# facebookresearch/gtn

Hardware: AMD Instinct MI355X
Metric: CTC forward+backward losses/sec (T=1000, C=256) (higher is better)
Workload: dtype f32; 1 GPU; BASELINE config C3: compose(ctc_target, emissions)+forwardScore CTC loss fwd+bwd, T=1000, C=256, U=100, batch=512 per GPU; global_batch=512, parallelism=dp1 (utterance sharding, all_gather of losses), rccl_ranks=0

## Files before the change

gtn_amd/_capi.py:

```python
import ctypes as C
import os

c_graph = C.c_void_p
c_graph_p = C.POINTER(C.c_void_p)
c_i32_p = C.POINTER(C.c_int)
c_i64_p = C.POINTER(C.c_int64)
c_u8_p = C.POINTER(C.c_uint8)
c_f32_p = C.POINTER(C.c_float)

GRAD_FN = C.CFUNCTYPE(C.c_int, C.c_void_p, c_graph_p, C.c_int, c_graph)
CTX_FREE = C.CFUNCTYPE(None, C.c_void_p)

OK, INVALID_ARGUMENT, LOGIC_ERROR, RUNTIME_ERROR, OUT_OF_RANGE, DEVICE_ERROR = range(6)

_SIGS = {
    "gtnx_set_device": [C.c_int],
    "gtnx_get_device": [c_i32_p],
    "gtnx_set_stream": [C.c_void_p],
    "gtnx_compose_mode": [C.c_int, C.POINTER(C.c_int)],
    "gtnx_synchronize": [],
    "gtnx_memory_stats": [C.POINTER(C.c_uint64), C.POINTER(C.c_uint64)],
    "gtnx_empty_cache": [],
    "gtnx_reclaim": [],
    "gtnx_graph_create": [C.c_int, c_graph_p],
    "gtnx_graph_copy": [c_graph, c_graph_p],
    "gtnx_graph_deep_copy": [c_graph, c_graph_p],
    "gtnx_graph_destroy": [c_graph],
    "gtnx_graph_add_node": [c_graph, C.c_int, C.c_int, c_i32_p],
    "gtnx_graph_add_arc": [c_graph, C.c_int, C.c_int, C.c_int, C.c_int, C.c_float, c_i32_p],
    "gtnx_graph_add_nodes": [c_graph, C.c_int, C.c_void_p, C.c_void_p],
    "gtnx_graph_add_arcs": [c_graph, C.c_int, C.c_void_p, C.c_void_p, C.c_void_p, C.c_void_p, C.c_void_p],
    "gtnx_graph_num_nodes": [c_graph, c_i64_p],
    "gtnx_graph_num_arcs": [c_graph, c_i64_p],
    "gtnx_graph_num_start": [c_graph, c_i64_p],
    "gtnx_graph_num_accept": [c_graph, c_i64_p],
    "gtnx_graph_item": [c_graph, c_f32_p],
    "gtnx_graph_arc_sort": [c_graph, C.c_int],
    "gtnx_graph_mark_arc_sorted": [c_graph, C.c_int],
    "gtnx_graph_ilabel_sorted": [c_graph, c_i32_p],
    "gtnx_graph_olabel_sorted": [c_graph, c_i32_p],
    "gtnx_graph_weights": [c_graph, C.c_int, C.POINTER(c_f32_p)],
    "gtnx_graph_get_weights": [c_graph, C.c_void_p],
    "gtnx_graph_set_weights": [c_graph, C.c_void_p],
    "gtnx_graph_set_weights_device": [c_graph, C.c_void_p],
    "gtnx_graph_weights_device": [c_graph, C.POINTER(C.c_void_p)],
    "gtnx_graph_labels_to_array": [c_graph, C.c_void_p, C.c_int],
    "gtnx_graph_get_start": [c_graph, C.c_void_p],
    "gtnx_graph_get_accept": [c_graph, C.c_void_p],
    "gtnx_graph_is_start": [c_graph, C.c_int, c_i32_p],
    "gtnx_graph_is_accept": [c_graph, C.c_int, c_i32_p],
    "gtnx_graph_make_accept": [c_graph, C.c_int],
    "gtnx_graph_num_out": [c_graph, C.c_int, c_i64_p],
    "gtnx_graph_num_in": [c_graph, C.c_int, c_i64_p],
    "gtnx_graph_get_out": [c_graph, C.c_int, C.c_void_p],
    "gtnx_graph_get_in": [c_graph, C.c_int, C.c_void_p],
    "gtnx_graph_get_arcs": [c_graph, C.c_void_p, C.c_void_p, C.c_void_p, C.c_void_p],
    "gtnx_graph_get_arc": [c_graph, C.c_int, c_i32_p, c_i32_p, c_i32_p, c_i32_p, c_f32_p],
    "gtnx_graph_set_weight": [c_graph, C.c_int, C.c_float],
    "gtnx_graph_calc_grad": [c_graph, c_i32_p],
    "gtnx_graph_set_calc_grad": [c_graph, C.c_int],
    "gtnx_graph_is_grad_available": [c_graph, c_i32_p],
    "gtnx_graph_grad": [c_graph, c_graph_p],
    "gtnx_graph_zero_grad": [c_graph],
    "gtnx_graph_add_grad": [c_graph, C.c_void_p, C.c_int64],
    "gtnx_graph_add_grad_graph": [c_graph, c_graph],
    "gtnx_graph_id": [c_graph, C.POINTER(C.c_size_t)],
    "gtnx_graph_create_op": [c_graph_p, C.c_int, GRAD_FN, C.c_void_p, CTX_FREE, c_graph_p],
    "gtnx_graph_num_inputs": [c_graph, c_i64_p],
    "gtnx_graph_get_input": [c_graph, C.c_int, c_graph_p],
    "gtnx_graph_set_inputs": [c_graph, c_graph_p, C.c_int],
    "gtnx_graph_set_grad_fn": [c_graph, GRAD_FN, C.c_void_p, CTX_FREE],
    "gtnx_graph_has_grad_fn": [c_graph, c_i32_p],
    "gtnx_scalar_graph": [C.c_float, C.c_int, c_graph_p],
    "gtnx_linear_graph": [C.c_int, C.c_int, C.c_int, c_graph_p],
    "gtnx_linear_graph_n": [C.c_int, C.c_int, C.c_int, C.c_int, C.c_void_p, c_graph_p],
    "gtnx_linear_graph_borrow_n": [C.c_int, C.c_int, C.c_int, C.c_int, C.c_void_p, c_graph_p],
    "gtnx_negate": [c_graph, c_graph_p],
    "gtnx_add": [c_graph, c_graph, c_graph_p],
    "gtnx_subtract": [c_graph, c_graph, c_graph_p],
    "gtnx_compose": [c_graph, c_graph, c_graph_p],
    "gtnx_intersect": [c_graph, c_graph, c_graph_p],
    "gtnx_forward_score": [c_graph, c_graph_p],
    "gtnx_viterbi_score": [c_graph, c_graph_p],
    "gtnx_viterbi_path": [c_graph, c_graph_p],
    "gtnx_negate_n": [c_graph_p, C.c_int, c_graph_p],
    "gtnx_add_n": [c_graph_p, C.c_int, c_graph_p, C.c_int, c_graph_p],
    "gtnx_subtract_n": [c_graph_p, C.c_int, c_graph_p, C.c_int, c_graph_p],
    "gtnx_compose_n": [c_graph_p, C.c_int, c_graph_p, C.c_int, c_graph_p],
    "gtnx_intersect_n": [c_graph_p, C.c_int, c_graph_p, C.c_int, c_graph_p],
    "gtnx_forward_score_n": [c_graph_p, C.c_int, c_graph_p],
    "gtnx_viterbi_score_n": [c_graph_p, C.c_int, c_graph_p],
    "gtnx_viterbi_path_n": [c_graph_p, C.c_int, c_graph_p],
    "gtnx_items_n": [c_graph_p, C.c_int, C.c_void_p],
    "gtnx_items_device_n": [c_graph_p, C.c_int, C.c_void_p],
    "gtnx_grads_device_n": [c_graph_p, C.c_int, C.c_void_p, C.c_void_p],
    "gtnx_grads_bind_device_n": [c_graph_p, C.c_int, C.c_void_p, C.c_void_p],
    "gtnx_clone": [c_graph, C.c_int, c_graph_p],
    "gtnx_concat": [c_graph_p, C.c_int, c_graph_p],
    "gtnx_closure": [c_graph, c_graph_p],
    "gtnx_union": [c_graph_p, C.c_int, c_graph_p],
    "gtnx_batch_from_graphs": [c_graph_p, C.c_int, c_graph_p],
    "gtnx_batch_ctc_targets": [C.c_void_p, C.c_void_p, C.c_int, C.c_int, C.c_int, c_graph_p],
    "gtnx_batch_asg_force_align": [C.c_void_p, C.c_void_p, C.c_int, c_graph, C.c_int, c_graph_p],
    "gtnx_batch_linear": [C.c_int, C.c_int, C.c_int, C.c_int, C.c_void_p, C.c_int, c_graph_p],
    "gtnx_batch_linear_rows": [C.c_int, C.c_int, C.c_int, C.c_void_p, C.c_int, C.c_void_p, C.c_int, c_graph_p],
    "gtnx_batch_destroy": [c_graph],
    "gtnx_batch_size": [c_graph, c_i32_p],
    "gtnx_batch_get": [c_graph, C.c_int, c_graph_p],
    "gtnx_batch_negate": [c_graph, c_graph_p],
    "gtnx_batch_add": [c_graph, c_graph, c_graph_p],
    "gtnx_batch_subtract": [c_graph, c_graph, c_graph_p],
    "gtnx_batch_subtract_into": [c_graph, c_graph, C.c_void_p, c_graph_p],
    "gtnx_batch_compose": [c_graph, c_graph, c_graph_p],
    "gtnx_batch_intersect": [c_graph, c_graph, c_graph_p],
    "gtnx_batch_forward_score": [c_graph, c_graph_p],
    "gtnx_batch_viterbi_score": [c_graph, c_graph_p],
    "gtnx_batch_viterbi_path": [c_graph, c_graph_p],
    "gtnx_batch_viterbi_align": [c_graph, C.c_void_p, C.c_void_p, C.c_int64, C.c_void_p, C.c_void_p],
    "gtnx_batch_align_stats": [c_i64_p, c_i64_p],
    "gtnx_batch_viterbi_decode": [c_graph, c_graph, C.c_void_p, C.c_void_p, C.c_int64, C.c_void_p, C.c_void_p,
                                  C.c_void_p],
    "gtnx_batch_decode_stats": [c_i64_p, c_i64_p],
    "gtnx_batch_full_connect_stats": [c_i64_p, c_i64_p],
    "gtnx_batch_linear_decode": [c_graph, C.c_void_p, C.c_int, C.c_void_p, C.c_int64, C.c_void_p, C.c_void_p,
                                 C.c_void_p, C.c_void_p],
    "gtnx_batch_linear_decode_stats": [c_i64_p, c_i64_p],
    "gtnx_batch_backward": [c_graph, C.c_int],
    "gtnx_batch_items": [c_graph, C.c_void_p],
    "gtnx_batch_items_device": [c_graph, C.c_void_p],
    "gtnx_batch_grads_bind_device": [c_graph, C.c_void_p, C.c_void_p],
    "gtnx_batch_grads_device": [c_graph, C.c_void_p, C.c_void_p],
    "gtnx_backward": [c_graph, C.c_int],
    "gtnx_backward_with_grad": [c_graph, c_graph, C.c_int],
    "gtnx_backward_n": [c_graph_p, C.c_int, C.c_int],
    "gtnx_equal": [c_graph, c_graph, c_i32_p],
    "gtnx_isomorphic": [c_graph, c_graph, c_i32_p],
    "gtnx_remove": [c_graph, C.c_int, C.c_int, c_graph_p],
    "gtnx_graph_load_buffer": [C.c_void_p, C.c_size_t, c_graph_p],
    "gtnx_parallel_enter": [],
    "gtnx_parallel_leave": [],
    "gtnx_parallel_flush": [],
    "gtnx_prof_enable": [C.c_int],
    "gtnx_prof_reset": [],
    "gtnx_prof_get": [C.c_char_p, C.POINTER(C.c_double), c_i64_p, C.POINTER(C.c_double)],
    "gtnx_prof_names": [C.c_char_p, C.c_size_t],
    "gtnx_debug_symbolic_route": [c_graph, C.c_int, c_i32_p],
    "gtnx_debug_route_name": [C.c_int, C.c_char_p, C.c_size_t],
    "gtnx_debug_viterbi_ties": [c_i64_p, c_i64_p],
    "gtnx_debug_tie_ranks": [c_graph, C.c_void_p, C.c_void_p, C.c_void_p],
    "gtnx_comm_create": [c_i32_p, C.c_int, C.POINTER(C.c_void_p)],
    "gtnx_comm_destroy": [C.c_void_p],
    "gtnx_comm_size": [C.c_void_p, c_i32_p],
    "gtnx_comm_all_gather_f32": [C.c_void_p, C.POINTER(C.c_void_p), C.POINTER(C.c_void_p), C.c_int64],
    "gtnx_comm_all_reduce_sum_f32": [C.c_void_p, C.POINTER(C.c_void_p), C.c_int64],
}

_RESTYPE = {
    "gtnx_last_error": (C.c_char_p, []),
    "gtnx_version": (C.c_char_p, []),
    "gtnx_backend": (C.c_char_p, []),
    "gtnx_device_count": (C.c_int, []),
}

ALL_SYMBOLS = sorted(list(_SIGS) + list(_RESTYPE))


def default_library_path():
    return os.path.join(os.path.dirname(os.path.abspath(__file__)), "lib", "libgtn_amd.so")


def load(path=None):
    path = path or default_library_path()
    if not os.path.exists(path):
        raise ImportError(
            f"gtn_amd: native library not found at {path}. Build it with "
            "`python -c 'import __graft_entry__ as g; g.build()'` (hipcc, gfx950). "
            "There is no CPU fallback."
        )
    lib = C.CDLL(path, mode=C.RTLD_GLOBAL if hasattr(C, "RTLD_GLOBAL") else 0)
    for name, args in _SIGS.items():
        try:
            fn = getattr(lib, name)
        except AttributeError:
            if name.startswith("gtnx_batch_") or name.startswith("gtnx_comm_") or name in ("gtnx_linear_graph_borrow_n", "gtnx_grads_bind_device_n",
                                                             "gtnx_parallel_enter", "gtnx_parallel_leave", "gtnx_parallel_flush"):
                continue
            raise
        fn.argtypes = args
        fn.restype = C.c_int
    for name, (res, args) in _RESTYPE.items():
        fn = getattr(lib, name)
        fn.argtypes = args
        fn.restype = res
    lib._path = path
    return lib
```

gtn_amd/criteria/ctc_criterion.h:

```cpp
#pragma once

#include <chrono>
#include <cstdint>
#include <stdexcept>
#include <vector>

#include "gtn/gtn.h"

namespace gtn {
namespace criteria {

inline Graph ctcTargetGraph(const std::vector<int>& target, int blank = 0, bool calcGrad = true) {
  const int L = 2 * (int)target.size() + 1;
  std::vector<uint8_t> st(L, 0), ac(L, 0);
  std::vector<int> src, dst, lab;
  src.reserve(3 * L);
  dst.reserve(3 * L);
  lab.reserve(3 * L);
  for (int l = 0; l < L; l++) {
    const int idx = (l - 1) / 2;
    st[l] = l == 0;
    ac[l] = l == L - 1 || l + 2 == L;
    const int label = l % 2 ? target[idx] : blank;
    src.push_back(l), dst.push_back(l), lab.push_back(label);
    if (l > 0) src.push_back(l - 1), dst.push_back(l), lab.push_back(label);
    if (l % 2 && l > 1 && label != target[idx - 1]) src.push_back(l - 2), dst.push_back(l), lab.push_back(label);
  }
  Graph ctc(calcGrad);
  detail::check(gtnx_graph_add_nodes(ctc.handle(), L, st.data(), ac.data()));
  detail::check(gtnx_graph_add_arcs(ctc.handle(), (int)src.size(), src.data(), dst.data(), lab.data(), lab.data(), nullptr));
  ctc.arcSort();
  return ctc;
}

struct CtcStepTimes {
  double build = 0, linear = 0, intersect = 0, forward = 0, backward = 0;
};

inline void ctcLossBatch(
    const void* emissions,
    const int* labels,
    const int* lengths,
    int B,
    int T,
    int C,
    int blank,
    void* lossDev,
    void* gradDev,
    bool targetGrad = true,
    CtcStepTimes* times = nullptr,
    Batch* targetsOut = nullptr,
    const int* frames = nullptr) {
  auto now = [] { return std::chrono::steady_clock::now(); };
  auto ms = [](auto a, auto b) { return std::chrono::duration<double, std::milli>(b - a).count(); };
  if (frames)
    for (int b = 0; b < B; ++b)
      if (frames[b] < 1 || frames[b] > T) throw std::invalid_argument("[ctcLossBatch] a frame count outside 1 .. T");
  auto t0 = now();
  Batch ctcs = Batch::ctcTargets(labels, lengths, B, blank, targetGrad);
  auto t1 = now();
  Batch ems = Batch::linear(B, T, C, emissions, gradDev != nullptr, true, frames);
  std::vector<int64_t> off(B);
  for (int b = 0; b < B; ++b) off[b] = (int64_t)b * T * C;
  if (gradDev) ems.bindGrads(gradDev, off.data());
  auto t2 = now();
  Batch comp = batched::intersect(ctcs, ems);
  auto t3 = now();
  Batch score = batched::forwardScore(comp);
  Batch norm = batched::forwardScore(ems);
  Batch losses = batched::subtract(norm, score, lossDev);
  auto t4 = now();
  if (gradDev) batched::backward(losses);
  auto t5 = now();
  if (times) *times = {ms(t0, t1), ms(t1, t2), ms(t2, t3), ms(t3, t4), ms(t4, t5)};
  losses.itemsToDevice(lossDev);
  if (gradDev) ems.gradsToDevice(gradDev, off.data());
  if (targetsOut) *targetsOut = std::move(ctcs);
}

inline void ctcLossBatch(
    const void* emissions,
    const std::vector<std::vector<int>>& targets,
    int T,
    int C,
    int blank,
    void* lossDev,
    void* gradDev,
    bool targetGrad = true,
    CtcStepTimes* times = nullptr) {
  std::vector<int> flat, len;
  for (auto& t : targets) {
    flat.insert(flat.end(), t.begin(), t.end());
    len.push_back((int)t.size());
  }
  ctcLossBatch(emissions, flat.data(), len.data(), (int)targets.size(), T, C, blank, lossDev, gradDev, targetGrad, times);
}

inline void ctcAlignBatch(
    const void* emissions,
    const int* targets,
    const int* lengths,
    int B,
    int T,
    int C,
    int blank,
    const int* frames,
    void* labels,
    void* tokens,
    void* scores) {
  Batch ctcs = Batch::ctcTargets(targets, lengths, B, blank, false);
  Batch ems = Batch::linear(B, T, C, emissions, false, true);
  Batch comp = batched::intersect(ctcs, ems);
  batched::viterbiAlign(comp, static_cast<int*>(labels), T, static_cast<int*>(tokens), static_cast<float*>(scores), frames);
}

inline void ctcDecodeBatch(
    const void* emissions,
    int B,
    int T,
    int C,
    int blank,
    const int* frames,
    void* labelsDev,
    void* scoresDev,
    void* collapsedDev,
    void* startsDev,
    void* lengthsDev) {
  Batch ems = Batch::linear(B, T, C, emissions, false, true);
  batched::linearDecode(ems, static_cast<int*>(labelsDev), T, static_cast<float*>(scoresDev), frames, blank,
                        static_cast<int*>(collapsedDev), static_cast<int*>(startsDev), static_cast<int*>(lengthsDev));
}

}
}
```

gtn_amd/csrc/band.hip:

```cpp
#include <hip/hip_runtime.h>

#include <algorithm>
#include <cstdlib>
#include <stdexcept>
#include <type_traits>

#include "kernels.h"

#ifdef GTNX_BAND_TIMING
__device__ long long g_band_timing[256];
#endif

namespace gtnx {
namespace {

constexpr float NEGF = -1.0e30f;
constexpr float DEADF = -1.0e29f;
constexpr float LOG2E = 1.44269504088896340736f;
constexpr double LN2 = 0.693147180559945309417;
constexpr int BW = 256;
constexpr int WG = 512;
constexpr int WGB = 768;
constexpr int NBE = 5;
constexpr int NBG = 7;
// ... 172 lines not shown
          }
        }
      }
    }
  }
}

__device__ __forceinline__ float em2(float x) { return fmaxf(x * LOG2E, NEGF); }

__device__ __forceinline__ int row_of(int e, int W, float invW) {
  int r = int(float(e) * invW);
  if (r * W > e) --r;
  if ((r + 1) * W <= e) ++r;
  return r;
}

template <int NS, int LN = BW>
struct Stage {
  float v[NS];
  template <bool VEC>
  __device__ __forceinline__ void issue(const GTNX_G float* src, int cnt, int tid) {
    if (cnt <= 0) return;
#pragma unroll
    for (int i = 0; i < NS / 4; ++i) {
      if (i > 0 && 4 * i * LN >= cnt) break;
      const int e = min(4 * (i * LN + tid), cnt - 4);
      const gtnx_f4 q = *reinterpret_cast<const GTNX_G gtnx_f4*>(reinterpret_cast<const GTNX_G char*>(src) + unsigned(4 * e));
      v[4 * i] = q.x;
      v[4 * i + 1] = q.y;
      v[4 * i + 2] = q.z;
      v[4 * i + 3] = q.w;
    }
  }
  int off[NS / 4];
  __device__ __forceinline__ void init_offsets(int W, int stride, int K, int tid, bool reverse = true) {
    const float invW = 1.0f / float(W);
#pragma unroll
    for (int i = 0; i < NS / 4; ++i) {
      const int e = 4 * (i * LN + tid);
      const int r = row_of(min(e, 4096), W, invW);
      off[i] = (reverse ? K - 1 - r : r) * stride + (e - r * W);
    }
  }
  template <class F>
  __device__ __forceinline__ void each_vec(int cnt, int shift, int tid, F&& f) const {
#pragma unroll
    for (int i = 0; i < NS / 4; ++i) {
      if (i > 0 && 4 * i * LN >= cnt) break;
      if (4 * (i * LN + tid) < cnt) f(i, off[i] - shift, gtnx_f4{v[4 * i], v[4 * i + 1], v[4 * i + 2], v[4 * i + 3]});
    }
  }
  __device__ __forceinline__ void settle_all() {
#pragma unroll
    for (int i = 0; i < NS; ++i) asm volatile("" : "+v"(v[i]));
  }
  template <bool VEC, class F>
  __device__ __forceinline__ void each(int cnt, int W, int tid, F&& f) const {
    const float invW = 1.0f / float(W);
    if constexpr (VEC) {
#pragma unroll
      for (int i = 0; i < NS / 4; ++i) {
        if (i > 0 && 4 * i * LN >= cnt) break;
        const int e = 4 * (i * LN + tid);
        if (e < cnt) {
          const int r = row_of(e, W, invW);
          f(i, e, r, e - r * W, gtnx_f4{v[4 * i], v[4 * i + 1], v[4 * i + 2], v[4 * i + 3]});
        }
      }
    } else {
#pragma unroll
      for (int i = 0; i < NS / 4; ++i) {
        if (i > 0 && 4 * i * LN >= cnt) break;
        if (4 * (i * LN + tid) < cnt) {
          const int e = min(4 * (i * LN + tid), cnt - 4);
          const int r0 = row_of(e, W, invW), c0 = e - r0 * W;
#pragma unroll
          for (int k = 0; k < 4; ++k) {
            int r = r0, col = c0 + k;
            if (col >= W) {
              col -= W;
              ++r;
            }
            f(i, e + k, r, col, gtnx_f4{v[4 * i + k], 0.0f, 0.0f, 0.0f});
          }
        }
      }
    }
  }
};

struct BandLds {
  int CS;
  int o_ering, o_aring, o_oring, o_snode, o_misc, total;
};
__host__ __device__ inline BandLds band_lds(int C, int K, int NSmax, bool backward) {
  BandLds L;
  L.CS = C + 4;
  int o = 0;
  L.o_ering = o;
  o += (backward ? NBGE : NBE) * K * L.CS;
  o = (o + 3) & ~3;
  L.o_aring = o;
  o += backward ? NBE * K * NSmax : 0;
  o = (o + 3) & ~3;
  L.o_oring = o;
  o += backward ? max(NBG * K * NSmax, 2 * C) : 0;
  o = (o + 3) & ~3;
  L.o_snode = o;
  o += backward ? 512 : 0;
  L.o_misc = o;
  o += 160 + 32 + 8 + 2 * NBE * K * 4 + 40 * K + 8 + 512;
  L.total = o;
  return L;
}
struct BandMisc {
  double *offr, *red, *find, *aofr;
  float *bndr, *fin, *lsep;
};
template <int K>
__device__ __forceinline__ BandMisc band_misc(float* lds, const BandLds& L) {
  BandMisc m;
  m.offr = reinterpret_cast<double*>(lds + L.o_misc);
  m.red = m.offr + 80;
  m.find = m.red + 16;
  m.aofr = m.find + 4;
  m.bndr = lds + L.o_misc + 200 + 2 * NBE * K * 4;
  m.fin = m.bndr + 40 * K;
  m.lsep = m.fin + 8;
  return m;
}

__device__ __forceinline__ float wave_max_of(const float* v, int n) {
  float mx = v[0];
  for (int j = 1; j < n; ++j) mx = fmaxf(mx, v[j]);
  return wave_max(mx);
}

template <int NPL, bool UNIT, int K, bool VEC>
__global__ __launch_bounds__(WG) void band_forward_kernel(const BandPair* __restrict__ pairs, int NSmax) {
#define GTNX_BAND_PAIR pairs[blockIdx.x]
#include "band_forward_body.inc"
#undef GTNX_BAND_PAIR
}
template <int NPL, bool UNIT, int K, bool VEC>
__global__ __launch_bounds__(WG) void band_forward_one_kernel(BandPair one, int NSmax) {
#define GTNX_BAND_PAIR one
#include "band_forward_body.inc"
#undef GTNX_BAND_PAIR
}

__device__ __forceinline__ BandPair band_patched(BandPair P, const BandPatch& pt) {
  if (pt.on) {
    const int b = P.bidx;
    P.delta = pt.delta + b;
    P.delta_norm = pt.delta_norm ? pt.delta_norm + b : nullptr;
    P.rowlse = pt.rowlse ? pt.rowlse + int64_t(b) * pt.M : nullptr;
    P.norm = nullptr;
    P.em_copy = nullptr;
    P.grad_em = pt.grad_em ? pt.grad_em + int64_t(b) * pt.A : nullptr;
    P.grad_fixed = pt.grad_fixed ? pt.grad_fixed + P.goff : nullptr;
  }
  return P;
}
template <int NPL, bool UNIT, bool GRADG, int K, bool VEC, bool BIG>
__global__ __launch_bounds__(WGB, BIG ? 3 : 6) void band_backward_kernel(const BandPair* __restrict__ pairs, int NSmax, BandPatch patch) {
#define GTNX_BAND_PAIR band_patched(pairs[blockIdx.x], patch)
#include "band_backward_body.inc"
#undef GTNX_BAND_PAIR
}
template <int NPL, bool UNIT, bool GRADG, int K, bool VEC, bool BIG>
__global__ __launch_bounds__(WGB, BIG ? 3 : 6) void band_backward_one_kernel(BandPair one, int NSmax) {
#define GTNX_BAND_PAIR one
#include "band_backward_body.inc"
#undef GTNX_BAND_PAIR
}


__global__ __launch_bounds__(512) void ctc_targets_kernel(const CtcTargetArgs* __restrict__ args, int blank) {
  const CtcTargetArgs a = args[blockIdx.x];
  __shared__ __attribute__((aligned(16))) int tl[256 + 4];
  __shared__ __attribute__((aligned(16))) int tk[256 + 4];
  const int N = a.N, U = (N - 1) >> 1, m = threadIdx.x;
  if (m < 260) {
    const int v = m < U ? a.labels[m] : 0x7fffffff;
    tl[m] = v;
    tk[m] = (m > 0 && m < U && v != a.labels[m - 1]) ? 1 : 0;
  }
  __syncthreads();
  if (m >= N) return;
  const bool odd = (m & 1) != 0;
  const int my = odd ? tl[(m - 1) >> 1] : blank;
  const int skip = odd ? tk[(m - 1) >> 1] : 0;
  const int mi = (m - 1) >> 1;
  const int before = odd ? mi : (m >> 1);
  int rank = 0, skips = 0;
  for (int o = 0; o < U; o += 4) {
    const gtnx_i4 l4 = *reinterpret_cast<const gtnx_i4*>(tl + o), k4 = *reinterpret_cast<const gtnx_i4*>(tk + o);
    const int lo[4] = {l4.x, l4.y, l4.z, l4.w}, ko[4] = {k4.x, k4.y, k4.z, k4.w};
#pragma unroll
    for (int k = 0; k < 4; ++k) {
      const bool front = o + k < before;
      rank += (lo[k] < my || (lo[k] == my && front)) ? 1 : 0;
      skips += front ? ko[k] : 0;
    }
  }
  rank += blank < my ? U + 1 : (blank == my ? (m + 1) >> 1 : 0);
  const int base = (m > 0 ? 2 * m - 1 : 0) + skips;
  GTNX_G BandNode* nd = const_cast<GTNX_G BandNode*>(a.nodes);
  nd[m].lab = my;
  nd[m].aid[0] = base;
  nd[m].aid[1] = m > 0 ? base + 1 : -1;
  nd[m].aid[2] = skip ? base + 2 : -1;
  a.nflags[m] = uint8_t((m == 0 ? NF_START : 0) | (m + 2 >= N ? NF_ACCEPT : 0));
  a.snode[rank] = m;
  a.slab[rank] = my;
  if (m == N - 1 && a.n_arcs) a.n_arcs[0] = base + 1 + (m > 0 ? 1 : 0) + skip;
}

__global__ __launch_bounds__(512) void band_viterbi_kernel(const BandDecode* __restrict__ pairs) {
  const BandDecode P = pairs[blockIdx.x];
  const int T = P.T, C = P.C, N = P.N, NS = P.NS;
  extern __shared__ float lds[];
  const float NINF = -__builtin_inff();
  float* a0 = lds;
  float* a1 = lds + 516;
  float* stage = lds + 1032;
  const int m = threadIdx.x;
  const GTNX_G gtnx_i4* nodes = reinterpret_cast<const GTNX_G gtnx_i4*>(P.nodes);
  int lab = 0;
  float wi[3] = {NINF, NINF, NINF};
  bool accept = false, start = false;
  if (m < N) {
    const gtnx_i4 q = nodes[m];
    lab = q.x >= 0 ? q.x : 0;
    const int a[3] = {q.y, q.z, q.w};
#pragma unroll
    for (int k = 0; k < 3; ++k)
      if (a[k] >= 0) wi[k] = P.w ? P.w[a[k]] : 0.0f;
    const uint8_t f = P.nflags[m];
    start = (f & NF_START) != 0;
    accept = (f & NF_ACCEPT) != 0;
  }
  if (m < 2) a0[m] = a1[m] = NINF;
  a0[2 + m] = start ? 0.0f : NINF;
  a1[2 + m] = NINF;
  int tie = 0;
  const int R = max(1, min(64, P.stage_floats / C));
  float* cur = a0;
  float* nxt = a1;
  __syncthreads();
  for (int t0 = 0; t0 < T; t0 += R) {
    const int rows = min(R, T - t0);
    for (int e = threadIdx.x; e < rows * C; e += blockDim.x) stage[e] = P.em[int64_t(t0) * C + e];
    __syncthreads();
    for (int i = 0; i < rows; ++i) {
      const float e = stage[i * C + lab];
      const float c0 = cur[2 + m] + (wi[0] + e), c1 = cur[1 + m] + (wi[1] + e), c2 = cur[m] + (wi[2] + e);
      float best = c0;
      int k = 0;
      if (c1 > best) best = c1, k = 1;
      if (c2 > best) best = c2, k = 2;
      if (best > NINF && ((k != 0 && c0 == best) || (k != 1 && c1 == best) || (k != 2 && c2 == best))) tie = 1;
      if (m < NS) P.bp[int64_t(t0 + i) * NS + m] = uint8_t(best > NINF ? k : 3);
      nxt[2 + m] = m < N ? best : NINF;
      __syncthreads();
      float* sw = cur;
      cur = nxt;
      nxt = sw;
    }
  }
  __shared__ float red_v[8];
  __shared__ int red_m[8], s_best, s_tie;
  float v = accept ? cur[2 + m] : NINF;
  int bm = (m < N && accept && v > NINF) ? m : 1 << 30;
  const float wmx = wave_max(v);
  if (!(v == wmx)) bm = 1 << 30;
  int cnt = (bm != (1 << 30)) ? 1 : 0;
  for (int o = 32; o > 0; o >>= 1) {
    bm = min(bm, __shfl_xor(bm, o));
    cnt += __shfl_xor(cnt, o);
  }
  if ((threadIdx.x & 63) == 0) {
    red_v[threadIdx.x >> 6] = wmx;
    red_m[threadIdx.x >> 6] = bm;
  }
  if (cnt > 1) tie = 1;
  if (threadIdx.x == 0) s_tie = 0;
  __syncthreads();
  if (threadIdx.x == 0) {
    float bv = NINF;
    int bn = -1;
    for (int w = 0; w < 8; ++w) {
      if (red_m[w] == (1 << 30)) continue;
      if (red_v[w] > bv) bv = red_v[w], bn = red_m[w];
      else if (red_v[w] == bv && bv > NINF) s_tie = 1;
    }
    s_best = bn;
    P.score[0] = bv;
  }
  if (tie) atomicOr(&s_tie, 1);
  __syncthreads();
  const int best = s_best;
  if (threadIdx.x == 0) {
    P.tie[0] = s_tie;
    P.path_len[0] = best >= 0 ? T : -1;
  }
  if (best < 0 || T == 0) return;
  uint8_t* bst = reinterpret_cast<uint8_t*>(stage);
  const int RB = max(1, min(T, P.stage_floats * 4 / NS));
  __shared__ int s_node;
  if (threadIdx.x == 0) {
    s_node = best;
    P.pnode[T] = best;
  }
  for (int hi = T; hi > 0; hi -= RB) {
    const int lo = max(0, hi - RB);
    __syncthreads();
    for (int e = threadIdx.x; e < (hi - lo) * NS; e += blockDim.x) bst[e] = P.bp[int64_t(lo) * NS + e];
    __syncthreads();
    if (threadIdx.x == 0) {
      int node = s_node;
      for (int t = hi - 1; t >= lo; --t) {
        node -= bst[(t - lo) * NS + node] & 3;
        P.pnode[t] = node;
      }
      s_node = node;
    }
  }
  __threadfence_block();
  __syncthreads();
  for (int t = threadIdx.x; t < T; t += blockDim.x) {
    const int m1 = P.pnode[t + 1], k = m1 - P.pnode[t];
    const gtnx_i4 q = nodes[m1];
    const int arc = k == 0 ? q.y : (k == 1 ? q.z : q.w);
    P.path_arc[t] = arc;
    P.path_lab[t] = q.x;
    P.path_w[t] = (P.w ? P.w[arc] : 0.0f) + P.em[int64_t(t) * C + q.x];
  }
}

constexpr int VBLK = 2048;

template <int NPL, bool RANKED>
__global__ __launch_bounds__(64) void band_viterbi_wave_kernel(const BandDecode* __restrict__ pairs) {
  const BandDecode P = pairs[blockIdx.x];
  const int T = P.T, C = P.C, N = P.N;
  const int lane = threadIdx.x;
  constexpr int SPW = 16 / NPL;
  constexpr int NLD = VBLK / 256;
  __shared__ __attribute__((aligned(16))) float ring[3 * VBLK];
  const float NINF = -__builtin_inff();
  const GTNX_G gtnx_i4* nodes = reinterpret_cast<const GTNX_G gtnx_i4*>(P.nodes);
  int loff[NPL];
  float w0[NPL], w1[NPL], w2[NPL], alpha[NPL];
  bool acc[NPL];
#pragma unroll
  for (int j = 0; j < NPL; ++j) {
    const int m = lane * NPL + j;
    loff[j] = 0;
    w0[j] = w1[j] = w2[j] = NINF;
    alpha[j] = NINF;
    acc[j] = false;
    if (m < N) {
      const gtnx_i4 q = nodes[m];
      loff[j] = 4 * (q.x >= 0 ? q.x : 0);
      if (q.y >= 0) w0[j] = P.w ? P.w[q.y] : 0.0f;
      if (q.z >= 0) w1[j] = P.w ? P.w[q.z] : 0.0f;
      if (q.w >= 0) w2[j] = P.w ? P.w[q.w] : 0.0f;
      const uint8_t f = P.nflags[m];
// ... 279 lines not shown
    big_lds(band_backward_kernel<NPL, false, true, K, VEC, BIG>);
    big_lds(band_backward_kernel<NPL, false, false, K, VEC, BIG>);
    if constexpr (ONE) {
      big_lds(band_backward_one_kernel<NPL, true, true, K, VEC, BIG>);
      big_lds(band_backward_one_kernel<NPL, true, false, K, VEC, BIG>);
      big_lds(band_backward_one_kernel<NPL, false, true, K, VEC, BIG>);
      big_lds(band_backward_one_kernel<NPL, false, false, K, VEC, BIG>);
    }
  }
  if constexpr (ONE) {
    if (one) {
      if (unit) {
        if (gradg) hipLaunchKernelGGL((band_backward_one_kernel<NPL, true, true, K, VEC, BIG>), dim3(1), dim3(WGB), lds, st, *one, ns);
        else hipLaunchKernelGGL((band_backward_one_kernel<NPL, true, false, K, VEC, BIG>), dim3(1), dim3(WGB), lds, st, *one, ns);
      } else {
        if (gradg) hipLaunchKernelGGL((band_backward_one_kernel<NPL, false, true, K, VEC, BIG>), dim3(1), dim3(WGB), lds, st, *one, ns);
        else hipLaunchKernelGGL((band_backward_one_kernel<NPL, false, false, K, VEC, BIG>), dim3(1), dim3(WGB), lds, st, *one, ns);
      }
      return;
    }
  }
  if (unit) {
    if (gradg) hipLaunchKernelGGL((band_backward_kernel<NPL, true, true, K, VEC, BIG>), dim3(n), dim3(WGB), lds, st, d, ns, pt);
    else hipLaunchKernelGGL((band_backward_kernel<NPL, true, false, K, VEC, BIG>), dim3(n), dim3(WGB), lds, st, d, ns, pt);
  } else {
    if (gradg) hipLaunchKernelGGL((band_backward_kernel<NPL, false, true, K, VEC, BIG>), dim3(n), dim3(WGB), lds, st, d, ns, pt);
    else hipLaunchKernelGGL((band_backward_kernel<NPL, false, false, K, VEC, BIG>), dim3(n), dim3(WGB), lds, st, d, ns, pt);
  }
}
template <int NPL, int K>
void launch_bwd(const BandPair* d, const BandPair* one, int n, int ns, size_t lds, bool unit, bool gradg, bool vec, bool big,
                hipStream_t st, const BandPatch& pt) {
  if constexpr (K == 2) {
    if (big) {
      if (vec) launch_bwd3<NPL, K, true, true>(d, one, n, ns, lds, unit, gradg, st, pt);
      else launch_bwd3<NPL, K, false, true>(d, one, n, ns, lds, unit, gradg, st, pt);
      return;
    }
  }
  if (vec) launch_bwd3<NPL, K, true, false>(d, one, n, ns, lds, unit, gradg, st, pt);
  else launch_bwd3<NPL, K, false, false>(d, one, n, ns, lds, unit, gradg, st, pt);
}

constexpr size_t LDS_TWO = 78 * 1024;
constexpr size_t LDS_ONE = 156 * 1024;

}

int band_block_rows(int C, int max_NS, bool backward);
static int band_backward_lds_stride(int K, int max_NS) { return K == 4 ? (max_NS + 15) / 16 * 16 : max_NS; }
int band_max_nodes() { return 512; }
int band_max_labels() { return 1024; }
int band_min_labels() { return 4; }
int band_npl(int max_nodes) { return max_nodes <= 256 ? 1 : 2; }
int band_row_stride(int N, int) { return (N + 3) / 4 * 4; }
#ifndef GTNX_FWD_SHIFT_ROWS
#define GTNX_FWD_SHIFT_ROWS 4
#endif
int band_forward_lgrn(int C) {
  const int K = band_block_rows(C, 0, false);
  return K >= GTNX_FWD_SHIFT_ROWS ? (GTNX_FWD_SHIFT_ROWS == 8 ? 3 : 2) : (K >= 4 ? 2 : 1);
}
int band_block_rows(int C, int max_NS, bool backward) {
  for (int k = backward ? 4 : 8; k >= 2; k /= 2) {
    if (k * C > 2048 || k * max_NS > 2048) continue;
    if (backward && k > 2 && (k * C > 1024 || k * max_NS > 1024)) continue;
    const int ns_lds = backward ? band_backward_lds_stride(k, max_NS) : max_NS;
    if (4 * size_t(band_lds(C, k, ns_lds, backward).total) + 64 <= LDS_TWO) return k;
  }
  if (4 * size_t(band_lds(C, 2, max_NS, backward).total) + 64 <= LDS_ONE) return 2;
  return 0;
}

bool band_one_ok(int npl, int C, int max_NS, bool vec, bool backward) {
  if (npl != 1 || !vec) return false;
  if (!backward) return true;
  const int K = band_block_rows(C, max_NS, true);
  return !(K * C > 1024 || K * max_NS > 1024);
}
void launch_band_forward(const BandPair* d_pairs, int n, int npl, int C, int max_NS, bool unit, bool vec, hipStream_t st,
                         const BandPair* one) {
  if (n <= 0) return;
  if (one && (n != 1 || !band_one_ok(npl, C, max_NS, vec, false))) throw std::logic_error("band.hip: not a single-pair launch");
  const int K = band_block_rows(C, 0, false);
  const size_t lds = 4 * size_t(band_lds(C, K, max_NS, false).total) + 64;
  if (npl == 1) {
    if (K == 8) launch_fwd<1, 8>(d_pairs, one, n, max_NS, lds, unit, vec, st);
    else if (K == 4) launch_fwd<1, 4>(d_pairs, one, n, max_NS, lds, unit, vec, st);
    else launch_fwd<1, 2>(d_pairs, one, n, max_NS, lds, unit, vec, st);
  } else {
    if (K == 8) launch_fwd<2, 8>(d_pairs, one, n, max_NS, lds, unit, vec, st);
    else if (K == 4) launch_fwd<2, 4>(d_pairs, one, n, max_NS, lds, unit, vec, st);
    else launch_fwd<2, 2>(d_pairs, one, n, max_NS, lds, unit, vec, st);
  }
}

void launch_band_backward(const BandPair* d_pairs, int n, int npl, int C, int max_NS, bool unit, bool gradg, bool vec,
                          hipStream_t st, const BandPair* one, const BandPatch* patch) {
  if (n <= 0) return;
  if (one && patch) throw std::logic_error("band.hip: a patched launch reads a device table");
  BandPatch pt{};
  if (patch) pt = *patch;
  if (one && (n != 1 || !band_one_ok(npl, C, max_NS, vec, true))) throw std::logic_error("band.hip: not a single-pair launch");
  const int K = band_block_rows(C, max_NS, true);
  const bool big = K * C > 1024 || K * max_NS > 1024;
  const int ns_lds = band_backward_lds_stride(K, max_NS);
  const size_t lds = 4 * size_t(band_lds(C, K, ns_lds, true).total) + 64;
  if (npl == 1) {
    if (K == 4) launch_bwd<1, 4>(d_pairs, one, n, ns_lds, lds, unit, gradg, vec, big, st, pt);
    else launch_bwd<1, 2>(d_pairs, one, n, ns_lds, lds, unit, gradg, vec, big, st, pt);
  } else {
    if (K == 4) throw std::logic_error("band.hip: four rows per block with two nodes per lane");
    launch_bwd<2, 2>(d_pairs, one, n, ns_lds, lds, unit, gradg, vec, big, st, pt);
  }
}

template <int NPL>
static void launch_viterbi_wave(const BandDecode* d_pairs, int n, int ranked, hipStream_t st) {
  if (ranked) hipLaunchKernelGGL((band_viterbi_wave_kernel<NPL, true>), dim3(n), dim3(64), 0, st, d_pairs);
  else hipLaunchKernelGGL((band_viterbi_wave_kernel<NPL, false>), dim3(n), dim3(64), 0, st, d_pairs);
}
bool band_viterbi_wave_ok(int max_nodes, int max_labels, int vec) {
  static const bool force_wg = std::getenv("GTNX_VITERBI_WG") != nullptr;
  return !force_wg && vec && max_nodes <= 512 && max_labels <= VBLK;
}
void launch_band_viterbi(const BandDecode* d_pairs, int n, int stage_floats, int max_nodes, int max_labels, int vec,
                         hipStream_t st, int ranked) {
  if (n <= 0) return;
  if (band_viterbi_wave_ok(max_nodes, max_labels, vec)) {
    if (max_nodes <= 64) launch_viterbi_wave<1>(d_pairs, n, ranked, st);
    else if (max_nodes <= 128) launch_viterbi_wave<2>(d_pairs, n, ranked, st);
    else if (max_nodes <= 256) launch_viterbi_wave<4>(d_pairs, n, ranked, st);
    else launch_viterbi_wave<8>(d_pairs, n, ranked, st);
    return;
  }
  if (ranked) return;
  static std::atomic<uint64_t> done{0};
  if (gtnx_first_on_device first{done}) big_lds(band_viterbi_kernel);
  hipLaunchKernelGGL(band_viterbi_kernel, dim3(n), dim3(512), 4 * size_t(1032 + stage_floats) + 64, st, d_pairs);
}

void launch_asg_fal_targets(const AsgFalArgs* d_args, int n, int n_labels, hipStream_t st) {
  if (n > 0) hipLaunchKernelGGL(asg_fal_targets_kernel, dim3(n), dim3(512), 0, st, d_args, n_labels);
}
void launch_asg_fal_scatter(const float* g, const int* maps, const int64_t* tab, int n_seq, int64_t longest, float* trans_grad,
                            hipStream_t st) {
  if (n_seq > 0 && longest > 0)
    hipLaunchKernelGGL(asg_fal_scatter_kernel, dim3(unsigned(std::min<int64_t>((longest + 255) / 256, 64)), unsigned(n_seq)),
                       dim3(256), 0, st, g, maps, tab, trans_grad);
}
void launch_ctc_targets(const CtcTargetArgs* d_args, int n, int blank, hipStream_t st) {
  if (n > 0) hipLaunchKernelGGL(ctc_targets_kernel, dim3(n), dim3(512), 0, st, d_args, blank);
}

}
```

gtn_amd/csrc/band_forward_body.inc:

```
#ifndef GTNX_FWD_SHIFT_ROWS
#define GTNX_FWD_SHIFT_ROWS 4
#endif
  constexpr int RNk = K >= GTNX_FWD_SHIFT_ROWS ? GTNX_FWD_SHIFT_ROWS : (K >= 4 ? 4 : K);
  constexpr int NP = K / RNk;
  constexpr int D = 8 / K > GTNX_FWD_DEPTH ? 8 / K : GTNX_FWD_DEPTH;
  const BandPair P = GTNX_BAND_PAIR;
  const int T = P.T, C = P.C, NS = P.NS;
  extern __shared__ float lds[];
  const BandLds L = band_lds(C, K, NSmax, false);
  float* ering = lds + L.o_ering;
  const BandMisc M = band_misc<K>(lds, L);
  const int CS = L.CS;
  const int wv = __builtin_amdgcn_readfirstlane(threadIdx.x >> 6);
  const bool sweeper = wv < 4;
  const int l = threadIdx.x & 63;
  const int nblocks = (T + K - 1) / K;
  const int nticks = nblocks + 3;
  GTNX_TM_INIT(0);

  if (sweeper) {
    __builtin_amdgcn_s_setprio(1);
    const int w = wv;
    const int m0 = threadIdx.x * NPL;
    NodeRegs<NPL> g;
// ... 179 lines not shown
      constexpr bool COPY = decltype(copy_tag)::value;
      float* base = ering + c5 * K * CS;
      GTNX_G float* cdst = em_copy + int64_t(c) * K * C;
      s.template each<VEC>(rows_of(c) * C, C, hid, [&](int, int e, int r, int col, gtnx_f4 q) {
        float* d = base + r * CS + col;
        if (vec) *reinterpret_cast<gtnx_f4*>(d) = gtnx_f4{em2(q.x), em2(q.y), em2(q.z), em2(q.w)};
        else d[0] = em2(q.x);
        if (COPY) {
          if (vec) __builtin_nontemporal_store(q, reinterpret_cast<GTNX_G gtnx_f4*>(cdst + e));
          else __builtin_nontemporal_store(q.x, cdst + e);
        }
      });
    };
    constexpr int LPR = BW / K, G16 = LPR / 16;
    const int EPL = (C + LPR - 1) / LPR;
    double normacc = 0.0;
    auto lse_a_n = [&](int c, int c5 , auto nconst) {
      constexpr int NE = decltype(nconst)::value;
      const int rows = rows_of(c), rr = hid / LPR, sub = hid - rr * LPR;
      if (rows <= 0) return;
      const float* e = ering + (c5 * K + min(rr, rows - 1)) * CS + sub * EPL;
      float x[NE];
      float m = NEGF;
      if (VEC && (EPL & 3) == 0) {
#pragma unroll
        for (int i = 0; i < NE; i += 4) {
          const bool in = i < EPL && sub * EPL + i < C;
          const gtnx_f4 q = in ? *reinterpret_cast<const gtnx_f4*>(e + i) : gtnx_f4{NEGF, NEGF, NEGF, NEGF};
          x[i] = q.x, x[i + 1] = q.y, x[i + 2] = q.z, x[i + 3] = q.w;
          m = fmaxf(fmaxf(m, fmaxf(q.x, q.y)), fmaxf(q.z, q.w));
        }
      } else {
#pragma unroll
        for (int i = 0; i < NE; ++i) {
          x[i] = (i < EPL && sub * EPL + i < C) ? e[i] : NEGF;
          m = fmaxf(m, x[i]);
        }
      }
      m = row16_max(m);
      float sum = 0.0f;
#pragma unroll
      for (int i = 0; i < NE; ++i) sum += (i < EPL) ? ex2(x[i] - m) : 0.0f;
      sum = row16_sum(sum);
      if ((hid & 15) == 0 && rr < rows) {
        float* p = M.lsep + (c & 1) * 256 + (rr * 8 + (sub >> 4)) * 2;
        p[0] = m;
        p[1] = sum;
      }
    };
    auto lse_a = [&](int c, int c5) {
      if (EPL <= 4) lse_a_n(c, c5, std::integral_constant<int, 4>{});
      else if (EPL <= 8) lse_a_n(c, c5, std::integral_constant<int, 8>{});
      else lse_a_n(c, c5, std::integral_constant<int, 16>{});
    };
    auto lse_b = [&](int c) {
      const int rows = rows_of(c);
      if (hid < rows) {
        const float* p = M.lsep + (c & 1) * 256 + hid * 16;
        float Mx = p[0];
#pragma unroll
        for (int k = 1; k < G16; ++k) Mx = fmaxf(Mx, p[2 * k]);
        float S = 0.0f;
#pragma unroll
        for (int k = 0; k < G16; ++k) S += p[2 * k + 1] * ex2(p[2 * k] - Mx);
        const float l2 = Mx + lg2(S);
        if (P.rowlse) P.rowlse[c * K + hid] = l2;
        normacc += double(l2);
      }
    };
    auto run = [&](auto copy_tag) {
      issue(st[0], 0);
      land(st[0], 0, 0, copy_tag);
#pragma unroll
      for (int c = 1; c <= D; ++c) issue(st[c % D], c);
      lds_barrier();
      int t5 = 0;
      for (int tau0 = 0; tau0 < nticks; tau0 += D) {
#pragma unroll
        for (int d = 0; d < D; ++d) {
          const int tau = tau0 + d;
          if (tau >= nticks) break;
          GTNX_TM(0);
          const int n5 = t5 + 1 == NBE ? 0 : t5 + 1;
          land(st[(d + 1) % D], tau + 1, n5, copy_tag);
          GTNX_TM(1);
          issue(st[(d + 1) % D], tau + 1 + D);
          GTNX_TM(2);
          if (want_lse) {
            if (tau >= 1 && tau - 1 < nblocks) lse_b(tau - 1);
            if (tau < nblocks) lse_a(tau, t5);
          }
          t5 = n5;
          GTNX_TM(4);
          lds_barrier();
          GTNX_TM(6);
          GTNX_TM_TICK();
        }
      }
    };
    auto run_copy = [&]() {
      constexpr int DC = GTNX_FWD_COPY_DEPTH < 8 / K ? 8 / K : GTNX_FWD_COPY_DEPTH;
      constexpr int R = DC + 1;
      Stage<8> sc[R];
      issue(sc[0], 0);
      land(sc[0], 0, 0, std::true_type{});
#pragma unroll
      for (int c = 1; c <= DC; ++c) issue(sc[c % R], c);
      lds_barrier();
      int t5 = 0;
      for (int tau0 = 0; tau0 < nticks; tau0 += R) {
#pragma unroll
        for (int d = 0; d < R; ++d) {
          const int tau = tau0 + d;
          if (tau >= nticks) break;
          GTNX_TM(0);
          const int n5 = t5 + 1 == NBE ? 0 : t5 + 1;
          sc[(d + 1) % R].settle_all();
          issue(sc[d % R], tau + 1 + DC);
          GTNX_TM(2);
          land(sc[(d + 1) % R], tau + 1, n5, std::true_type{});
          GTNX_TM(1);
          if (want_lse) {
            if (tau >= 1 && tau - 1 < nblocks) lse_b(tau - 1);
            if (tau < nblocks) lse_a(tau, t5);
          }
          t5 = n5;
          GTNX_TM(4);
          lds_barrier();
          GTNX_TM(6);
          GTNX_TM_TICK();
        }
      }
    };
    if (em_copy) {
      if (GTNX_FWD_COPY_ROTATE) run_copy();
      else run(std::true_type{});
    } else {
      run(std::false_type{});
    }
    if (hid < 16) M.red[hid] = normacc;
  }
  GTNX_TM_DUMP();
  lds_barrier();
  if (threadIdx.x == 0) {
    double Mx = double(NEGF);
    for (int k = 0; k < 4; ++k)
      if (M.fin[2 * k] > DEADF) Mx = fmax(Mx, M.find[k] + double(M.fin[2 * k]));
    const bool dead = !(Mx > double(DEADF));
    float S = 0.0f;
    for (int k = 0; k < 4; ++k)
      if (M.fin[2 * k] > DEADF) S += M.fin[2 * k + 1] * ex2(float(M.find[k] + double(M.fin[2 * k]) - Mx));
    const double z2 = dead ? double(NEGF) : Mx + double(lg2(S));
    P.aoff[0] = z2;
    P.score[0] = dead ? -__builtin_inff() : float(z2 * LN2);
    if (P.norm) {
      double n2 = 0.0;
      for (int k = 0; k < 16; ++k) n2 += M.red[k];
      P.norm[0] = n2 < double(DEADF) ? -__builtin_inff() : float(n2 * LN2);
    }
  }
```

gtn_amd/csrc/batch.cpp:

```cpp
#include "batch.h"

#include <algorithm>
#include <atomic>
#include <cstdlib>
#include <cstring>
#include <limits>
#include <unordered_map>
#include <unordered_set>

namespace gtnx {

namespace {

std::atomic<uint64_t> g_batch_seq{1};

struct CompMode {
  int old;
  CompMode() : old(compose_mode_hint(2)) {}
  ~CompMode() { compose_mode_hint(old); }
};

BatchP make_batch(Batch::Kind k, int n, bool cg) {
  auto b = std::make_shared<Batch>();
  b->kind = k;
// ... 231 lines not shown
    }
    DevMemP dt = upload_vec(tab);
    launch_asg_fal_scatter(out.g_dev, out.rec_mem->as<int>(), dt->as<int64_t>(), out.n, longest, gm->as<float>(), rt.stream());
    tr.add_grad_device(gm, gm->as<float>(), true);
  }
};

std::atomic<int64_t> g_full_fast{0}, g_full_fallback{0};
struct BFullOp : BatchOp {
  AsgFullArgs args{};
  DevMemP arena;
  DevMemP rows_mem;
  DevMemP w_mem;
  DevMemP through_acc;
  void backward(Batch& out) override {
    Batch& prod = *inputs[0];
    Batch& ch = *prod.chain;
    Graph& tr = prod.fixed->graphs[0];
    Runtime& rt = Runtime::get();
    const float* delta = out.g_dev;
    if (through_acc || t_batch_retain) {
      const size_t n = size_t(prod.n);
      if (!through_acc) through_acc = rt.alloc_zero(sizeof(float) * (n ? n : 1));
      launch_vec_axpby(through_acc->as<float>(), out.g_dev, nullptr, n, 1.0f, 0.0f, 1, rt.stream());
      delta = through_acc->as<float>();
    }
    const bool want_tr = tr.calc_grad();
    if (!ch.calc_grad && !want_tr) return;
    GradTarget ge;
    if (ch.calc_grad) ge = grad_target(ch, false);
    AsgFullArgs a = args;
    a.delta = delta;
    a.grad_em = ge.ptr;
    const size_t A = size_t(a.N) + size_t(a.N) * size_t(a.N);
    DevMemP part;
    if (want_tr) {
      part = rt.alloc(sizeof(float) * A * size_t(a.n));
      a.partial = part->as<float>();
    }
    {
      GTNX_PROF("asg_full_backward", 4.0 * double(a.n) * a.M * a.N * (ge.ptr ? 3 : 2) + (want_tr ? 4.0 * double(A) * a.n : 0.0));
      launch_asg_full_backward(a, rt.stream());
    }
    if (ch.calc_grad) add_scratch(ch, ge);
    if (want_tr) {
      DevMemP gm = rt.alloc(sizeof(float) * A);
      {
        GTNX_PROF("asg_full_reduce", 4.0 * double(A) * (a.n + 1));
        launch_asg_full_reduce(part->as<float>(), a.n, a.N, gm->as<float>(), rt.stream());
      }
      tr.add_grad_device(gm, gm->as<float>(), true);
    }
  }
};

struct BFromGraphsOp : BatchOp {
  DevMemP passed;
  void backward(Batch& out) override {
    Batch& src = *inputs[0];
    Runtime& rt = Runtime::get();
    const size_t n = size_t(src.n);
    DevMemP delta = rt.alloc(sizeof(float) * (n ? n : 1));
    if (passed)
      launch_vec_axpby(delta->as<float>(), out.g_dev, passed->as<float>(), n, 1.0f, -1.0f, 0, rt.stream());
    else
      rt.d2d(delta->ptr, out.g_dev, sizeof(float) * n);
    if (retain) {
      if (!passed) passed = rt.alloc(sizeof(float) * (n ? n : 1));
      rt.d2d(passed->ptr, out.g_dev, sizeof(float) * n);
    }
    std::vector<Graph> roots;
    for (int b = 0; b < src.n; ++b) {
      Graph& r = src.graphs[size_t(b)];
      if (!r.calc_grad()) continue;
      r.add_grad_device(delta, delta->as<float>() + b, true);
      roots.push_back(r);
    }
    if (!roots.empty()) op_backward(roots, nullptr, retain, false);
  }
  bool retain = false;
};

}

Batch::~Batch() {
  if (host_ev) (void)hipEventDestroy(static_cast<hipEvent_t>(host_ev));
  if (give_back && !origins.empty()) {
    for (const Origin& o : origins) {
      auto* part = new std::vector<Graph>();
      part->reserve(o.end - o.begin);
      for (size_t i = o.begin; i < o.end && i < graphs.size(); ++i) part->push_back(std::move(graphs[i]));
      give_back(o.home, part);
    }
    graphs.clear();
    return;
  }
  if (graphs.size() < 64 || !Runtime::initialized()) return;
  Runtime& rt = Runtime::get();
  for (size_t i = 0; i < graphs.size(); i += 32) {
    auto* part = new std::vector<Graph>();
    const size_t e = std::min(graphs.size(), i + 32);
    part->reserve(e - i);
    for (size_t k = i; k < e; ++k) part->push_back(std::move(graphs[k]));
    rt.defer_delete(part, [](void* q) { delete static_cast<std::vector<Graph>*>(q); }, e - i);
  }
  graphs.clear();
}

int64_t Batch::elem_size(int b) const {
  switch (kind) {
    case SCALAR: return 1;
    case LINEAR: return int64_t(M) * C;
    case CTC_TARGETS:
      if (fal) return 2 * int64_t(lab_off[size_t(b) + 1] - lab_off[size_t(b)]);
      return 3 * int64_t(2 * (lab_off[size_t(b) + 1] - lab_off[size_t(b)]) + 1);
    default: return 0;
  }
}

BatchP batch_from_graphs(std::vector<Graph> gs) {
  bool cg = false;
  for (auto& g : gs) cg |= g.calc_grad();
  BatchP b = make_batch(Batch::GRAPHS, int(gs.size()), cg);
  b->graphs = std::move(gs);
  b->materialised = true;
  return b;
}

namespace {
Graph ctc_target_graph_host(const int* t, int U, int blank, bool cg) {
  const int L = 2 * U + 1;
  std::vector<uint8_t> st(size_t(L), 0), ac(size_t(L), 0);
  std::vector<int> src, dst, lab;
  src.reserve(size_t(3 * L));
  dst.reserve(size_t(3 * L));
  lab.reserve(size_t(3 * L));
  for (int l = 0; l < L; ++l) {
    const int idx = (l - 1) / 2;
    st[size_t(l)] = l == 0;
    ac[size_t(l)] = l == L - 1 || l + 2 == L;
    const int label = l % 2 ? t[idx] : blank;
    src.push_back(l), dst.push_back(l), lab.push_back(label);
    if (l > 0) src.push_back(l - 1), dst.push_back(l), lab.push_back(label);
    if (l % 2 && l > 1 && label != t[idx - 1]) src.push_back(l - 2), dst.push_back(l), lab.push_back(label);
  }
  Graph g(cg);
  g.add_nodes(L, st.data(), ac.data());
  g.add_arcs(int(src.size()), src.data(), dst.data(), lab.data(), lab.data(), nullptr);
  g.arc_sort(false);
  return g;
}
}

BatchP batch_ctc_targets(const int* labels, const int* lengths, int n, int blank, bool calc_grad) {
  GTNX_HOST_T("batch.ctc_targets");
  if (n < 0) throw_invalid("[gtnx_batch_ctc_targets] negative batch size");
  BatchP b = make_batch(Batch::CTC_TARGETS, n, calc_grad);
  b->blank = blank;
  b->lab_off.resize(size_t(n) + 1);
  b->lab_off[0] = 0;
  for (int i = 0; i < n; ++i) {
    if (lengths[i] < 0) throw_invalid("[gtnx_batch_ctc_targets] negative length");
    b->lab_off[size_t(i) + 1] = b->lab_off[size_t(i)] + lengths[i];
    b->max_nodes = std::max(b->max_nodes, 2 * lengths[i] + 1);
  }
  const size_t total = size_t(b->lab_off[size_t(n)]);
  b->labels.assign(labels, labels + total);
  int mn = blank;
  b->max_label = blank;
  for (size_t i = 0; i < total; ++i) {
    b->max_label = std::max(b->max_label, labels[i]);
    mn = std::min(mn, labels[i]);
  }
  if (mn < 0 || b->max_nodes > band_max_nodes() || n == 0) {
    std::vector<Graph> gs;
    gs.reserve(size_t(n));
    for (int i = 0; i < n; ++i)
      gs.push_back(ctc_target_graph_host(labels + b->lab_off[size_t(i)], lengths[i], blank, calc_grad));
    return batch_from_graphs(std::move(gs));
  }
  Runtime& rt = Runtime::get();
  const size_t lab_bytes = align_up(sizeof(int) * (total ? total : 1), 256);
  const size_t arg_bytes = align_up(sizeof(CtcTargetArgs) * size_t(n), 256);
  size_t bytes = lab_bytes + arg_bytes;
  b->rec_off.resize(size_t(n));
  for (int i = 0; i < n; ++i) {
    const size_t N = size_t(2 * lengths[i] + 1);
    b->rec_off[size_t(i)] = bytes;
    bytes += align_up(sizeof(BandNode) * N, 64) + align_up(N, 64) + 2 * align_up(4 * N, 64) + 64;
  }
  b->rec_mem = rt.alloc(bytes);
  PinnedMemP pin = rt.alloc_pinned(lab_bytes + arg_bytes);
  std::memcpy(pin->ptr, labels, sizeof(int) * total);
  CtcTargetArgs* args = reinterpret_cast<CtcTargetArgs*>(static_cast<char*>(pin->ptr) + lab_bytes);
  for (int i = 0; i < n; ++i) {
    const size_t N = size_t(2 * lengths[i] + 1);
    char* base = b->rec_mem->as<char>(b->rec_off[size_t(i)]);
    CtcTargetArgs& a = args[size_t(i)];
    a.labels = b->rec_mem->as<int>() + b->lab_off[size_t(i)];
    a.nodes = reinterpret_cast<BandNode*>(base);
    base += align_up(sizeof(BandNode) * N, 64);
    a.nflags = reinterpret_cast<uint8_t*>(base);
    base += align_up(N, 64);
    a.snode = reinterpret_cast<int*>(base);
    base += align_up(4 * N, 64);
    a.slab = reinterpret_cast<int*>(base);
    base += align_up(4 * N, 64);
    a.n_arcs = reinterpret_cast<int*>(base);
    a.N = int(N);
    a.pad = 0;
  }
  rt.h2d_pinned(b->rec_mem->ptr, pin->ptr, lab_bytes + arg_bytes);
  launch_ctc_targets(reinterpret_cast<const CtcTargetArgs*>(b->rec_mem->as<char>(lab_bytes)), n, blank, rt.stream());
  return b;
}


BatchP batch_asg_force_align(const int* labels, const int* lengths, int n, Graph& transitions, int n_labels) {
  if (n < 0) throw_invalid("[gtnx_batch_asg_force_align] negative batch size");
  if (transitions.num_nodes() != int64_t(n_labels) + 1 || transitions.num_arcs() != int64_t(n_labels) * (n_labels + 1))
    throw_invalid("[gtnx_batch_asg_force_align] the transitions graph must have the asgTransitions(N) layout");
  BatchP b = make_batch(Batch::CTC_TARGETS, n, transitions.calc_grad());
  b->fal = true;
  b->trans = transitions;
  b->trans_labels = n_labels;
  b->lab_off.resize(size_t(n) + 1);
  b->lab_off[0] = 0;
  int max_u = 0;
  for (int i = 0; i < n; ++i) {
    if (lengths[i] < 0) throw_invalid("[gtnx_batch_asg_force_align] negative length");
    b->lab_off[size_t(i) + 1] = b->lab_off[size_t(i)] + lengths[i];
    max_u = std::max(max_u, lengths[i]);
  }
  b->max_nodes = max_u + 1;
  const size_t total = size_t(b->lab_off[size_t(n)]);
  b->labels.assign(labels, labels + total);
  int mn = 0;
  for (size_t i = 0; i < total; ++i) {
    b->max_label = std::max(b->max_label, labels[i]);
    mn = std::min(mn, labels[i]);
  }
  if (mn < 0 || b->max_label >= n_labels || b->max_nodes > band_max_nodes() || n == 0) {
    b->kind = Batch::GRAPHS;
    batch_materialise(*b);
    return b;
  }
  Runtime& rt = Runtime::get();
  std::vector<Weights*> ws{transitions.w.get()};
  ensure_weights_device_batch(ws);
  size_t bytes = align_up(sizeof(int) * (total ? total : 1), 256);
  b->rec_off.resize(size_t(n));
  b->w_off.resize(size_t(n));
  b->map_off.resize(size_t(n));
  for (int i = 0; i < n; ++i) {
    const size_t N = size_t(lengths[i]) + 1, A = 2 * size_t(lengths[i]);
    b->rec_off[size_t(i)] = bytes;
    bytes += align_up(sizeof(BandNode) * N, 64) + align_up(N, 64) + 2 * align_up(4 * N, 64);
    b->w_off[size_t(i)] = bytes;
    bytes += align_up(4 * (A ? A : 1), 64);
    b->map_off[size_t(i)] = bytes;
    bytes += align_up(4 * (A ? A : 1), 64);
  }
  b->rec_mem = rt.alloc(bytes);
  {
    PinnedMemP pin = rt.alloc_pinned(sizeof(int) * (total ? total : 1));
    std::memcpy(pin->ptr, labels, sizeof(int) * total);
    rt.h2d_pinned(b->rec_mem->ptr, pin->ptr, sizeof(int) * total);
  }
  std::vector<AsgFalArgs> args;
  args.resize(size_t(n));
  for (int i = 0; i < n; ++i) {
    const size_t N = size_t(lengths[i]) + 1;
    char* base = b->rec_mem->as<char>(b->rec_off[size_t(i)]);
    AsgFalArgs& a = args[size_t(i)];
    a.labels = b->rec_mem->as<int>() + b->lab_off[size_t(i)];
    a.trans_w = transitions.w->dev;
    a.nodes = reinterpret_cast<BandNode*>(base);
    base += align_up(sizeof(BandNode) * N, 64);
    a.nflags = reinterpret_cast<uint8_t*>(base);
    base += align_up(N, 64);
    a.snode = reinterpret_cast<int*>(base);
    base += align_up(4 * N, 64);
    a.slab = reinterpret_cast<int*>(base);
    a.w = b->rec_mem->as<float>(b->w_off[size_t(i)]);
    a.arc_map = b->rec_mem->as<int>(b->map_off[size_t(i)]);
    a.U = lengths[i];
    a.pad = 0;
  }
  DevMemP d = upload_vec(args);
  launch_asg_fal_targets(d->as<AsgFalArgs>(), n, n_labels, rt.stream());
  auto op = std::make_shared<BFalOp>();
  op->seq = g_batch_seq.fetch_add(1);
  b->op = op;
  return b;
}

BatchP batch_linear(int n, int M, int C, bool calc_grad, const void* dev, bool borrow, const int* rows) {
  if (n < 0 || M < 0 || C < 0) throw_invalid("[gtnx_batch_linear] negative size");
  int64_t pad_rows = 0;
  if (rows)
    for (int i = 0; i < n; ++i) {
      if (rows[i] < 1 || rows[i] > M) throw_invalid("[gtnx_batch_linear_rows] a row count outside 1 .. M");
      pad_rows += M - rows[i];
    }
  Runtime& rt = Runtime::get();
  BatchP b = make_batch(Batch::LINEAR, n, calc_grad);
  b->M = M;
  b->C = C;
  const size_t bytes = sizeof(float) * size_t(n) * size_t(M) * size_t(C);
  if (borrow && dev) {
    b->w_mem = std::make_shared<DevMem>();
    b->w_mem->ptr = const_cast<void*>(dev);
    b->w_mem->bytes = bytes;
    b->w_mem->borrowed = true;
  } else {
    b->w_mem = dev ? rt.alloc(bytes ? bytes : 4) : rt.alloc_zero(bytes ? bytes : 4);
    if (dev && bytes) rt.d2d(b->w_mem->ptr, dev, bytes);
  }
  b->w_dev = b->w_mem->as<float>();
  if (pad_rows > 0) {
    b->rows.assign(rows, rows + n);
    b->pad_floats = pad_rows * C;
  }
  return b;
}

BatchP batch_ctc_targets_from_graphs(const std::vector<Graph>& gs) {
  GTNX_HOST_T("batch.ctc_targets_from_graphs");
  const int n = int(gs.size());
  if (n == 0) return nullptr;
  detect_ctc_shape(*gs[0].s);
  const Structure& s0 = *gs[0].s;
  if (!s0.ctc_labels) return nullptr;
  const bool cg = gs[0].calc_grad();
  std::vector<int> flat, len;
  len.reserve(size_t(n));
  flat.reserve(size_t(n) * s0.ctc_labels->size());
  for (auto& g : gs) {
    detect_ctc_shape(*g.s);
    const Structure& s = *g.s;
    if (!s.ctc_labels || s.ctc_blank != s0.ctc_blank || g.calc_grad() != cg || s.N > band_max_nodes() ||
        !g.w->is_all_zero())
      return nullptr;
    flat.insert(flat.end(), s.ctc_labels->begin(), s.ctc_labels->end());
    len.push_back(int(s.ctc_labels->size()));
  }
  BatchP b = batch_ctc_targets(flat.data(), len.data(), n, s0.ctc_blank, cg);
  if (b->kind != Batch::CTC_TARGETS) return nullptr;
  b->graphs = gs;
  b->leaf = true;
  for (auto& g : gs) g.s->leaf_batch = b;
  return b;
}

BatchP batch_linear_from_graphs(const std::vector<Graph>& gs) {
  GTNX_HOST_T("batch.linear_from_graphs");
  const int n = int(gs.size());
  if (n == 0) return nullptr;
  const Structure& s0 = *gs[0].s;
  if (s0.kind != KIND_LINEAR || s0.M < 1 || s0.C < 1) return nullptr;
  const bool cg = gs[0].calc_grad();
  std::vector<Weights*> ws;
  ws.reserve(size_t(n));
  std::unordered_set<Weights*> distinct;
  for (auto& g : gs) {
    const Structure& s = *g.s;
// ... 47 lines not shown

namespace {
void push_grads_to_graphs(Batch& x) {
  if (!x.g_dev) return;
  GTNX_HOST_T("batch.push_grads_to_graphs");
  GradSink sink;
  const size_t n = size_t(x.n);
  for (size_t i = 0; i < n; ++i) {
    if (i + 6 < n) __builtin_prefetch(x.graphs[i + 6].g.get(), 1);
    if (i + 3 < n) __builtin_prefetch(x.graphs[i + 3].s.get(), 1);
    Graph& g = x.graphs[i];
    if (!g.calc_grad()) continue;
    float* ptr = x.g_dev + x.g_off[i];
    if (!g.s->deferred) {
      std::lock_guard<std::mutex> lk(g.s->grad_lock);
      if (!g.is_grad_available()) {
        g.g->lazy_owner = x.g_mem;
        g.g->lazy_ptr = ptr;
        continue;
      }
    }
    sink.add(g, x.g_mem, ptr);
  }
  sink.flush();
  x.g_dev = nullptr;
  x.g_mem.reset();
}
}

void batch_materialise(Batch& x) {
  if (x.materialised) return;
  if (x.leaf) {
    x.materialised = true;
    push_grads_to_graphs(x);
    return;
  }
  GraphSlabScope slab_scope(size_t(x.n > 0 ? x.n : 0));
  std::vector<Graph> gs;
  switch (x.fal && x.kind == Batch::GRAPHS ? Batch::CTC_TARGETS : x.kind) {
    case Batch::GRAPHS: break;
    case Batch::CTC_TARGETS:
      gs.reserve(size_t(x.n));
      if (x.fal) {
        std::vector<Graph> fals;
        for (int i = 0; i < x.n; ++i) {
          const int* t = x.labels.data() + x.lab_off[size_t(i)];
          const int U = x.lab_off[size_t(i) + 1] - x.lab_off[size_t(i)];
          Graph f(false);
          f.add_node(true, U == 0);
          for (int l = 1; l <= U; ++l) {
            f.add_node(false, l == U);
            f.add_arc(l - 1, l, t[l - 1], t[l - 1], 0.0f);
            f.add_arc(l, l, t[l - 1], t[l - 1], 0.0f);
          }
          fals.push_back(std::move(f));
        }
        std::vector<Graph> tr{x.trans};
        gs = op_compose(fals, tr, false);
        break;
      }
      for (int i = 0; i < x.n; ++i)
        gs.push_back(ctc_target_graph_host(x.labels.data() + x.lab_off[size_t(i)],
                                           x.lab_off[size_t(i) + 1] - x.lab_off[size_t(i)], x.blank, x.calc_grad));
      break;
    case Batch::LINEAR: {
      gs.reserve(size_t(x.n));
      const int64_t stride = int64_t(x.M) * x.C;
      for (int i = 0; i < x.n; ++i) {
        Graph g = Graph::make_result(x.calc_grad);
        Structure& s = *g.s;
        const int rows = x.rows_of(i);
        const int64_t A = int64_t(rows) * x.C;
        s.kind = KIND_LINEAR;
        s.M = rows;
        s.C = x.C;
        s.N = int64_t(rows) + 1;
        s.A = A;
        s.ilabel_sorted = s.olabel_sorted = true;
        Weights& w = *g.w;
        w.n = A;
        if (x.w_pend) x.w_pend->settle();
        w.dev_mem = x.w_mem;
        w.dev = x.w_dev + size_t(i) * size_t(stride);
        w.dev_valid = true;
        w.host_valid = false;
        w.version++;
        gs.push_back(std::move(g));
      }
      break;
    }
    case Batch::PRODUCT: {
      batch_materialise(*x.fixed);
      batch_materialise(*x.chain);
      std::unique_ptr<CompMode> symbolic;
      if (!x.wide && !x.full) symbolic.reset(new CompMode);
      if (x.full) g_full_fallback.fetch_add(x.n);
      gs = x.chain_first ? op_compose(x.chain->graphs, x.fixed->graphs, x.intersect)
                         : op_compose(x.fixed->graphs, x.chain->graphs, x.intersect);
      break;
    }
    case Batch::SCALAR: {
      if (!x.v_mem && x.v_dev) {
        Runtime& rt = Runtime::get();
        x.v_mem = rt.alloc(sizeof(float) * size_t(x.n ? x.n : 1));
        rt.d2d(x.v_mem->ptr, x.v_dev, sizeof(float) * size_t(x.n));
        x.v_dev = x.v_mem->as<float>();
      }
      if (!x.op) {
        gs.reserve(size_t(x.n));
        for (int i = 0; i < x.n; ++i) {
          Graph g(false);
          Structure& s = *g.s;
          s.kind = KIND_LINEAR;
          s.M = s.C = 1;
          s.N = 2;
          s.A = 1;
          Weights& w = *g.w;
          w.n = 1;
          w.dev_mem = x.v_mem;
          w.dev = x.v_dev + i;
          w.dev_valid = true;
          w.host_valid = false;
          w.version++;
          gs.push_back(std::move(g));
        }
        break;
      }
      for (auto& in : x.op->inputs) batch_materialise(*in);
      if (auto* so = dynamic_cast<BScalarOp*>(x.op.get())) {
        std::vector<Graph> none;
        gs = op_scalar(so->kind, so->inputs[0]->graphs, so->inputs.size() > 1 ? so->inputs[1]->graphs : none);
      } else {
        gs = op_shortest_distance(x.op->inputs[0]->graphs, false);
      }
      break;
    }
  }
  if (x.kind != Batch::GRAPHS || x.fal) x.graphs = std::move(gs);
  x.materialised = true;
  if (x.g_dev && ((x.kind == Batch::CTC_TARGETS && !x.fal) || x.kind == Batch::LINEAR)) {
    for (int i = 0; i < x.n; ++i) x.graphs[size_t(i)].add_grad_device(x.g_mem, x.g_dev + x.g_off[size_t(i)], true);
    x.g_dev = nullptr;
    x.g_mem.reset();
  }
}

Graph batch_get(const BatchP& x, int i) {
  if (i < 0 || i >= x->n) throw_range("[gtnx_batch_get] element index out of range");
  batch_materialise(*x);
  return x->graphs[size_t(i)];
}

namespace {
bool asg_transitions_layout(Graph& g, int N) {
  if (!g.s || g.s->lazy || g.s->deferred || g.s->kind != KIND_EXPLICIT || N < 1) return false;
  if (g.num_nodes() != int64_t(N) + 1 || g.num_arcs() != int64_t(N) * (N + 1)) return false;
  Structure& s = *g.s;
  s.ensure_host();
  const size_t A = size_t(N) * size_t(N + 1);
  if (s.src.size() != A || s.dst.size() != A || s.il.size() != A || s.ol.size() != A || s.nflags.size() != size_t(N) + 1)
    return false;
  if (s.nflags[0] != NF_START) return false;
  for (int i = 0; i < N; ++i) {
    if (s.nflags[size_t(i) + 1] != NF_ACCEPT) return false;
    if (s.src[size_t(i)] != 0 || s.dst[size_t(i)] != i + 1 || s.il[size_t(i)] != i || s.ol[size_t(i)] != i) return false;
    for (int j = 0; j < N; ++j) {
      const size_t k = size_t(N) + size_t(i) * size_t(N) + size_t(j);
      if (s.src[k] != j + 1 || s.dst[k] != i + 1 || s.il[k] != i || s.ol[k] != i) return false;
    }
  }
  return true;
}
}

void batch_full_connect_stats(int64_t* fast, int64_t* fallback) {
  if (fast) *fast = g_full_fast.load();
  if (fallback) *fallback = g_full_fallback.load();
}

BatchP batch_compose(const BatchP& a, const BatchP& b, bool intersect) {
  {
    const bool a_lin = native(*a, Batch::LINEAR) && b->kind == Batch::GRAPHS && !b->fal && b->n == 1 && b->graphs.size() == 1;
    const bool b_lin = native(*b, Batch::LINEAR) && a->kind == Batch::GRAPHS && !a->fal && a->n == 1 && a->graphs.size() == 1;
    if (a_lin || b_lin) {
      const BatchP& lin = a_lin ? a : b;
      const BatchP& one = a_lin ? b : a;
      static const bool all = [] {
        const char* e = std::getenv("GTNX_FULL_CONNECT");
        return e && *e && std::strcmp(e, "0") != 0;
      }();
      if (!lin->leaf && !lin->materialised && lin->n > 0 && lin->M >= 1 && lin->w_dev && (!lin->rows.empty() || all) &&
          asg_transitions_layout(one->graphs[0], lin->C)) {
        if (lin->C <= asg_full_max_labels()) {
          struct Op : BatchOp {
            void backward(Batch&) override {}
          };
          auto op = std::make_shared<Op>();
          op->inputs = {a, b};
          BatchP r = result(Batch::PRODUCT, lin->n, op);
          r->fixed = one;
          r->chain = lin;
          r->chain_first = a_lin;
          r->intersect = intersect;
          r->full = true;
          return r;
        }
        g_full_fallback.fetch_add(lin->n);
      }
    }
  }
  const Batch *fx = nullptr, *ch = nullptr;
  bool chain_first = false;
  if (native(*a, Batch::CTC_TARGETS) && native(*b, Batch::LINEAR)) fx = a.get(), ch = b.get();
  if (native(*a, Batch::LINEAR) && native(*b, Batch::CTC_TARGETS)) fx = b.get(), ch = a.get(), chain_first = true;
  const bool wide = fx && fx->fal && ch->C > band_max_labels() && ch->C <= asg_align_max_labels();
  if (fx && a->n == b->n && ch->C >= band_min_labels() && (ch->C <= band_max_labels() || wide) && fx->max_label < ch->C &&
      ch->M <= (1 << 20)) {
    struct Op : BatchOp {
      void backward(Batch&) override {}
    };
    auto op = std::make_shared<Op>();
    op->inputs = {a, b};
    BatchP r = result(Batch::PRODUCT, a->n, op);
    r->fixed = chain_first ? b : a;
    r->chain = chain_first ? a : b;
    r->chain_first = chain_first;
    r->intersect = intersect;
    r->wide = wide;
    return r;
  }
  batch_materialise(*a);
  batch_materialise(*b);
  return batch_from_graphs(op_compose(a->graphs, b->graphs, intersect));
}

BatchP batch_shortest_distance(const BatchP& x, bool tropical) {
  GTNX_HOST_T("batch.shortest_distance");
  Runtime& rt = Runtime::get();
  if (!tropical && native(*x, Batch::PRODUCT) && !x->materialised && x->full) {
    Batch& ch = *x->chain;
    Graph& tr = x->fixed->graphs[0];
    if (ch.w_pend) ch.w_pend->settle();
    std::vector<Weights*> ws{tr.w.get()};
    ensure_weights_device_batch(ws);
    const int n = x->n, M = ch.M, N = ch.C;
    const bool keep = x->calc_grad;
    auto op = std::make_shared<BFullOp>();
    op->inputs = {x};
    size_t bytes = align_up(4 * size_t(n), 256);
    const size_t o_zd = bytes;
    bytes = align_up(bytes + 8 * size_t(n), 256);
    const size_t o_L = bytes;
    if (keep) bytes = align_up(bytes + 8 * size_t(n) * size_t(M), 256);
    const size_t o_la = bytes;
    if (keep) bytes += 4 * size_t(n) * size_t(M) * size_t(N);
    op->arena = rt.alloc(bytes);
    if (!ch.rows.empty()) op->rows_mem = upload_vec(ch.rows);
    op->w_mem = tr.w->dev_mem;
    AsgFullArgs& a = op->args;
    a.em = ch.w_dev;
    a.rows = op->rows_mem ? op->rows_mem->as<int>() : nullptr;
    a.w = tr.w->dev;
    a.score = op->arena->as<float>();
    a.zd = op->arena->as<double>(o_zd);
    a.L = keep ? op->arena->as<double>(o_L) : nullptr;
    a.la = keep ? op->arena->as<float>(o_la) : nullptr;
    a.n = n;
    a.M = M;
    a.N = N;
    int64_t frames = 0;
    for (int b = 0; b < n; ++b) frames += ch.rows_of(b);
    {
      GTNX_PROF("asg_full_forward", 4.0 * double(frames) * N * (keep ? 2 : 1));
      launch_asg_full_forward(a, rt.stream());
    }
    g_full_fast.fetch_add(n);
    DevMemP arena = op->arena;
    BatchP r = result(Batch::SCALAR, n, op);
    r->v_mem = arena;
    r->v_dev = arena->as<float>();
    return r;
  }
  if (!tropical && native(*x, Batch::PRODUCT) && !x->materialised && !x->wide && !x->full) {
    Batch& fx = *x->fixed;
    Batch& ch = *x->chain;
    const int n = x->n, T = ch.M, C = ch.C;
    auto op = std::make_shared<BFsBandOp>();
    op->inputs = {x};
    const bool want_norm = ch.nc_norm == nullptr;
    size_t bytes = align_up(4 * size_t(n), 256);
    const size_t o_norm = bytes;
    bytes = align_up(bytes + 4 * size_t(n), 256);
    const size_t o_lse = bytes;
    bytes = align_up(bytes + 4 * size_t(n) * size_t(T > 0 ? T : 1), 256);
    std::vector<size_t> oo, ao;
    oo.resize(size_t(n));
    ao.resize(size_t(n));
    for (int b = 0; b < n; ++b) {
      const int Ub = fx.lab_off[size_t(b) + 1] - fx.lab_off[size_t(b)];
      const int N = fx.fal ? Ub + 1 : 2 * Ub + 1;
      const int ns = band_row_stride(N, band_npl(N));
      oo[size_t(b)] = bytes;
      bytes = align_up(bytes + 8 * (4 * size_t(T) + 16), 256);
      ao[size_t(b)] = bytes;
      bytes = align_up(bytes + 4 * size_t(T + 1) * size_t(ns), 256);
    }
    op->arena = rt.alloc(bytes);
    op->pairs.resize(size_t(n));
    std::vector<std::pair<BandLaunchKey, BandPair>> tab;
    tab.reserve(size_t(n));
    double abytes = 0;
    std::shared_ptr<PendingCopy> pend = ch.w_pend;
    std::unique_lock<std::mutex> pend_lock;
    bool fuse_copy = false;
    if (pend && !pend->done.load(std::memory_order_acquire)) {
      pend_lock = std::unique_lock<std::mutex>(pend->mu);
      fuse_copy = !pend->done.load(std::memory_order_relaxed) && pend->device == rt.device();
      const size_t A = size_t(T) * size_t(C);
      for (int b = 0; b < n && fuse_copy; ++b) fuse_copy = pend->src_of(ch.w_dev + size_t(b) * A) != nullptr;
      fuse_copy = fuse_copy && pend->segs.size() == size_t(n);
      if (!fuse_copy) {
        pend_lock.unlock();
        pend->settle();
      }
    }
    int64_t goff_run = 0;
    for (int b = 0; b < n; ++b) {
      BandPair& p = op->pairs[size_t(b)];
      p = BandPair{};
      const int U = fx.lab_off[size_t(b) + 1] - fx.lab_off[size_t(b)];
      const size_t N = fx.fal ? size_t(U) + 1 : size_t(2 * U + 1);
      char* base = fx.rec_mem->as<char>(fx.rec_off[size_t(b)]);
      p.nodes = reinterpret_cast<BandNode*>(base);
      base += align_up(sizeof(BandNode) * N, 64);
      p.nflags = reinterpret_cast<uint8_t*>(base);
      base += align_up(N, 64);
      p.snode = reinterpret_cast<int*>(base);
      base += align_up(4 * N, 64);
      p.slab = reinterpret_cast<int*>(base);
      p.n_lab = fx.fal ? U : int(N);
      p.w = fx.fal ? fx.rec_mem->as<float>(fx.w_off[size_t(b)]) : nullptr;
      p.em = ch.w_dev + size_t(b) * size_t(T) * size_t(C);
      p.N = int(N);
      p.T = ch.rows_of(b);
      p.C = C;
      p.NS = band_row_stride(p.N, band_npl(p.N));
      p.alpha = op->arena->as<float>(ao[size_t(b)]);
      p.aoff = op->arena->as<double>(oo[size_t(b)]);
      p.score = op->arena->as<float>(4 * size_t(b));
      if (want_norm) {
        p.norm = op->arena->as<float>(o_norm + 4 * size_t(b));
        p.rowlse = op->arena->as<float>(o_lse + 4 * size_t(b) * size_t(T));
      }
      p.hot = (!fx.fal && U + 1 >= 8) ? fx.blank : -1;
      p.lgrn = band_forward_lgrn(C);
      p.bidx = b;
      p.goff = goff_run;
      goff_run += int64_t(fx.elem_size(b));
      BandPair q = p;
      if (fuse_copy) {
        q.em = static_cast<const float*>(pend->src_of(p.em));
        q.em_copy = const_cast<float*>(p.em);
      }
      tab.push_back({BandLaunchKey{C, band_npl(q.N), fx.fal ? 0 : 1, 0, band_vec_ok(q)}, q});
      abytes += 4.0 * p.T * C + 4.0 * double(p.T + 1) * p.NS + (fuse_copy ? 4.0 * T * C : 0.0);
    }
    band_launch(tab, false, "band_forward_score", abytes, fuse_copy ? nullptr : &op->fwd_table);
    if (fuse_copy) pend->done.store(true, std::memory_order_release);
    if (want_norm) {
      ch.nc_mem = op->arena;
      ch.nc_norm = op->arena->as<float>(o_norm);
      ch.nc_rowlse = op->arena->as<float>(o_lse);
    }
    DevMemP arena = op->arena;
    BatchP r = result(Batch::SCALAR, n, op);
    r->v_mem = arena;
    r->v_dev = arena->as<float>();
    return r;
  }
  if (!tropical && native(*x, Batch::LINEAR) && !x->materialised && x->nc_norm) {
    auto op = std::make_shared<BFsLinearOp>();
    op->inputs = {x};
    BatchP r = result(Batch::SCALAR, x->n, op);
    r->v_mem = x->nc_mem;
    r->v_dev = x->nc_norm;
    return r;
  }
  if (!tropical && native(*x, Batch::LINEAR) && !x->materialised && x->n > 0 && x->M > 0) {
    if (x->w_pend) x->w_pend->settle();
    auto op = std::make_shared<BFsLinearOp>();
    op->inputs = {x};
    const int n = x->n;
    DevMemP res = rt.alloc(sizeof(float) * size_t(n) * 9);
    float* scal = res->as<float>();
    float* partial = scal + n;
    std::vector<LinArgs> args;
    args.resize(size_t(n));
    const size_t A = size_t(x->M) * size_t(x->C);
    for (int b = 0; b < n; ++b) {
      LinArgs& a = args[size_t(b)];
      a.w = x->w_dev + size_t(b) * A;
      a.M = x->rows_of(b);
      a.C = x->C;
      a.out_score = scal + b;
      a.partial = partial + size_t(b) * 8;
      a.delta = nullptr;
      a.grad = nullptr;
      a.accumulate = 0;
    }
    DevMemP d = upload_vec(args);
    const bool vec_rows = x->C % 4 == 0 && x->C <= 1024 && (reinterpret_cast<uintptr_t>(x->w_dev) & 15) == 0 && (A % 4) == 0;
    {
      GTNX_PROF("linear_forward", 4.0 * double(A) * n);
      launch_linear_forward(d->as<LinArgs>(), n, 0, vec_rows ? 1 : 0, rt.stream());
    }
    BatchP r = result(Batch::SCALAR, n, op);
    r->v_mem = res;
    r->v_dev = scal;
    return r;
  }
  batch_materialise(*x);
  return batch_from_graphs(op_shortest_distance(x->graphs, tropical));
}

BatchP batch_viterbi_path(const BatchP& x) {
  batch_materialise(*x);
  return batch_from_graphs(op_viterbi_path(x->graphs));
}

namespace {
std::atomic<int64_t> g_align_fast{0}, g_align_fallback{0};

void align_fallback(const BatchP& x, const int* frames, int* labels_dev, int64_t row_stride, int* tokens_dev,
                    float* scores_dev) {
  if (tokens_dev)
    throw_invalid("[gtnx_batch_viterbi_align] token indices are defined for device-built CTC targets or ASG force-alignment "
                  "acceptors composed with a linear batch only (this batch takes the path-graph route)");
  if (frames)
    throw_invalid("[gtnx_batch_viterbi_align] per-utterance frame counts need device-built CTC targets or ASG "
                  "force-alignment acceptors composed with a linear batch (this batch takes the path-graph route)");
  GTNX_HOST_T("batch.viterbi_align.fallback");
  Runtime& rt = Runtime::get();
  const int n = x->n;
  int64_t width = (x->kind == Batch::PRODUCT && x->chain && x->chain->kind == Batch::LINEAR) ? x->chain->M : 0;
  BatchP paths = batch_viterbi_path(x);
  for (int b = 0; b < n; ++b) width = std::max<int64_t>(width, paths->graphs[size_t(b)].num_arcs());
  if (width > row_stride) throw_invalid("[gtnx_batch_viterbi_align] row_stride is shorter than the longest path");
  PinnedMemP hl = rt.alloc_pinned(sizeof(int) * size_t(n) * size_t(width ? width : 1));
  PinnedMemP hs = rt.alloc_pinned(sizeof(float) * size_t(n));
  std::fill(hl->as<int>(), hl->as<int>() + size_t(n) * size_t(width), -1);
  for (int b = 0; b < n; ++b) {
    Graph& g = paths->graphs[size_t(b)];
    const int64_t len = g.num_arcs();
    float score = g.num_nodes() > 0 ? 0.0f : -std::numeric_limits<float>::infinity();
    if (len > 0) {
      g.s->ensure_host();
      std::copy(g.s->il.begin(), g.s->il.begin() + len, hl->as<int>() + size_t(b) * size_t(width));
      const float* w = g.weights_host(false);
      for (int64_t t = 0; t < len; ++t) score += w[t];
    }
    hs->as<float>()[b] = score;
  }
  if (width > 0)
    HIP_CHECK(hipMemcpy2DAsync(labels_dev, sizeof(int) * size_t(row_stride), hl->ptr, sizeof(int) * size_t(width),
                               sizeof(int) * size_t(width), size_t(n), hipMemcpyHostToDevice, rt.stream()));
  if (scores_dev) rt.h2d_pinned(scores_dev, hs->ptr, sizeof(float) * size_t(n));
  g_align_fallback.fetch_add(n);
}
}

void batch_align_stats(int64_t* fast, int64_t* fallback) {
  if (fast) *fast = g_align_fast.load();
  if (fallback) *fallback = g_align_fallback.load();
}

void batch_viterbi_align(const BatchP& x, const int* frames, int* labels_dev, int64_t row_stride, int* tokens_dev,
                         float* scores_dev) {
  GTNX_HOST_T("batch.viterbi_align");
  Runtime& rt = Runtime::get();
  if (!labels_dev) throw_invalid("[gtnx_batch_viterbi_align] null labels pointer");
  if (row_stride < 0) throw_invalid("[gtnx_batch_viterbi_align] negative row stride");
  const int n = x->n;
  if (n <= 0) return;
  if (!ptr_local_to(labels_dev, rt.device()) || (tokens_dev && !ptr_local_to(tokens_dev, rt.device())) ||
      (scores_dev && !ptr_local_to(scores_dev, rt.device())))
    throw_invalid("[gtnx_batch_viterbi_align] an output pointer is not memory of the engine's current device");
  bool fast = x->kind == Batch::PRODUCT && x->fixed && x->chain && x->fixed->kind == Batch::CTC_TARGETS && !x->fixed->fal &&
              x->chain->kind == Batch::LINEAR && x->fixed->rec_mem && x->fixed->n == n && x->chain->n == n;
  if (fast) {
    const Batch& fx = *x->fixed;
    const Batch& ch = *x->chain;
    const int vec = ch.C % 4 == 0 && (reinterpret_cast<uintptr_t>(ch.w_dev) & 15) == 0;
    fast = band_align_ok(fx.max_nodes, ch.C, vec) && fx.max_label < ch.C;
    for (size_t i = 0; i < fx.labels.size() && fast; ++i) fast = fx.labels[i] > fx.blank;
  }
  bool asg = x->kind == Batch::PRODUCT && x->fixed && x->chain && x->fixed->kind == Batch::CTC_TARGETS && x->fixed->fal &&
             x->chain->kind == Batch::LINEAR && x->fixed->rec_mem && x->fixed->n == n && x->chain->n == n;
  if (asg) {
    const Batch& fx = *x->fixed;
    const Batch& ch = *x->chain;
    const int vec = ch.C % 4 == 0 && (reinterpret_cast<uintptr_t>(ch.w_dev) & 15) == 0;
    asg = asg_align_ok(fx.max_nodes, ch.C, vec) && fx.trans_labels == ch.C && fx.max_label < ch.C;
  }
  if (!fast && !asg) {
    align_fallback(x, frames, labels_dev, row_stride, tokens_dev, scores_dev);
    return;
  }
  Batch& fx = *x->fixed;
  Batch& ch = *x->chain;
  const int T = ch.M, C = ch.C;
  if (row_stride < T) throw_invalid("[gtnx_batch_viterbi_align] row_stride is shorter than the chains");
  if (frames)
    for (int b = 0; b < n; ++b) {
      if (frames[b] < 0 || frames[b] > T) throw_invalid("[gtnx_batch_viterbi_align] a frame count outside 0 .. T");
      if (frames[b] > ch.rows_of(b))
        throw_invalid("[gtnx_batch_viterbi_align] a frame count beyond the rows the chain carries");
    }
  if (ch.w_pend) ch.w_pend->settle();
  if (asg) {
    const int npl = asg_align_npl(fx.max_nodes);
    const size_t plane = asg_align_plane_bytes(T, npl);
    DevMemP work = rt.alloc(plane * size_t(n));
    std::vector<AsgAlignArgs> tab(static_cast<size_t>(n));
    double abytes = 0;
    for (int b = 0; b < n; ++b) {
      AsgAlignArgs& a = tab[size_t(b)];
      a = AsgAlignArgs{};
      const int U = fx.lab_off[size_t(b) + 1] - fx.lab_off[size_t(b)];
      const size_t N = size_t(U) + 1;
      char* base = fx.rec_mem->as<char>(fx.rec_off[size_t(b)]);
      a.nodes = reinterpret_cast<BandNode*>(base);
      a.nflags = reinterpret_cast<uint8_t*>(base + align_up(sizeof(BandNode) * N, 64));
      a.w = fx.rec_mem->as<float>(fx.w_off[size_t(b)]);
      a.em = ch.w_dev + size_t(b) * size_t(T) * size_t(C);
      a.bp = work->as<unsigned>(plane * size_t(b));
      a.labels = labels_dev + int64_t(b) * row_stride;
      a.tokens = tokens_dev ? tokens_dev + int64_t(b) * row_stride : nullptr;
      a.score = scores_dev ? scores_dev + b : nullptr;
      a.N = int(N);
      a.T = frames ? frames[b] : ch.rows_of(b);
      a.T_full = T;
      a.C = C;
      abytes += 4.0 * a.T * C + 0.25 * double(a.T) * double(N) + 8.0 * a.T;
    }
    DevMemP d = upload_vec(tab);
    GTNX_PROF("asg_viterbi_align", abytes);
    launch_asg_align(d->as<AsgAlignArgs>(), n, fx.max_nodes, rt.stream());
    g_align_fast.fetch_add(n);
    return;
  }
  const int npl = align_npl(fx.max_nodes);
  const size_t plane = align_up((size_t(T) * size_t(npl) + 15) / 16 * 256 + 256, 256);
  DevMemP work = rt.alloc(plane * size_t(n));
  std::vector<AlignArgs> tab(static_cast<size_t>(n));
  double abytes = 0;
  for (int b = 0; b < n; ++b) {
    AlignArgs& a = tab[size_t(b)];
    a = AlignArgs{};
    const int* t = fx.labels.data() + fx.lab_off[size_t(b)];
    const int U = fx.lab_off[size_t(b) + 1] - fx.lab_off[size_t(b)];
    const size_t N = size_t(2 * U + 1);
    char* base = fx.rec_mem->as<char>(fx.rec_off[size_t(b)]);
    a.nodes = reinterpret_cast<BandNode*>(base);
    a.nflags = reinterpret_cast<uint8_t*>(base + align_up(sizeof(BandNode) * N, 64));
    a.em = ch.w_dev + size_t(b) * size_t(T) * size_t(C);
    a.bp = work->as<unsigned>(plane * size_t(b));
    a.labels = labels_dev + int64_t(b) * row_stride;
    a.tokens = tokens_dev ? tokens_dev + int64_t(b) * row_stride : nullptr;
    a.score = scores_dev ? scores_dev + b : nullptr;
    a.N = int(N);
    a.T = frames ? frames[b] : ch.rows_of(b);
    a.T_full = T;
    a.C = C;
    int p = 0;
    while (p + 1 < U && t[p] < t[p + 1]) ++p;
// ... 505 lines not shown
```

gtn_amd/csrc/batch.h:

```cpp
#pragma once

#include <memory>
#include <vector>

#include "ops.h"

namespace gtnx {

struct Batch;
using BatchP = std::shared_ptr<Batch>;

struct BatchOp {
  uint64_t seq = 0;
  std::vector<BatchP> inputs;
  virtual void backward(Batch& out) = 0;
  virtual ~BatchOp() {}
};

struct Batch {
  enum Kind { GRAPHS, CTC_TARGETS, LINEAR, PRODUCT, SCALAR };
  Kind kind = GRAPHS;
  int n = 0;
  bool calc_grad = false;

  bool materialised = false;
  std::vector<Graph> graphs;
  bool leaf = false;
  struct Origin {
    std::shared_ptr<void> home;
    size_t begin, end;
  };
  std::vector<Origin> origins;
  void (*give_back)(const std::shared_ptr<void>& home, std::vector<Graph>* part) = nullptr;
  std::vector<float> host_vals;
  bool host_vals_valid = false;
  PinnedMemP host_pin;
  void* host_ev = nullptr;

  std::vector<int> labels, lab_off;
  int blank = 0;
  int max_label = -1, max_nodes = 0;
  DevMemP rec_mem;
  std::vector<size_t> rec_off;
  bool fal = false;
  Graph trans;
  int trans_labels = 0;
  std::vector<size_t> w_off, map_off;
  int M = 0, C = 0;
  DevMemP w_mem;
  float* w_dev = nullptr;
  std::shared_ptr<PendingCopy> w_pend;
  DevMemP nc_mem;
  float* nc_norm = nullptr;
  float* nc_rowlse = nullptr;
  std::vector<int> rows;
  int64_t pad_floats = 0;
  DevMemP pad_mem;
  int rows_of(int b) const { return rows.empty() ? M : rows[size_t(b)]; }
  BatchP fixed, chain;
  bool chain_first = false, intersect = false;
  bool wide = false;
  bool full = false;
  DevMemP v_mem;
  float* v_dev = nullptr;

  std::shared_ptr<BatchOp> op;
  bool tape_cleared = false;
  DevMemP g_mem;
  float* g_dev = nullptr;
  std::vector<int64_t> g_off;
  DevMemP dest_mem;
  float* dest = nullptr;

  int64_t elem_size(int b) const;
  ~Batch();
};

BatchP batch_from_graphs(std::vector<Graph> gs);
BatchP batch_ctc_targets(const int* labels, const int* lengths, int n, int blank, bool calc_grad);
BatchP batch_asg_force_align(const int* labels, const int* lengths, int n, Graph& transitions, int n_labels);
BatchP batch_linear(int n, int M, int C, bool calc_grad, const void* dev, bool borrow, const int* rows = nullptr);
BatchP batch_compose(const BatchP& a, const BatchP& b, bool intersect);
BatchP batch_shortest_distance(const BatchP& x, bool tropical);
void batch_full_connect_stats(int64_t* fast, int64_t* fallback);
BatchP batch_viterbi_path(const BatchP& x);
void batch_viterbi_align(const BatchP& x, const int* frames, int* labels_dev, int64_t row_stride, int* tokens_dev,
                         float* scores_dev);
void batch_align_stats(int64_t* fast, int64_t* fallback);
void batch_viterbi_decode(const BatchP& ems, Graph& transitions, const int* frames, int* labels_dev, int64_t row_stride,
                          float* scores_dev, int* collapsed_dev, int* lengths_dev);
void batch_decode_stats(int64_t* fast, int64_t* fallback);
void batch_linear_decode(const BatchP& ems, const int* frames, int blank, int* labels_dev, int64_t row_stride,
                         float* scores_dev, int* collapsed_dev, int* starts_dev, int* lengths_dev);
void batch_linear_decode_stats(int64_t* fast, int64_t* fallback);
BatchP batch_scalar(ScalarKind k, const BatchP& a, const BatchP& b, void* items_dev = nullptr);
void batch_backward(const BatchP& root, bool retain);
void batch_items_host(const BatchP& x, float* out);
void batch_items_device(const BatchP& x, void* dev_out);
void batch_grads_device(const BatchP& x, void* dev_out, const int64_t* offsets);
void batch_grads_bind(const BatchP& x, void* dev_out, const int64_t* offsets);
Graph batch_get(const BatchP& x, int i);
float batch_item_host(const BatchP& x, int i);
void batch_prefetch_items(const BatchP& x);
BatchP batch_ctc_targets_from_graphs(const std::vector<Graph>& gs);
BatchP batch_linear_from_graphs(const std::vector<Graph>& gs);
void batch_materialise(Batch& x);

}
```

gtn_amd/csrc/capi.cpp:

```cpp
#include <atomic>
#include <chrono>
#include <condition_variable>
#include <cstdlib>
#include <cstring>
#include <mutex>
#include <string>
#include <vector>

#include "batch.h"
#include "ops.h"
#include "ops_internal.h"
#include "region.h"

#define GTNX_API extern "C" __attribute__((visibility("default")))

using namespace gtnx;

namespace {
thread_local std::string g_err;

gtnx_status_t fail(gtnx_status_t s, const std::string& m) {
  g_err = m;
  return s;
}
// ... 592 lines not shown
    auto r = make_linear_graphs_device(B, M, N, cg != 0, dev, true);
    put(r, out);
  });
}

#define UNARY_FN(name, expr, LAZY_OK, ROP)                                  \
  GTNX_API gtnx_status_t name(gtnx_graph_t g, gtnx_graph_t* out) {          \
    return guard([&] {                                                      \
      if (region_active()) {                                                \
        *out = H(region_record(ROP, RAW(g), nullptr));                      \
        return;                                                             \
      }                                                                     \
      std::vector<Graph> v{LAZY_OK ? GL(g) : G(g)};                         \
      auto r = expr;                                                        \
      *out = H(std::move(r[0]));                                            \
    });                                                                     \
  }                                                                         \
  GTNX_API gtnx_status_t name##_n(const gtnx_graph_t* g, int n, gtnx_graph_t* out) { \
    return guard([&] {                                                      \
      if (n >= 2) {                                                         \
        run_vector(ROP, g, n, nullptr, 0, out);                             \
        return;                                                             \
      }                                                                     \
      auto v = vec(g, n, LAZY_OK);                                          \
      auto r = expr;                                                        \
      put(r, out);                                                          \
    });                                                                     \
  }
#define BINARY_FN(name, expr, ROP)                                                      \
  GTNX_API gtnx_status_t name(gtnx_graph_t a, gtnx_graph_t b, gtnx_graph_t* out) {      \
    return guard([&] {                                                                  \
      if (region_active()) {                                                            \
        *out = H(region_record(ROP, RAW(a), &RAW(b)));                                  \
        return;                                                                         \
      }                                                                                 \
      std::vector<Graph> va{G(a)}, vb{G(b)};                                            \
      auto r = expr;                                                                    \
      *out = H(std::move(r[0]));                                                        \
    });                                                                                 \
  }                                                                                     \
  GTNX_API gtnx_status_t name##_n(const gtnx_graph_t* a, int na, const gtnx_graph_t* b, \
                                  int nb, gtnx_graph_t* out) {                          \
    return guard([&] {                                                                  \
      if (na >= 2 || nb >= 2) {                                                         \
        run_vector(ROP, a, na, b, nb, out);                                             \
        return;                                                                         \
      }                                                                                 \
      auto va = vec(a, na);                                                             \
      auto vb = vec(b, nb);                                                             \
      auto r = expr;                                                                    \
      put(r, out);                                                                      \
    });                                                                                 \
  }

namespace {
std::vector<Graph> g_empty;
void run_vector(RegionOp op, const gtnx_graph_t* a, int na, const gtnx_graph_t* b, int nb, gtnx_graph_t* out) {
  std::vector<Graph*> pa(static_cast<size_t>(na > 0 ? na : 0)), pb(static_cast<size_t>(b && nb > 0 ? nb : 0));
  for (int i = 0; i < na; ++i) pa[size_t(i)] = &RAW(a[i]);
  for (size_t i = 0; i < pb.size(); ++i) pb[i] = &RAW(b[i]);
  const int n = b ? std::max(na, nb) : na;
  std::vector<Graph> res(static_cast<size_t>(n), Graph(Graph::Empty{}));
  region_run_vector(op, pa.data(), na, b ? pb.data() : nullptr, nb, res.data());
  put(res, out);
}
}
UNARY_FN(gtnx_negate, op_scalar(SK_NEGATE, v, g_empty), false, RO_NEG)
BINARY_FN(gtnx_add, op_scalar(SK_ADD, va, vb), RO_ADD)
BINARY_FN(gtnx_subtract, op_scalar(SK_SUBTRACT, va, vb), RO_SUB)
BINARY_FN(gtnx_compose, op_compose(va, vb, false), RO_COMPOSE)
BINARY_FN(gtnx_intersect, op_compose(va, vb, true), RO_INTERSECT)
UNARY_FN(gtnx_forward_score, op_shortest_distance(v, false), true, RO_FS)
UNARY_FN(gtnx_viterbi_score, op_shortest_distance(v, true), true, RO_VS)
UNARY_FN(gtnx_viterbi_path, op_viterbi_path(v), true, RO_VP)

GTNX_API gtnx_status_t gtnx_items_n(const gtnx_graph_t* g, int n, float* out) {
  return guard([&] {
    bool all = n > 0;
    for (int i = 0; i < n && all; ++i) {
      Graph& raw = RAW(g[i]);
      all = raw.s->pending && region_item(raw, out + i);
    }
    if (all) return;
    auto v = vec(g, n);
    items_host(v, out);
  });
}
GTNX_API gtnx_status_t gtnx_items_device_n(const gtnx_graph_t* g, int n, void* out) {
  return guard([&] {
    std::vector<Graph*> hs(static_cast<size_t>(n > 0 ? n : 0));
    for (int i = 0; i < n; ++i) hs[size_t(i)] = &RAW(g[i]);
    if (region_items_device(hs.data(), n, out)) return;
    auto v = vec(g, n);
    items_device(v, out);
  });
}
GTNX_API gtnx_status_t gtnx_grads_device_n(const gtnx_graph_t* g, int n, void* out, const int64_t* offsets) {
  return guard([&] {
    auto v = vec(g, n);
    grads_device(v, out, offsets);
  });
}
GTNX_API gtnx_status_t gtnx_grads_bind_device_n(const gtnx_graph_t* g, int n, void* out, const int64_t* offsets) {
  return guard([&] {
    auto v = vec(g, n);
    grads_bind_device(v, out, offsets);
  });
}

GTNX_API gtnx_status_t gtnx_clone(gtnx_graph_t g, int projection, gtnx_graph_t* out) {
  return guard([&] {
    if (projection < 0 || projection > 2) throw_invalid("[gtnx_clone] projection must be 0, 1 or 2");
    std::vector<Graph> v{G(g)};
    *out = H(op_rational(RAT_CLONE, v, projection));
  });
}
GTNX_API gtnx_status_t gtnx_concat(const gtnx_graph_t* g, int n, gtnx_graph_t* out) {
  return guard([&] {
    auto v = vec(g, n);
    *out = H(op_rational(RAT_CONCAT, v, 0));
  });
}
GTNX_API gtnx_status_t gtnx_closure(gtnx_graph_t g, gtnx_graph_t* out) {
  return guard([&] {
    std::vector<Graph> v{G(g)};
    *out = H(op_rational(RAT_CLOSURE, v, 0));
  });
}
GTNX_API gtnx_status_t gtnx_union(const gtnx_graph_t* g, int n, gtnx_graph_t* out) {
  return guard([&] {
    auto v = vec(g, n);
    *out = H(op_rational(RAT_UNION, v, 0));
  });
}

GTNX_API gtnx_status_t gtnx_remove(gtnx_graph_t g, int ilabel, int olabel, gtnx_graph_t* out) {
  return guard([&] { *out = H(op_remove(G(g), ilabel, olabel)); });
}

namespace {
inline BatchP& BH(gtnx_batch_t h) {
  if (!h) throw_invalid("null batch handle");
  return *reinterpret_cast<BatchP*>(h);
}
inline gtnx_batch_t HB(BatchP b) { return reinterpret_cast<gtnx_batch_t>(new BatchP(std::move(b))); }
}
GTNX_API gtnx_status_t gtnx_batch_from_graphs(const gtnx_graph_t* g, int n, gtnx_batch_t* out) {
  return guard([&] { *out = HB(batch_from_graphs(vec(g, n, true))); });
}
GTNX_API gtnx_status_t gtnx_batch_ctc_targets(const int* labels, const int* lengths, int n, int blank, int cg,
                                              gtnx_batch_t* out) {
  return guard([&] { *out = HB(batch_ctc_targets(labels, lengths, n, blank, cg != 0)); });
}
GTNX_API gtnx_status_t gtnx_batch_asg_force_align(const int* labels, const int* lengths, int n, gtnx_graph_t transitions,
                                                  int n_labels, gtnx_batch_t* out) {
  return guard([&] { *out = HB(batch_asg_force_align(labels, lengths, n, G(transitions), n_labels)); });
}
GTNX_API gtnx_status_t gtnx_batch_linear(int n, int M, int N, int cg, const void* dev, int borrow, gtnx_batch_t* out) {
  return guard([&] { *out = HB(batch_linear(n, M, N, cg != 0, dev, borrow != 0)); });
}
GTNX_API gtnx_status_t gtnx_batch_linear_rows(int n, int M, int N, const int* rows, int cg, const void* dev, int borrow,
                                             gtnx_batch_t* out) {
  return guard([&] { *out = HB(batch_linear(n, M, N, cg != 0, dev, borrow != 0, rows)); });
}
GTNX_API gtnx_status_t gtnx_batch_destroy(gtnx_batch_t b) {
  return guard([&] {
    auto* p = reinterpret_cast<BatchP*>(b);
    if (!p) return;
    if (Runtime::initialized())
      Runtime::get().defer_delete(p, [](void* q) { delete static_cast<BatchP*>(q); },
                                  (*p && (*p)->materialised) ? size_t((*p)->n > 0 ? (*p)->n : 1) : 1);
    else
      delete p;
  });
}
GTNX_API gtnx_status_t gtnx_batch_size(gtnx_batch_t b, int* out) {
  return guard([&] { *out = BH(b)->n; });
}
GTNX_API gtnx_status_t gtnx_batch_get(gtnx_batch_t b, int i, gtnx_graph_t* out) {
  return guard([&] { *out = H(batch_get(BH(b), i)); });
}
GTNX_API gtnx_status_t gtnx_batch_negate(gtnx_batch_t a, gtnx_batch_t* out) {
  return guard([&] { *out = HB(batch_scalar(SK_NEGATE, BH(a), nullptr)); });
}
GTNX_API gtnx_status_t gtnx_batch_add(gtnx_batch_t a, gtnx_batch_t b, gtnx_batch_t* out) {
  return guard([&] { *out = HB(batch_scalar(SK_ADD, BH(a), BH(b))); });
}
GTNX_API gtnx_status_t gtnx_batch_subtract(gtnx_batch_t a, gtnx_batch_t b, gtnx_batch_t* out) {
  return guard([&] { *out = HB(batch_scalar(SK_SUBTRACT, BH(a), BH(b))); });
}
GTNX_API gtnx_status_t gtnx_batch_subtract_into(gtnx_batch_t a, gtnx_batch_t b, void* items_device, gtnx_batch_t* out) {
  return guard([&] { *out = HB(batch_scalar(SK_SUBTRACT, BH(a), BH(b), items_device)); });
}
GTNX_API gtnx_status_t gtnx_batch_compose(gtnx_batch_t a, gtnx_batch_t b, gtnx_batch_t* out) {
  return guard([&] { *out = HB(batch_compose(BH(a), BH(b), false)); });
}
GTNX_API gtnx_status_t gtnx_batch_intersect(gtnx_batch_t a, gtnx_batch_t b, gtnx_batch_t* out) {
  return guard([&] { *out = HB(batch_compose(BH(a), BH(b), true)); });
}
GTNX_API gtnx_status_t gtnx_batch_forward_score(gtnx_batch_t a, gtnx_batch_t* out) {
  return guard([&] { *out = HB(batch_shortest_distance(BH(a), false)); });
}
GTNX_API gtnx_status_t gtnx_batch_viterbi_score(gtnx_batch_t a, gtnx_batch_t* out) {
  return guard([&] { *out = HB(batch_shortest_distance(BH(a), true)); });
}
GTNX_API gtnx_status_t gtnx_batch_full_connect_stats(int64_t* fast, int64_t* fallback) {
  return guard([&] { batch_full_connect_stats(fast, fallback); });
}
GTNX_API gtnx_status_t gtnx_batch_viterbi_path(gtnx_batch_t a, gtnx_batch_t* out) {
  return guard([&] { *out = HB(batch_viterbi_path(BH(a))); });
}
GTNX_API gtnx_status_t gtnx_batch_viterbi_align(gtnx_batch_t a, const int* frames, void* labels_device, int64_t row_stride,
                                                void* tokens_device, void* scores_device) {
  return guard([&] {
    batch_viterbi_align(BH(a), frames, static_cast<int*>(labels_device), row_stride, static_cast<int*>(tokens_device),
                        static_cast<float*>(scores_device));
  });
}
GTNX_API gtnx_status_t gtnx_batch_align_stats(int64_t* fast, int64_t* fallback) {
  return guard([&] { batch_align_stats(fast, fallback); });
}
GTNX_API gtnx_status_t gtnx_batch_viterbi_decode(gtnx_batch_t ems, gtnx_graph_t transitions, const int* frames,
                                                 void* labels_device, int64_t row_stride, void* scores_device,
                                                 void* collapsed_device, void* lengths_device) {
  return guard([&] {
    batch_viterbi_decode(BH(ems), G(transitions), frames, static_cast<int*>(labels_device), row_stride,
                         static_cast<float*>(scores_device), static_cast<int*>(collapsed_device),
                         static_cast<int*>(lengths_device));
  });
}
GTNX_API gtnx_status_t gtnx_batch_decode_stats(int64_t* fast, int64_t* fallback) {
  return guard([&] { batch_decode_stats(fast, fallback); });
}
GTNX_API gtnx_status_t gtnx_batch_linear_decode(gtnx_batch_t ems, const int* frames, int blank, void* labels_device,
                                                int64_t row_stride, void* scores_device, void* collapsed_device,
                                                void* starts_device, void* lengths_device) {
  return guard([&] {
    batch_linear_decode(BH(ems), frames, blank, static_cast<int*>(labels_device), row_stride,
                        static_cast<float*>(scores_device), static_cast<int*>(collapsed_device),
                        static_cast<int*>(starts_device), static_cast<int*>(lengths_device));
  });
}
GTNX_API gtnx_status_t gtnx_batch_linear_decode_stats(int64_t* fast, int64_t* fallback) {
  return guard([&] { batch_linear_decode_stats(fast, fallback); });
}
GTNX_API gtnx_status_t gtnx_batch_backward(gtnx_batch_t a, int retain) {
  return guard([&] { batch_backward(BH(a), retain != 0); });
}
GTNX_API gtnx_status_t gtnx_batch_items(gtnx_batch_t a, float* out) {
  return guard([&] { batch_items_host(BH(a), out); });
}
GTNX_API gtnx_status_t gtnx_batch_items_device(gtnx_batch_t a, void* out) {
  return guard([&] { batch_items_device(BH(a), out); });
}
GTNX_API gtnx_status_t gtnx_batch_grads_bind_device(gtnx_batch_t a, void* out, const int64_t* offsets) {
  return guard([&] { batch_grads_bind(BH(a), out, offsets); });
}
GTNX_API gtnx_status_t gtnx_batch_grads_device(gtnx_batch_t a, void* out, const int64_t* offsets) {
  return guard([&] { batch_grads_device(BH(a), out, offsets); });
}

GTNX_API gtnx_status_t gtnx_backward(gtnx_graph_t g, int retain) {
  return guard([&] {
    if (region_active()) {
      region_record_backward(RAW(g), retain != 0);
      return;
    }
    std::vector<Graph> v{G(g)};
    op_backward(v, nullptr, retain != 0);
  });
}
GTNX_API gtnx_status_t gtnx_backward_with_grad(gtnx_graph_t g, gtnx_graph_t grad, int retain) {
  return guard([&] {
    std::vector<Graph> v{G(g)};
    op_backward(v, &G(grad), retain != 0);
  });
}
GTNX_API gtnx_status_t gtnx_backward_n(const gtnx_graph_t* g, int n, int retain) {
  return guard([&] {
    if (n >= 2) {
      std::vector<Graph*> roots(static_cast<size_t>(n));
      for (int i = 0; i < n; ++i) roots[size_t(i)] = &RAW(g[i]);
      region_run_backward_vector(roots.data(), n, retain != 0);
      return;
    }
    auto v = vec(g, n);
    op_backward(v, nullptr, retain != 0);
  });
}

GTNX_API gtnx_status_t gtnx_equal(gtnx_graph_t a, gtnx_graph_t b, int* out) {
  return guard([&] { *out = graphs_equal(G(a), G(b)); });
}
GTNX_API gtnx_status_t gtnx_isomorphic(gtnx_graph_t a, gtnx_graph_t b, int* out) {
  return guard([&] { *out = graphs_isomorphic(G(a), G(b)); });
}

GTNX_API gtnx_status_t gtnx_graph_load_buffer(const void* data, size_t bytes, gtnx_graph_t* out) {
  return guard([&] {
    if (!data) throw_invalid("[gtnx_graph_load_buffer] null buffer");
    *out = H(op_load_buffer(data, bytes));
  });
}

GTNX_API gtnx_status_t gtnx_prof_enable(int on) {
  return guard([&] {
// ... 40 lines not shown
```

gtn_amd/csrc/kernels.h:

```cpp
#pragma once

#include <hip/hip_runtime.h>

#include <cstdint>

#include <atomic>
#include <cstdint>
struct gtnx_first_on_device {
  std::atomic<uint64_t>& done;
  uint64_t bit;
  bool first;
  explicit gtnx_first_on_device(std::atomic<uint64_t>& d) : done(d) {
    int dev = 0;
    (void)hipGetDevice(&dev);
    bit = uint64_t(1) << (dev & 63);
    first = !(done.load(std::memory_order_acquire) & bit);
  }
  gtnx_first_on_device(const gtnx_first_on_device&) = delete;
  ~gtnx_first_on_device() {
    if (first) done.fetch_or(bit, std::memory_order_acq_rel);
  }
  explicit operator bool() const { return first; }
};

// ... 196 lines not shown
  const GTNX_G gtnx_i4* s2_in;
};
int compose_max_bitmap_bytes();
size_t compose_chain_bitmap_bytes(int No, int slices);
size_t compose_g1_cache_bytes(int N1, int A1);
int compose_lds_budget(int wide);
void launch_compose(const ComposeArgs* d_args, int n, int matcher, int lin1, int lin2, int dyn_lds_bytes,
                    int fast, int cache1, int wide, hipStream_t st);
void launch_compose_replicate(const ComposeArgs* d_args, int n, int lin2, int max_acap, hipStream_t st);
int compose_wide_node_cap();
void launch_compose_wide(const ComposeArgs* d_args, int n, int lin2, int max_acap, hipStream_t st);
void launch_compose_pairs(const ComposeArgs* d_args, int n, int matcher, hipStream_t st);
void launch_sorted_view(const DGraph& g, int key_olabel, void* out_view , void* in_view, hipStream_t st);
struct ComposeFillArgs {
  int N, A;
  const GTNX_G int* out_off;
  const GTNX_G int* dst;
  const GTNX_G float* w;
  const GTNX_G int* gi1;
  const GTNX_G int* gi2;
  const GTNX_G int* lab1;
  const GTNX_G int* lab2;
  int C1, C2;
  GTNX_G int* src;
  GTNX_G int* il;
  GTNX_G int* ol;
  GTNX_G int* in_cursor;
  GTNX_G int* in_list;
  GTNX_G int* in_src;
  GTNX_G float* in_w;
};
void launch_compose_fill(const ComposeFillArgs& a, hipStream_t st);
size_t compose_transpose_scratch_bytes(int n, int maxNcap);
void launch_compose_transpose(const ComposeArgs* d_args, int n, int maxAcap, int maxNcap, void* scratch,
                              hipStream_t st);

void launch_build_records(const DGraph& g, void* out_rec, void* in_rec, hipStream_t st);

struct ComposeGradArgs {
  const GTNX_G float* delta;
  const GTNX_G int* gi1;
  const GTNX_G int* gi2;
  int A;
  int A1, A2;
  GTNX_G float* grad1;
  GTNX_G float* grad2;
};
void launch_compose_grad(const ComposeGradArgs* d_args, int n, int maxA, hipStream_t st);

struct LazyGroup {
  DGraph g;
  int chain_first;
  int T, C, N, nb;
  int Npad, Cpad;
  const gtnx_i4* lrec_in;
  const gtnx_i4* lrec_out;
  const float* const* em;
  const float* em_base;
  int64_t em_stride;
  float* alpha;
  float* beta;
  int* bp;
  float* score;
  int* best;
  const float* const* delta;
  float* const* grad_em;
  float* grad_fixed;
  const float* E;
  const float* cmax;
  const int* nlab;
  int lab_unique;
  int tie_by_node;
  float* amax;
  float* bmax;
  float* amaxp;
  float* bmaxp;
  int ntp;
  float* R;
  const float* zt;
  float* xt[2];
  const float* Ep;
  const float* ETp;
  int Kpad, Npad2, nbpad;
  int rot;
  int rel;
  const float* mp_Wq;
  const int* mp_colidx;
  const int* mp_colnode;
  const int* mp_dead;
  int mp_ncol, mp_ndead;
};
size_t lazy_step_lds_bytes(const LazyGroup& g);
int lazy_tile_nodes();
int lazy_tile_batch();
void launch_lazy_pack(const LazyGroup& g, gtnx_i4* lrec_in, gtnx_i4* lrec_out, hipStream_t st);
void launch_lazy_init(const LazyGroup& g, int which, hipStream_t st);
void launch_lazy_step(const LazyGroup& g, int t, int mode, int backward, hipStream_t st);
void launch_lazy_final(const LazyGroup& g, int mode, hipStream_t st);
void launch_lazy_path(const LazyGroup& g, int* path_arc, int* path_il, int* path_ol, float* path_w, int* path_len,
                      hipStream_t st);
void launch_lazy_local_z(const LazyGroup& g, float* zt, hipStream_t st);
void launch_lazy_chain_grad(const LazyGroup& g, const int* node_label, hipStream_t st);
bool lazy_z_chain_grad_ok(const LazyGroup& g);
void launch_lazy_z_chain_grad(const LazyGroup& g, const int* node_label, float* zt, hipStream_t st);
void launch_lazy_fixed_grad(const LazyGroup& g, int max_in_deg, hipStream_t st);
struct LazyPathGrad {
  const float* delta;
  int delta_stride;
  const int* path_arc;
  const int* il;
  const int* ol;
  int len, C, chain_first;
  float* grad_chain;
  float* grad_fixed;
};
void launch_lazy_path_grad(const LazyPathGrad& a, hipStream_t st);
struct LazyPair {
  DGraph g;
  const GTNX_G float* em;
  GTNX_G float* alpha;
  GTNX_G float* score;
  const GTNX_G float* delta;
  GTNX_G float* grad_em;
  GTNX_G float* grad_fixed;
  int T, C, chain_first, pad;
};
int lazy_pair_max_nodes();
int lazy_pair_max_degree();
int lazy_pair_block(int max_nodes);
int lazy_pair_max_labels(int block);
void launch_lazy_pair_forward(const LazyPair* d_pairs, int n, int block, int C, int cus, hipStream_t st);
void launch_lazy_pair_backward(const LazyPair* d_pairs, int n, int block, int C, int cus, hipStream_t st);
struct BandNode {
  int lab;
  int aid[3];
};
struct BandPair {
  const GTNX_G BandNode* nodes;
  const GTNX_G uint8_t* nflags;
  const GTNX_G int* snode;
  const GTNX_G int* slab;
  const GTNX_G float* w;
  const GTNX_G float* em;
  GTNX_G float* em_copy;
  GTNX_G float* alpha;
  GTNX_G double* aoff;
  GTNX_G float* score;
  GTNX_G float* norm;
  GTNX_G float* rowlse;
  const GTNX_G float* delta;
  const GTNX_G float* delta_norm;
  GTNX_G float* grad_em;
  GTNX_G float* grad_fixed;
  int N, T, C, NS;
  int hot;
  int lgrn;
  int n_lab;
  int bidx;
  int64_t goff;
};
struct BandPatch {
  int on;
  int M;
  const GTNX_G float* delta;
  const GTNX_G float* delta_norm;
  GTNX_G float* rowlse;
  GTNX_G float* grad_em;
  GTNX_G float* grad_fixed;
  int64_t A;
};
struct BandDecode {
  const GTNX_G BandNode* nodes;
  const GTNX_G uint8_t* nflags;
  const GTNX_G float* w;
  const GTNX_G float* em;
  GTNX_G uint8_t* bp;
  GTNX_G int* pnode;
  GTNX_G int* path_arc;
  GTNX_G int* path_lab;
  GTNX_G float* path_w;
  GTNX_G int* path_len;
  GTNX_G float* score;
  GTNX_G int* tie;
  const GTNX_G int* rank_in;
  const GTNX_G int* rank_acc;
  int N, T, C, NS;
  int stage_floats, pad;
};
void launch_band_viterbi(const BandDecode* d_pairs, int n, int stage_floats, int max_nodes, int max_labels, int vec,
                         hipStream_t st, int ranked = 0);
bool band_viterbi_wave_ok(int max_nodes, int max_labels, int vec);
struct AlignArgs {
  const GTNX_G BandNode* nodes;
  const GTNX_G uint8_t* nflags;
  const GTNX_G float* em;
  GTNX_G unsigned* bp;
  GTNX_G int* labels;
  GTNX_G int* tokens;
  GTNX_G float* score;
  int N, T, T_full, C;
  int p, pad;
};
int align_npl(int max_nodes);
bool band_align_ok(int max_nodes, int max_labels, int vec);
void launch_band_align(const AlignArgs* d_args, int n, int max_nodes, hipStream_t st);
struct AsgAlignArgs {
  const GTNX_G BandNode* nodes;
  const GTNX_G uint8_t* nflags;
  const GTNX_G float* w;
  const GTNX_G float* em;
  GTNX_G unsigned* bp;
  GTNX_G int* labels;
  GTNX_G int* tokens;
  GTNX_G float* score;
  int N, T, T_full, C;
};
int asg_align_npl(int max_nodes);
int asg_align_max_labels();
bool asg_align_ok(int max_nodes, int max_labels, int vec);
size_t asg_align_plane_bytes(int T, int npl);
void launch_asg_align(const AsgAlignArgs* d_args, int n, int max_nodes, hipStream_t st);
struct RationalSeg {
  DGraph g;
  int node_off, arc_off;
  int conn_off;
  int keep_start, keep_accept;
  int pad;
};
struct RationalOut {
  int N, A;
  GTNX_G int* src;
  GTNX_G int* dst;
  GTNX_G int* il;
  GTNX_G int* ol;
  GTNX_G float* w;
  GTNX_G uint8_t* nflags;
  GTNX_G int* start_list;
  GTNX_G int* accept_list;
  GTNX_G int* out_off;
  GTNX_G int* out_list;
  GTNX_G int* in_off;
  GTNX_G int* in_list;
};
size_t rational_csr_temp_bytes(int N, int A);
void launch_rational_build(const RationalSeg* d_segs, int nseg, int max_A, int max_N, int max_conn, const RationalOut& out,
                           int projection, int closure, void* temp, hipStream_t st);
void launch_rational_adjacency(const RationalOut& out, void* temp, hipStream_t st);
struct RemoveArgs {
  DGraph g;
  int ilabel, olabel;
  const GTNX_G int* new_id;
  const GTNX_G int* roots;
  int K, root0, rows;
  GTNX_G int* stamp;
  GTNX_G int* queue;
  GTNX_G int* arc_cnt;
  const GTNX_G int* arc_off;
  RationalOut out;
};
void launch_remove_keep(const DGraph& g, int ilabel, int olabel, int* keep, hipStream_t st);
void launch_remove_roots(const int* keep, const int* new_id, int N, int* roots, hipStream_t st);
void launch_remove_walk(const RemoveArgs& a, bool emit, hipStream_t st);
size_t scan_temp_bytes(int n);
void launch_exclusive_scan(const int* in, int* out, int n, void* temp, size_t temp_bytes, hipStream_t st);
void launch_rational_load(const void* rows, const float* w, const uint8_t* flags, const RationalOut& out, void* temp,
                          hipStream_t st);
struct CtcTargetArgs {
  const GTNX_G int* labels;
  GTNX_G BandNode* nodes;
  GTNX_G uint8_t* nflags;
  GTNX_G int* snode;
  GTNX_G int* slab;
  GTNX_G int* n_arcs;
  int N, pad;
};
void launch_ctc_targets(const CtcTargetArgs* d_args, int n, int blank, hipStream_t st);
struct AsgFalArgs {
  const GTNX_G int* labels;
  const GTNX_G float* trans_w;
  GTNX_G BandNode* nodes;
  GTNX_G uint8_t* nflags;
  GTNX_G int* snode;
  GTNX_G int* slab;
  GTNX_G float* w;
  GTNX_G int* arc_map;
  int U, pad;
};
void launch_asg_fal_targets(const AsgFalArgs* d_args, int n, int n_labels, hipStream_t st);
void launch_asg_fal_scatter(const float* g, const int* maps, const int64_t* tab , int n_seq, int64_t longest,
                            float* trans_grad, hipStream_t st);
int band_max_nodes();
int band_max_labels();
int band_min_labels();
int band_npl(int max_nodes);
int band_row_stride(int N, int npl);
int band_forward_lgrn(int C);
bool band_one_ok(int npl, int C, int max_NS, bool vec, bool backward);
void launch_band_forward(const BandPair* d_pairs, int n, int npl, int C, int max_NS, bool unit, bool vec, hipStream_t st,
                         const BandPair* one = nullptr);
void launch_band_backward(const BandPair* d_pairs, int n, int npl, int C, int max_NS, bool unit, bool gradg, bool vec,
                          hipStream_t st, const BandPair* one = nullptr, const BandPatch* patch = nullptr);
void launch_lazy_dense_prep(const LazyGroup& g, float* E, float* cmax, hipStream_t st);
void launch_lazy_dense_step(const LazyGroup& g, int t, int backward, hipStream_t st, const float* vin = nullptr,
                            float* vout = nullptr);
void launch_lazy_dense_fixed_grad(const LazyGroup& g, hipStream_t st);
size_t maxplus_w_floats(const LazyGroup& g);
void launch_maxplus_prep(const LazyGroup& g, hipStream_t st);
void launch_maxplus_step(const LazyGroup& g, int t, hipStream_t st);
void launch_maxplus_path(const LazyGroup& g, int* path_arc, int* path_il, int* path_ol, float* path_w, int* path_len,
                         hipStream_t st);
void launch_asg_decode(const LazyGroup& g, const int* d_frames, int* labels, int64_t row_stride, float* scores,
                       int* collapsed, int* lengths, hipStream_t st);
void launch_lazy_mfma_prep(const LazyGroup& g, hipStream_t st);
void launch_lazy_mfma_init(const LazyGroup& g, int which, hipStream_t st);
void launch_lazy_mfma_step(const LazyGroup& g, int t, int backward, hipStream_t st);
size_t lazy_mfma_chain_sync_ints(const LazyGroup& g);
bool launch_lazy_mfma_chain(const LazyGroup& g, int backward, int* zeroed_sync, int cus, hipStream_t st);
void launch_lazy_mfma_keys(float* keys, int64_t n, hipStream_t st);
void launch_lazy_mfma_rowmax(const LazyGroup& g, int which, hipStream_t st);
void launch_lazy_mfma_score(const LazyGroup& g, hipStream_t st);
size_t lazy_mfma_fixed_grad_scratch_bytes(const LazyGroup& g);
void launch_lazy_mfma_fixed_grad(const LazyGroup& g, void* pair_consts , hipStream_t st, void* partials = nullptr,
                                 size_t partials_bytes = 0);

void launch_fill_i32(int* p, int v, size_t n, hipStream_t st);
void launch_fill_f32(float* p, float v, size_t n, hipStream_t st);
void launch_scalar_seed(float* root, float* g0, float s0, int acc0, float* g1, float s1, int acc1, size_t n, hipStream_t st);
struct ScalarArgs {
  const GTNX_G float* a;
  const GTNX_G float* b;
  GTNX_G float* out;
  GTNX_G float* mirror;
};
void launch_scalar_combine(const ScalarArgs* d_args, int n, float sa, float sb, hipStream_t st);
void launch_copy_small(void* dst, const void* src, size_t bytes, hipStream_t st);
void launch_scalar_combine_one(const ScalarArgs& a, float sa, float sb, hipStream_t st);
struct ScalarFanArgs {
  const GTNX_G float* d;
  GTNX_G float* seed;
  GTNX_G float* o0;
  GTNX_G float* o1;
};
void launch_scalar_fan(const ScalarFanArgs* d_args, int n, float s0, float s1, hipStream_t st);
void launch_scalar_fan_one(const ScalarFanArgs& a, float s0, float s1, hipStream_t st);
struct AxpyArgs {
  GTNX_G float* dst;
  const GTNX_G float* src;
  int64_t n;
  float scale;
};
void launch_axpy_batch(const AxpyArgs* d_args, int n, int64_t maxn, int atomic, hipStream_t st);
struct CopySeg {
  void* dst;
  const void* src;
  int64_t bytes;
};
void launch_copy_segments(const CopySeg* d_segs, int n, int64_t max_bytes, hipStream_t st);
void launch_gather_scalars(const float* const* d_ptrs, float* out, int n, hipStream_t st);
void launch_vec_axpby(float* out, const float* a, const float* b, size_t n, float sa, float sb, int accumulate, hipStream_t st);
struct ScatterArgs {
  const GTNX_G int* idx;
  const GTNX_G float* delta;
  GTNX_G float* grad;
  int n;
};
void launch_scatter_add(const ScatterArgs* d_args, int n, int maxn, hipStream_t st);
struct PadFillArgs {
  GTNX_G float* base;
  const GTNX_G int64_t* offs;
  const GTNX_G int* rows;
  const GTNX_G int64_t* prefix;
  int64_t stride;
  int n, C;
};
void launch_pad_fill(const PadFillArgs& a, int64_t total_floats, hipStream_t st);
struct AsgFullArgs {
  const GTNX_G float* em;
  const GTNX_G int* rows;
  const GTNX_G float* w;
  GTNX_G float* score;
  GTNX_G float* la;
  GTNX_G double* L;
  GTNX_G double* zd;
  const GTNX_G float* delta;
  GTNX_G float* grad_em;
  GTNX_G float* partial;
  int n, M, N;
};
int asg_full_max_labels();
void launch_asg_full_forward(const AsgFullArgs& a, hipStream_t st);
void launch_asg_full_backward(const AsgFullArgs& a, hipStream_t st);
void launch_asg_full_reduce(const float* partial, int n, int N, float* out, hipStream_t st);
struct LinearDecodeArgs {
  const GTNX_G float* em;
  const GTNX_G int* frames;
  GTNX_G int* labels;
  GTNX_G float* rowmax;
  GTNX_G float* scores;
  GTNX_G int* collapsed;
  GTNX_G int* starts;
  GTNX_G int* lengths;
  int64_t row_stride;
  int n, M, C, blank;
};
void launch_linear_decode(const LinearDecodeArgs& a, int which, hipStream_t st);
void launch_linear_materialize(int M, int C, int* src, int* dst, int* il, int* ol, hipStream_t st);

}
```

gtn_amd/csrc/runtime.cpp:

```cpp
#include "runtime.h"

#include "kernels.h"

#include <malloc.h>

#include <atomic>
#include <condition_variable>
#include <cstring>
#include <deque>
#include <thread>

namespace gtnx {

namespace {
constexpr int kMaxDevices = 64;
std::atomic<Runtime*> g_rts[kMaxDevices];
std::atomic<bool> g_any_rt{false};
std::mutex g_rt_mu;
std::atomic<int> g_default_device{-1};
thread_local int t_device = -1;

int hip_device_now() {
  int d = -1;
  if (hipGetDevice(&d) != hipSuccess) {
// ... 432 lines not shown

void Runtime::release_dev(void* p, size_t bytes) {
  std::lock_guard<std::mutex> lk(mu_);
  free_dev_.emplace(bytes, p);
  in_use_ -= bytes;
}

PinnedMemP Runtime::alloc_pinned(size_t bytes) {
  size_t sz = round_size(bytes ? bytes : 1);
  void* p = nullptr;
  {
    std::lock_guard<std::mutex> lk(mu_);
    auto recycle = [&] {
      for (size_t i = 0; i < pending_pinned_.size();) {
        if (hipEventQuery(pending_pinned_[i].ev) == hipSuccess) {
          for (auto& b : pending_pinned_[i].blocks) free_pinned_.emplace(b.second, b.first);
          ev_pool_.push_back(pending_pinned_[i].ev);
          if (i + 1 != pending_pinned_.size()) pending_pinned_[i] = std::move(pending_pinned_.back());
          pending_pinned_.pop_back();
        } else {
          (void)hipGetLastError();
          ++i;
        }
      }
    };
    recycle();
    {
      auto hit = free_pinned_.lower_bound(sz);
      if ((hit == free_pinned_.end() || hit->first > sz * 2) && !unstamped_pinned_.empty()) stamp_pinned_locked();
    }
    auto it = free_pinned_.lower_bound(sz);
    if (it != free_pinned_.end() && it->first <= sz * 2) {
      p = it->second;
      sz = it->first;
      free_pinned_.erase(it);
    }
  }
  if (!p) {
    GTNX_HOST_T("runtime.alloc_pinned.hipHostMalloc (pool miss)");
    HIP_CHECK(hipHostMalloc(&p, sz, hipHostMallocDefault));
  }
  auto m = std::make_shared<PinnedMem>();
  m->ptr = p;
  m->bytes = sz;
  m->owner = this;
  return m;
}

void Runtime::release_pinned(void* p, size_t bytes) {
  OnDevice here(device_);
  std::lock_guard<std::mutex> lk(mu_);
  static const size_t every = [] {
    const char* e = std::getenv("GTNX_PINNED_STAMP_EVERY");
    return e && std::atol(e) > 0 ? size_t(std::atol(e)) : kPinnedStampEvery;
  }();
  unstamped_pinned_.emplace_back(p, bytes);
  if (unstamped_pinned_.size() >= every) stamp_pinned_locked();
}
void Runtime::stamp_pinned_locked() {
  if (unstamped_pinned_.empty()) return;
  hipEvent_t ev;
  if (!ev_pool_.empty()) {
    ev = ev_pool_.back();
    ev_pool_.pop_back();
  } else if (hipEventCreateWithFlags(&ev, hipEventDisableTiming) != hipSuccess) {
    (void)hipGetLastError();
    (void)hipStreamSynchronize(stream_);
    for (auto& b : unstamped_pinned_) free_pinned_.emplace(b.second, b.first);
    unstamped_pinned_.clear();
    return;
  }
  (void)hipEventRecord(ev, stream_);
  pending_pinned_.push_back({ev, std::move(unstamped_pinned_)});
  unstamped_pinned_.clear();
}

void Runtime::empty_cache() {
  OnDevice here(device_);
  drain_all_inboxes();
  (void)hipStreamSynchronize(stream_);
  std::lock_guard<std::mutex> lk(mu_);
  for (auto& kv : free_dev_) {
    (void)hipFree(kv.second);
    reserved_ -= kv.first;
  }
  free_dev_.clear();
  for (auto& b : unstamped_pinned_) free_pinned_.emplace(b.second, b.first);
  unstamped_pinned_.clear();
  for (auto& g : pending_pinned_) {
    for (auto& b : g.blocks) free_pinned_.emplace(b.second, b.first);
    ev_pool_.push_back(g.ev);
  }
  pending_pinned_.clear();
  for (auto& kv : free_pinned_) (void)hipHostFree(kv.second);
  free_pinned_.clear();
}

void Runtime::stats(uint64_t* reserved, uint64_t* in_use) {
  drain_deferred();
  std::lock_guard<std::mutex> lk(mu_);
  if (reserved) *reserved = reserved_;
  if (in_use) *in_use = in_use_;
}

void Runtime::h2d(void* dst, const void* src, size_t bytes) {
  if (bytes) HIP_CHECK(hipMemcpyAsync(dst, src, bytes, hipMemcpyHostToDevice, stream_));
}
void Runtime::d2h_sync(void* dst, const void* src, size_t bytes) {
  if (bytes && bytes <= 4096) {
    PinnedMemP p = alloc_pinned(bytes);
    d2h_pinned_async(p->ptr, src, bytes);
    drain_while_busy();
    HIP_CHECK(hipStreamSynchronize(stream_));
    std::memcpy(dst, p->ptr, bytes);
    return;
  }
  if (bytes) HIP_CHECK(hipMemcpyAsync(dst, src, bytes, hipMemcpyDeviceToHost, stream_));
  drain_while_busy();
  HIP_CHECK(hipStreamSynchronize(stream_));
}
void Runtime::sync_while_draining() {
  drain_while_busy();
  HIP_CHECK(hipStreamSynchronize(stream_));
}
namespace {
bool local_to(const void* p, int dev) {
  static const int ndev = Runtime::device_count();
  if (ndev <= 1) return true;
  hipPointerAttribute_t a;
  if (hipPointerGetAttributes(&a, p) != hipSuccess) {
    (void)hipGetLastError();
    return false;
  }
  return a.type == hipMemoryTypeHost || (a.type == hipMemoryTypeDevice && a.device == dev);
}
}
bool ptr_local_to(const void* p, int dev) { return local_to(p, dev); }
void Runtime::d2d(void* dst, const void* src, size_t bytes) {
  if (!bytes) return;
  if (bytes <= (size_t(1) << 20) && local_to(src, device_) && local_to(dst, device_)) {
    launch_copy_small(dst, src, bytes, stream_);
    return;
  }
  HIP_CHECK(hipMemcpyAsync(dst, src, bytes, hipMemcpyDeviceToDevice, stream_));
}
void Runtime::d2h_pinned_async(void* pinned_dst, const void* src, size_t bytes) {
  if (!bytes) return;
  if (bytes <= (size_t(1) << 20) && local_to(src, device_)) {
    launch_copy_small(pinned_dst, src, bytes, stream_);
    return;
  }
  HIP_CHECK(hipMemcpyAsync(pinned_dst, src, bytes, hipMemcpyDeviceToHost, stream_));
}
void Runtime::h2d_pinned(void* dst, const void* pinned_src, size_t bytes) {
  if (!bytes) return;
  static const size_t lim = [] {
    const char* e = std::getenv("GTNX_H2D_KERNEL_BYTES");
    return e ? size_t(std::atol(e)) : size_t(1) << 20;
  }();
  if (bytes <= lim && local_to(dst, device_)) {
    launch_copy_small(dst, pinned_src, bytes, stream_);
    return;
  }
  HIP_CHECK(hipMemcpyAsync(dst, pinned_src, bytes, hipMemcpyHostToDevice, stream_));
}

Runtime::MirrorSlot Runtime::mirror_slot() {
  {
    std::lock_guard<std::mutex> lk(mu_);
    if (!mirror_ring_) {
      OnDevice here(device_);
      void* p = nullptr;
      HIP_CHECK(hipHostMalloc(&p, sizeof(float) * kMirrorSlots, hipHostMallocDefault));
      mirror_gen_ = new std::atomic<uint64_t>[kMirrorSlots];
      for (size_t i = 0; i < kMirrorSlots; ++i) mirror_gen_[i].store(0);
      mirror_ring_ = static_cast<float*>(p);
    }
  }
  const uint64_t g = mirror_next_.fetch_add(1) + 1;
  const size_t i = size_t(g % kMirrorSlots);
  mirror_gen_[i].store(g);
  return {mirror_ring_ + i, g};
}
bool Runtime::mirror_read(const MirrorSlot& m, float* out) {
  if (!m.ptr || !mirror_ring_) return false;
  const size_t i = size_t(m.ptr - mirror_ring_);
  if (i >= kMirrorSlots || mirror_gen_[i].load() != m.gen) return false;
  sync();
  const float v = *static_cast<volatile float*>(m.ptr);
  if (mirror_gen_[i].load() != m.gen) return false;
  *out = v;
  return true;
}

void Runtime::prof_enable(bool on) {
  if (!on) collect_prof();
  prof_on_ = on;
}
void Runtime::prof_reset() {
  collect_prof();
  prof_.clear();
}

Runtime::Scope::Scope(Runtime* r, const char* name, double bytes) : rt(r), idx(-1) {
  if (!rt->prof_on_) return;
  ProfRec rec;
  rec.name = name;
  rec.bytes = bytes;
  auto get_ev = [&]() {
    hipEvent_t e;
    HIP_CHECK(hipEventCreate(&e));
    return e;
  };
  rec.a = get_ev();
  rec.b = get_ev();
  HIP_CHECK(hipEventRecord(rec.a, rt->stream_));
  idx = (int)rt->prof_recs_.size();
  rt->prof_recs_.push_back(rec);
}
Runtime::Scope::~Scope() {
  if (idx >= 0) (void)hipEventRecord(rt->prof_recs_[idx].b, rt->stream_);
}

void Runtime::prof_add_bytes(const std::string& name, double bytes) { prof_[name].bytes += bytes; }

void Runtime::collect_prof() {
  if (prof_recs_.empty()) return;
  (void)hipStreamSynchronize(stream_);
  for (auto& r : prof_recs_) {
    float ms = 0;
    if (hipEventElapsedTime(&ms, r.a, r.b) == hipSuccess) {
      auto& e = prof_[r.name];
      e.total_ms += ms;
      e.launches += 1;
      e.bytes += r.bytes;
    } else {
      (void)hipGetLastError();
    }
    (void)hipEventDestroy(r.a);
    (void)hipEventDestroy(r.b);
  }
  prof_recs_.clear();
}

ProfEntry Runtime::prof_get(const std::string& name) {
  collect_prof();
  auto it = prof_.find(name);
  return it == prof_.end() ? ProfEntry{} : it->second;
}

std::string Runtime::prof_names() {
  collect_prof();
  std::string s;
  for (auto& kv : prof_) {
    if (!s.empty()) s += "\n";
    s += kv.first;
  }
  return s;
}

}

#include <chrono>
namespace gtnx {
namespace {
struct HostTable {
  std::mutex mu;
  std::map<std::string, std::pair<double, long>> t;
  ~HostTable() {
    if (!HostTimer::enabled()) return;
    for (auto& kv : t)
      std::fprintf(stderr, "[gtnx host] %-28s calls %6ld  total %9.2f ms  avg %8.3f ms\n", kv.first.c_str(),
                   kv.second.second, kv.second.first, kv.second.first / double(kv.second.second));
  }
};
HostTable& host_table() {
  static HostTable h;
  return h;
}
double now_ms() {
  return std::chrono::duration<double, std::milli>(std::chrono::steady_clock::now().time_since_epoch()).count();
}
}
double host_now_ms() { return now_ms(); }
bool HostTimer::enabled() {
  static const bool e = std::getenv("GTNX_HOST_TIMING") != nullptr;
  return e;
}
void host_timer_add(const char* name, double ms) {
  if (!HostTimer::enabled()) return;
  HostTable& h = host_table();
  std::lock_guard<std::mutex> lk(h.mu);
  auto& e = h.t[name];
  e.first += ms;
  e.second += 1;
}
HostTimer::HostTimer(const char* n) : name(n), t0(enabled() ? now_ms() : 0.0) {}
HostTimer::~HostTimer() {
  if (!enabled()) return;
  const double dt = now_ms() - t0;
  HostTable& h = host_table();
  std::lock_guard<std::mutex> lk(h.mu);
  auto& e = h.t[name];
  e.first += dt;
  e.second += 1;
}
}
```

gtn_amd/csrc/runtime.h:

```cpp
#pragma once

#include <atomic>
#include <functional>
#include <map>
#include <memory>
#include <mutex>
#include <string>
#include <vector>

#include "common.h"

namespace gtnx {

class Runtime;

struct DevMem {
  void* ptr = nullptr;
  size_t bytes = 0;
  bool borrowed = false;
  Runtime* owner = nullptr;
  std::shared_ptr<void> keep;
  ~DevMem();
  template <class T>
  T* as(size_t byte_off = 0) const { return reinterpret_cast<T*>(static_cast<char*>(ptr) + byte_off); }
};
using DevMemP = std::shared_ptr<DevMem>;

struct PinnedMem {
  void* ptr = nullptr;
  size_t bytes = 0;
  Runtime* owner = nullptr;
  ~PinnedMem();
  template <class T>
  T* as(size_t byte_off = 0) const { return reinterpret_cast<T*>(static_cast<char*>(ptr) + byte_off); }
};
using PinnedMemP = std::shared_ptr<PinnedMem>;

struct ProfEntry {
  double total_ms = 0;
  int64_t launches = 0;
  double bytes = 0;
};

class Runtime {
 public:
  static Runtime& get();
  static Runtime& of(int device);
  static int device_count();
  static bool initialized();
  static void set_current_device(int d);
  static int current_device();
  int device() const { return device_; }
  void activate();

  hipStream_t stream() const { return stream_; }
  void set_stream(hipStream_t s);
  void sync();

  DevMemP alloc(size_t bytes);
  DevMemP alloc_zero(size_t bytes);
  PinnedMemP alloc_pinned(size_t bytes);
  void release_dev(void* p, size_t bytes);
  void release_pinned(void* p, size_t bytes);
  void empty_cache();
  void stats(uint64_t* reserved, uint64_t* in_use);

  struct Inbox {
    std::mutex mu;
    std::vector<std::pair<void*, void (*)(void*)>> items;
    size_t load = 0;
    bool dead = false;
  };
  using InboxP = std::shared_ptr<Inbox>;
  static InboxP home();
  static void send(const InboxP& to, void* p, void (*del)(void*));
  static void drain_all_inboxes();
  static void defer_delete(void* p, void (*del)(void*), size_t weight = 1);
  static void drain_deferred();
  static bool drain_some(size_t max_items);
  static size_t deferred_count();
  void drain_until(void* hip_event);
  void drain_while_busy();
  void sync_while_draining();

  struct SideJob;
  using SideJobP = std::shared_ptr<SideJob>;
  SideJobP side_launch(std::function<void(hipStream_t)> fn);
  void side_join(const SideJobP& job);

  void h2d(void* dst, const void* src, size_t bytes);
  void d2h_sync(void* dst, const void* src, size_t bytes);
  void d2d(void* dst, const void* src, size_t bytes);
  void h2d_pinned(void* dst, const void* pinned_src, size_t bytes);
  void d2h_pinned_async(void* pinned_dst, const void* src, size_t bytes);

  struct MirrorSlot {
    float* ptr = nullptr;
    uint64_t gen = 0;
  };
  static constexpr size_t kMirrorSlots = 1024;
  MirrorSlot mirror_slot();
  bool mirror_read(const MirrorSlot& m, float* out);

  void prof_enable(bool on);
  void prof_add_bytes(const std::string& name, double bytes);
  void prof_reset();
  bool prof_on() const { return prof_on_; }
  struct Scope {
    Runtime* rt;
    int idx;
    Scope(Runtime* r, const char* name, double bytes);
    ~Scope();
  };
  ProfEntry prof_get(const std::string& name);
  std::string prof_names();
  int cu_count() const { return cu_count_; }

 private:
  explicit Runtime(int device);
  void collect_prof();
  float* mirror_ring_ = nullptr;
  std::atomic<uint64_t>* mirror_gen_ = nullptr;
  std::atomic<uint64_t> mirror_next_{0};
  hipStream_t own_stream_ = nullptr;
  hipStream_t stream_ = nullptr;
  int device_ = 0;
  int cu_count_ = 256;
  std::mutex mu_;
  std::multimap<size_t, void*> free_dev_;
  std::multimap<size_t, void*> free_pinned_;
  struct PinnedGroup {
    hipEvent_t ev;
    std::vector<std::pair<void*, size_t>> blocks;
  };
  static constexpr size_t kPinnedStampEvery = 8;
  std::vector<PinnedGroup> pending_pinned_;
  std::vector<std::pair<void*, size_t>> unstamped_pinned_;
  void stamp_pinned_locked();
  uint64_t reserved_ = 0, in_use_ = 0;
  bool prof_on_ = false;
  struct ProfRec {
    std::string name;
    double bytes;
    hipEvent_t a, b;
  };
  std::vector<ProfRec> prof_recs_;
  std::vector<hipEvent_t> ev_pool_;
  struct Side;
  std::atomic<Side*> side_{nullptr};
  std::map<std::string, ProfEntry> prof_;
  friend struct Scope;
};

bool ptr_local_to(const void* p, int dev);

#define GTNX_PROF(name, bytes) ::gtnx::Runtime::Scope _prof_scope(&::gtnx::Runtime::get(), name, bytes)

struct HostTimer {
  const char* name;
  double t0;
  explicit HostTimer(const char* n);
  ~HostTimer();
  static bool enabled();
};
double host_now_ms();
void host_timer_add(const char* name, double ms);
#define GTNX_HT_CAT2(a, b) a##b
#define GTNX_HT_CAT(a, b) GTNX_HT_CAT2(a, b)
#define GTNX_HOST_T(name) ::gtnx::HostTimer GTNX_HT_CAT(_host_t_, __LINE__)(name)

}
```

include/gtn/batch.h:

```cpp
#pragma once
#include <cstdint>
#include <utility>
#include <vector>

#include "gtn/functions.h"

namespace gtn {

class Batch {
 public:
  Batch() = default;
  explicit Batch(const std::vector<Graph>& graphs) {
    auto h = detail::handles(graphs);
    detail::check(gtnx_batch_from_graphs(h.data(), static_cast<int>(h.size()), &h_));
  }
  Batch(const Batch&) = delete;
  Batch& operator=(const Batch&) = delete;
  Batch(Batch&& o) noexcept : h_(o.h_) { o.h_ = nullptr; }
  Batch& operator=(Batch&& o) noexcept {
    if (this != &o) {
      reset();
      h_ = o.h_;
      o.h_ = nullptr;
    }
    return *this;
  }
  ~Batch() { reset(); }

  static Batch ctcTargets(const std::vector<std::vector<int>>& targets, int blank = 0, bool calcGrad = true) {
    std::vector<int> flat, len;
    len.reserve(targets.size());
    size_t total = 0;
    for (auto& t : targets) total += t.size();
    flat.reserve(total);
    for (auto& t : targets) {
      flat.insert(flat.end(), t.begin(), t.end());
      len.push_back(static_cast<int>(t.size()));
    }
    return ctcTargets(flat.data(), len.data(), static_cast<int>(targets.size()), blank, calcGrad);
  }
  static Batch ctcTargets(const int* labels, const int* lengths, int n, int blank = 0, bool calcGrad = true) {
    Batch b;
    detail::check(gtnx_batch_ctc_targets(labels, lengths, n, blank, calcGrad, &b.h_));
    return b;
  }
  static Batch asgForceAlign(const int* labels, const int* lengths, int n, const Graph& transitions, int numLabels) {
    Batch b;
    detail::check(gtnx_batch_asg_force_align(labels, lengths, n, transitions.handle(), numLabels, &b.h_));
    return b;
  }
  static Batch linear(int n, int M, int N, const void* deviceWeights, bool calcGrad = true, bool borrow = false,
                      const int* rows = nullptr) {
    Batch b;
    if (rows)
      detail::check(gtnx_batch_linear_rows(n, M, N, rows, calcGrad, deviceWeights, borrow, &b.h_));
    else
      detail::check(gtnx_batch_linear(n, M, N, calcGrad, deviceWeights, borrow, &b.h_));
    return b;
  }

  int size() const {
    int n = 0;
    if (h_) detail::check(gtnx_batch_size(h_, &n));
    return n;
  }
  Graph operator[](int i) const {
    gtnx_graph_t g;
    detail::check(gtnx_batch_get(h_, i, &g));
    return Graph::fromHandle(g);
  }
  std::vector<float> items() const {
    std::vector<float> v(static_cast<size_t>(size()));
    if (!v.empty()) detail::check(gtnx_batch_items(h_, v.data()));
    return v;
  }
  void itemsToDevice(void* deviceOut) const { detail::check(gtnx_batch_items_device(h_, deviceOut)); }
  void bindGrads(void* deviceOut, const int64_t* offsets) { detail::check(gtnx_batch_grads_bind_device(h_, deviceOut, offsets)); }
  void gradsToDevice(void* deviceOut, const int64_t* offsets) const {
    detail::check(gtnx_batch_grads_device(h_, deviceOut, offsets));
  }
  gtnx_batch_t handle() const { return h_; }
  static Batch fromHandle(gtnx_batch_t h) {
    Batch b;
    b.h_ = h;
    return b;
  }

 private:
  void reset() {
    if (h_) gtnx_batch_destroy(h_);
    h_ = nullptr;
  }
  gtnx_batch_t h_ = nullptr;
};

namespace detail {
template <class F>
Batch batchUnary(F f, const Batch& a) {
  gtnx_batch_t out;
  check(f(a.handle(), &out));
  return Batch::fromHandle(out);
}
template <class F>
Batch batchBinary(F f, const Batch& a, const Batch& b) {
  gtnx_batch_t out;
  check(f(a.handle(), b.handle(), &out));
  return Batch::fromHandle(out);
}
}

namespace batched {
inline Batch negate(const Batch& a) { return detail::batchUnary(&gtnx_batch_negate, a); }
inline Batch add(const Batch& a, const Batch& b) { return detail::batchBinary(&gtnx_batch_add, a, b); }
inline Batch subtract(const Batch& a, const Batch& b) { return detail::batchBinary(&gtnx_batch_subtract, a, b); }
inline Batch subtract(const Batch& a, const Batch& b, void* itemsDevice) {
  gtnx_batch_t out;
  detail::check(gtnx_batch_subtract_into(a.handle(), b.handle(), itemsDevice, &out));
  return Batch::fromHandle(out);
}
inline Batch compose(const Batch& a, const Batch& b) { return detail::batchBinary(&gtnx_batch_compose, a, b); }
inline Batch intersect(const Batch& a, const Batch& b) { return detail::batchBinary(&gtnx_batch_intersect, a, b); }
inline Batch forwardScore(const Batch& a) { return detail::batchUnary(&gtnx_batch_forward_score, a); }
inline Batch viterbiScore(const Batch& a) { return detail::batchUnary(&gtnx_batch_viterbi_score, a); }
inline Batch viterbiPath(const Batch& a) { return detail::batchUnary(&gtnx_batch_viterbi_path, a); }
inline void viterbiAlign(const Batch& product, int* labelsDevice, int64_t rowStride, int* tokensDevice = nullptr,
                         float* scoresDevice = nullptr, const int* frames = nullptr) {
  detail::check(gtnx_batch_viterbi_align(product.handle(), frames, labelsDevice, rowStride, tokensDevice, scoresDevice));
}
inline void viterbiDecode(const Batch& ems, const Graph& transitions, int* labelsDevice, int64_t rowStride,
                          float* scoresDevice = nullptr, const int* frames = nullptr, int* collapsedDevice = nullptr,
                          int* lengthsDevice = nullptr) {
  detail::check(gtnx_batch_viterbi_decode(ems.handle(), transitions.handle(), frames, labelsDevice, rowStride,
                                          scoresDevice, collapsedDevice, lengthsDevice));
}
inline void linearDecode(const Batch& ems, int* labelsDevice, int64_t rowStride, float* scoresDevice = nullptr,
                         const int* frames = nullptr, int blank = -1, int* collapsedDevice = nullptr,
                         int* startsDevice = nullptr, int* lengthsDevice = nullptr) {
  detail::check(gtnx_batch_linear_decode(ems.handle(), frames, blank, labelsDevice, rowStride, scoresDevice,
                                         collapsedDevice, startsDevice, lengthsDevice));
}
inline void backward(const Batch& a, bool retainGraph = false) { detail::check(gtnx_batch_backward(a.handle(), retainGraph)); }
}

}
```

include/gtn_amd.h:

```cpp
#ifndef GTN_AMD_H
#define GTN_AMD_H

#include <stddef.h>
#include <stdint.h>

#ifdef __cplusplus
extern "C" {
#endif

typedef int gtnx_status_t;
#define GTNX_OK 0
#define GTNX_INVALID_ARGUMENT 1
#define GTNX_LOGIC_ERROR 2
#define GTNX_RUNTIME_ERROR 3
#define GTNX_OUT_OF_RANGE 4
#define GTNX_DEVICE_ERROR 5

typedef struct gtnx_graph_s* gtnx_graph_t;

#define GTNX_EPSILON (-1)

const char* gtnx_last_error(void);
const char* gtnx_version(void);
const char* gtnx_backend(void);
int gtnx_device_count(void);
gtnx_status_t gtnx_set_device(int device);
gtnx_status_t gtnx_get_device(int* device);
gtnx_status_t gtnx_set_stream(void* hip_stream);
gtnx_status_t gtnx_synchronize(void);
gtnx_status_t gtnx_compose_mode(int mode, int* previous);
gtnx_status_t gtnx_memory_stats(uint64_t* reserved, uint64_t* in_use);
gtnx_status_t gtnx_empty_cache(void);
gtnx_status_t gtnx_reclaim(void);
gtnx_status_t gtnx_parallel_enter(void);
gtnx_status_t gtnx_parallel_leave(void);
gtnx_status_t gtnx_parallel_flush(void);

gtnx_status_t gtnx_graph_create(int calc_grad, gtnx_graph_t* out);
gtnx_status_t gtnx_graph_copy(gtnx_graph_t g, gtnx_graph_t* out);
gtnx_status_t gtnx_graph_deep_copy(gtnx_graph_t g, gtnx_graph_t* out);
gtnx_status_t gtnx_graph_destroy(gtnx_graph_t g);
gtnx_status_t gtnx_graph_add_node(gtnx_graph_t g, int start, int accept, int* id);
gtnx_status_t gtnx_graph_add_arc(gtnx_graph_t g, int src, int dst, int ilabel,
                                 int olabel, float weight, int* id);
gtnx_status_t gtnx_graph_add_nodes(gtnx_graph_t g, int n, const uint8_t* start,
                                   const uint8_t* accept);
gtnx_status_t gtnx_graph_add_arcs(gtnx_graph_t g, int n, const int* src,
                                  const int* dst, const int* ilabel,
                                  const int* olabel, const float* weight );
gtnx_status_t gtnx_graph_num_nodes(gtnx_graph_t g, int64_t* out);
gtnx_status_t gtnx_graph_num_arcs(gtnx_graph_t g, int64_t* out);
gtnx_status_t gtnx_graph_num_start(gtnx_graph_t g, int64_t* out);
gtnx_status_t gtnx_graph_num_accept(gtnx_graph_t g, int64_t* out);
gtnx_status_t gtnx_graph_item(gtnx_graph_t g, float* out);
gtnx_status_t gtnx_graph_arc_sort(gtnx_graph_t g, int olabel);
gtnx_status_t gtnx_graph_mark_arc_sorted(gtnx_graph_t g, int olabel);
gtnx_status_t gtnx_graph_ilabel_sorted(gtnx_graph_t g, int* out);
gtnx_status_t gtnx_graph_olabel_sorted(gtnx_graph_t g, int* out);
gtnx_status_t gtnx_graph_weights(gtnx_graph_t g, int mutable_, float** out);
gtnx_status_t gtnx_graph_get_weights(gtnx_graph_t g, float* out);
gtnx_status_t gtnx_graph_set_weights(gtnx_graph_t g, const float* weights);
gtnx_status_t gtnx_graph_set_weights_device(gtnx_graph_t g, const void* device_weights);
gtnx_status_t gtnx_graph_weights_device(gtnx_graph_t g, void** out);
gtnx_status_t gtnx_graph_labels_to_array(gtnx_graph_t g, int* out, int ilabel);
gtnx_status_t gtnx_graph_get_start(gtnx_graph_t g, int* out);
gtnx_status_t gtnx_graph_get_accept(gtnx_graph_t g, int* out);
gtnx_status_t gtnx_graph_is_start(gtnx_graph_t g, int node, int* out);
gtnx_status_t gtnx_graph_is_accept(gtnx_graph_t g, int node, int* out);
gtnx_status_t gtnx_graph_make_accept(gtnx_graph_t g, int node);
gtnx_status_t gtnx_graph_num_out(gtnx_graph_t g, int node, int64_t* out);
gtnx_status_t gtnx_graph_num_in(gtnx_graph_t g, int node, int64_t* out);
gtnx_status_t gtnx_graph_get_out(gtnx_graph_t g, int node, int* out);
gtnx_status_t gtnx_graph_get_in(gtnx_graph_t g, int node, int* out);
gtnx_status_t gtnx_graph_get_arcs(gtnx_graph_t g, int* src, int* dst, int* ilabel, int* olabel);
gtnx_status_t gtnx_graph_get_arc(gtnx_graph_t g, int arc, int* src, int* dst,
                                 int* ilabel, int* olabel, float* weight);
gtnx_status_t gtnx_graph_set_weight(gtnx_graph_t g, int arc, float weight);
gtnx_status_t gtnx_graph_calc_grad(gtnx_graph_t g, int* out);
gtnx_status_t gtnx_graph_set_calc_grad(gtnx_graph_t g, int calc_grad);
gtnx_status_t gtnx_graph_is_grad_available(gtnx_graph_t g, int* out);
gtnx_status_t gtnx_graph_grad(gtnx_graph_t g, gtnx_graph_t* out);
gtnx_status_t gtnx_graph_zero_grad(gtnx_graph_t g);
gtnx_status_t gtnx_graph_add_grad(gtnx_graph_t g, const float* host_grad, int64_t n);
gtnx_status_t gtnx_graph_add_grad_graph(gtnx_graph_t g, gtnx_graph_t other);
gtnx_status_t gtnx_graph_id(gtnx_graph_t g, uintptr_t* out);
typedef gtnx_status_t (*gtnx_grad_fn)(void* ctx, gtnx_graph_t* inputs, int n_inputs, gtnx_graph_t deltas);
gtnx_status_t gtnx_graph_create_op(gtnx_graph_t* inputs, int n_inputs, gtnx_grad_fn grad_fn,
                                   void* ctx, void (*ctx_free)(void*), gtnx_graph_t* out);
gtnx_status_t gtnx_graph_num_inputs(gtnx_graph_t g, int64_t* out);
gtnx_status_t gtnx_graph_get_input(gtnx_graph_t g, int i, gtnx_graph_t* out);
gtnx_status_t gtnx_graph_set_inputs(gtnx_graph_t g, const gtnx_graph_t* inputs, int n);
gtnx_status_t gtnx_graph_set_grad_fn(gtnx_graph_t g, gtnx_grad_fn grad_fn, void* ctx,
                                     void (*ctx_free)(void*));
gtnx_status_t gtnx_graph_has_grad_fn(gtnx_graph_t g, int* out);

gtnx_status_t gtnx_scalar_graph(float value, int calc_grad, gtnx_graph_t* out);
gtnx_status_t gtnx_linear_graph(int M, int N, int calc_grad, gtnx_graph_t* out);
gtnx_status_t gtnx_linear_graph_n(int B, int M, int N, int calc_grad,
                                  const void* device_weights, gtnx_graph_t* out );
gtnx_status_t gtnx_linear_graph_borrow_n(int B, int M, int N, int calc_grad,
                                         const void* device_weights, gtnx_graph_t* out );

gtnx_status_t gtnx_negate(gtnx_graph_t g, gtnx_graph_t* out);
gtnx_status_t gtnx_add(gtnx_graph_t a, gtnx_graph_t b, gtnx_graph_t* out);
gtnx_status_t gtnx_subtract(gtnx_graph_t a, gtnx_graph_t b, gtnx_graph_t* out);
gtnx_status_t gtnx_compose(gtnx_graph_t a, gtnx_graph_t b, gtnx_graph_t* out);
gtnx_status_t gtnx_intersect(gtnx_graph_t a, gtnx_graph_t b, gtnx_graph_t* out);
gtnx_status_t gtnx_forward_score(gtnx_graph_t g, gtnx_graph_t* out);
gtnx_status_t gtnx_viterbi_score(gtnx_graph_t g, gtnx_graph_t* out);
gtnx_status_t gtnx_viterbi_path(gtnx_graph_t g, gtnx_graph_t* out);

gtnx_status_t gtnx_negate_n(const gtnx_graph_t* g, int n, gtnx_graph_t* out);
gtnx_status_t gtnx_add_n(const gtnx_graph_t* a, int na, const gtnx_graph_t* b, int nb, gtnx_graph_t* out);
gtnx_status_t gtnx_subtract_n(const gtnx_graph_t* a, int na, const gtnx_graph_t* b, int nb, gtnx_graph_t* out);
gtnx_status_t gtnx_compose_n(const gtnx_graph_t* a, int na, const gtnx_graph_t* b, int nb, gtnx_graph_t* out);
gtnx_status_t gtnx_intersect_n(const gtnx_graph_t* a, int na, const gtnx_graph_t* b, int nb, gtnx_graph_t* out);
gtnx_status_t gtnx_forward_score_n(const gtnx_graph_t* g, int n, gtnx_graph_t* out);
gtnx_status_t gtnx_viterbi_score_n(const gtnx_graph_t* g, int n, gtnx_graph_t* out);
gtnx_status_t gtnx_viterbi_path_n(const gtnx_graph_t* g, int n, gtnx_graph_t* out);
gtnx_status_t gtnx_items_n(const gtnx_graph_t* g, int n, float* out);
gtnx_status_t gtnx_items_device_n(const gtnx_graph_t* g, int n, void* device_out);
gtnx_status_t gtnx_grads_device_n(const gtnx_graph_t* g, int n, void* device_out, const int64_t* offsets);
gtnx_status_t gtnx_grads_bind_device_n(const gtnx_graph_t* g, int n, void* device_out, const int64_t* offsets);

gtnx_status_t gtnx_clone(gtnx_graph_t g, int projection , gtnx_graph_t* out);
gtnx_status_t gtnx_concat(const gtnx_graph_t* g, int n, gtnx_graph_t* out);
gtnx_status_t gtnx_closure(gtnx_graph_t g, gtnx_graph_t* out);
gtnx_status_t gtnx_union(const gtnx_graph_t* g, int n, gtnx_graph_t* out);
gtnx_status_t gtnx_remove(gtnx_graph_t g, int ilabel, int olabel, gtnx_graph_t* out);

typedef struct gtnx_batch_s* gtnx_batch_t;
gtnx_status_t gtnx_batch_from_graphs(const gtnx_graph_t* g, int n, gtnx_batch_t* out);
gtnx_status_t gtnx_batch_ctc_targets(const int* labels, const int* lengths, int n, int blank, int calc_grad,
                                     gtnx_batch_t* out);
gtnx_status_t gtnx_batch_asg_force_align(const int* labels, const int* lengths, int n, gtnx_graph_t transitions,
                                         int n_labels, gtnx_batch_t* out);
gtnx_status_t gtnx_batch_linear(int n, int M, int N, int calc_grad, const void* device_weights, int borrow,
                                gtnx_batch_t* out);
gtnx_status_t gtnx_batch_linear_rows(int n, int M, int N, const int* rows, int calc_grad, const void* device_weights,
                                     int borrow, gtnx_batch_t* out);
gtnx_status_t gtnx_batch_destroy(gtnx_batch_t b);
gtnx_status_t gtnx_batch_size(gtnx_batch_t b, int* out);
gtnx_status_t gtnx_batch_get(gtnx_batch_t b, int i, gtnx_graph_t* out);
gtnx_status_t gtnx_batch_negate(gtnx_batch_t a, gtnx_batch_t* out);
gtnx_status_t gtnx_batch_add(gtnx_batch_t a, gtnx_batch_t b, gtnx_batch_t* out);
gtnx_status_t gtnx_batch_subtract(gtnx_batch_t a, gtnx_batch_t b, gtnx_batch_t* out);
gtnx_status_t gtnx_batch_subtract_into(gtnx_batch_t a, gtnx_batch_t b, void* items_device, gtnx_batch_t* out);
gtnx_status_t gtnx_batch_compose(gtnx_batch_t a, gtnx_batch_t b, gtnx_batch_t* out);
gtnx_status_t gtnx_batch_intersect(gtnx_batch_t a, gtnx_batch_t b, gtnx_batch_t* out);
gtnx_status_t gtnx_batch_forward_score(gtnx_batch_t a, gtnx_batch_t* out);
gtnx_status_t gtnx_batch_viterbi_score(gtnx_batch_t a, gtnx_batch_t* out);
gtnx_status_t gtnx_batch_viterbi_path(gtnx_batch_t a, gtnx_batch_t* out);
gtnx_status_t gtnx_batch_viterbi_align(gtnx_batch_t a, const int* frames, void* labels_device, int64_t row_stride,
                                       void* tokens_device, void* scores_device);
gtnx_status_t gtnx_batch_align_stats(int64_t* fast, int64_t* fallback);
gtnx_status_t gtnx_batch_viterbi_decode(gtnx_batch_t ems, gtnx_graph_t transitions, const int* frames,
                                        void* labels_device, int64_t row_stride, void* scores_device,
                                        void* collapsed_device, void* lengths_device);
gtnx_status_t gtnx_batch_decode_stats(int64_t* fast, int64_t* fallback);
gtnx_status_t gtnx_batch_full_connect_stats(int64_t* fast, int64_t* fallback);
gtnx_status_t gtnx_batch_linear_decode(gtnx_batch_t ems, const int* frames, int blank, void* labels_device,
                                       int64_t row_stride, void* scores_device, void* collapsed_device,
                                       void* starts_device, void* lengths_device);
gtnx_status_t gtnx_batch_linear_decode_stats(int64_t* fast, int64_t* fallback);
gtnx_status_t gtnx_batch_backward(gtnx_batch_t a, int retain_graph);
gtnx_status_t gtnx_batch_items(gtnx_batch_t a, float* out);
gtnx_status_t gtnx_batch_items_device(gtnx_batch_t a, void* device_out);
gtnx_status_t gtnx_batch_grads_bind_device(gtnx_batch_t a, void* device_out, const int64_t* offsets);
gtnx_status_t gtnx_batch_grads_device(gtnx_batch_t a, void* device_out, const int64_t* offsets);

gtnx_status_t gtnx_backward(gtnx_graph_t g, int retain_graph);
gtnx_status_t gtnx_backward_with_grad(gtnx_graph_t g, gtnx_graph_t grad, int retain_graph);
gtnx_status_t gtnx_backward_n(const gtnx_graph_t* g, int n, int retain_graph);

gtnx_status_t gtnx_equal(gtnx_graph_t a, gtnx_graph_t b, int* out);
gtnx_status_t gtnx_isomorphic(gtnx_graph_t a, gtnx_graph_t b, int* out);

gtnx_status_t gtnx_graph_load_buffer(const void* data, size_t bytes, gtnx_graph_t* out);

typedef struct gtnx_comm_s* gtnx_comm_t;
gtnx_status_t gtnx_comm_create(const int* devices, int n, gtnx_comm_t* out);
gtnx_status_t gtnx_comm_destroy(gtnx_comm_t c);
gtnx_status_t gtnx_comm_size(gtnx_comm_t c, int* n);
gtnx_status_t gtnx_comm_all_gather_f32(gtnx_comm_t c, const void* const* send, void* const* recv, int64_t count);
gtnx_status_t gtnx_comm_all_reduce_sum_f32(gtnx_comm_t c, void* const* bufs, int64_t count);

gtnx_status_t gtnx_prof_enable(int on);
gtnx_status_t gtnx_prof_reset(void);
gtnx_status_t gtnx_prof_get(const char* name, double* total_ms, int64_t* launches,
                            double* algorithmic_bytes);
gtnx_status_t gtnx_debug_viterbi_ties(int64_t* seen, int64_t* unresolved);
gtnx_status_t gtnx_debug_tie_ranks(gtnx_graph_t g, int* queue_rank, int* creation_rank, int* applies);
gtnx_status_t gtnx_prof_names(char* buf, size_t cap);
gtnx_status_t gtnx_debug_symbolic_route(gtnx_graph_t g, int tropical, int* route);
gtnx_status_t gtnx_debug_route_name(int route, char* buf, size_t cap);

#ifdef __cplusplus
}
#endif
#endif
```

Before: 1.004 million losses/s.

## Add fused CTC loss path combining target build, forward score and gradient

Result: no change. 1.004 million losses/s, median of 2 (-0.0%).

```diff
diff --git a/gtn_amd/_capi.py b/gtn_amd/_capi.py
--- a/gtn_amd/_capi.py
+++ b/gtn_amd/_capi.py
@@ -101,6 +101,8 @@
     "gtnx_union": [c_graph_p, C.c_int, c_graph_p],
     "gtnx_batch_from_graphs": [c_graph_p, C.c_int, c_graph_p],
     "gtnx_batch_ctc_targets": [C.c_void_p, C.c_void_p, C.c_int, C.c_int, C.c_int, c_graph_p],
+    "gtnx_batch_ctc_loss": [C.c_void_p, C.c_void_p, C.c_int, C.c_int, C.c_int, C.c_void_p, C.c_int, C.c_int, C.c_void_p,
+                            C.c_void_p, C.c_void_p, c_graph_p, C.c_void_p, C.POINTER(C.c_int)],
     "gtnx_batch_asg_force_align": [C.c_void_p, C.c_void_p, C.c_int, c_graph, C.c_int, c_graph_p],
     "gtnx_batch_linear": [C.c_int, C.c_int, C.c_int, C.c_int, C.c_void_p, C.c_int, c_graph_p],
     "gtnx_batch_linear_rows": [C.c_int, C.c_int, C.c_int, C.c_void_p, C.c_int, C.c_void_p, C.c_int, c_graph_p],
diff --git a/gtn_amd/criteria/ctc_criterion.h b/gtn_amd/criteria/ctc_criterion.h
--- a/gtn_amd/criteria/ctc_criterion.h
+++ b/gtn_amd/criteria/ctc_criterion.h
@@ -56,6 +56,13 @@
   if (frames)
     for (int b = 0; b < B; ++b)
       if (frames[b] < 1 || frames[b] > T) throw std::invalid_argument("[ctcLossBatch] a frame count outside 1 .. T");
+  {
+    double hostMs[3] = {0, 0, 0};
+    if (batched::ctcLoss(labels, lengths, B, blank, targetGrad, emissions, T, C, frames, lossDev, gradDev, targetsOut, hostMs)) {
+      if (times) *times = {hostMs[0], 0, 0, hostMs[1], hostMs[2]};
+      return;
+    }
+  }
   auto t0 = now();
   Batch ctcs = Batch::ctcTargets(labels, lengths, B, blank, targetGrad);
   auto t1 = now();
diff --git a/gtn_amd/csrc/band.hip b/gtn_amd/csrc/band.hip
--- a/gtn_amd/csrc/band.hip
+++ b/gtn_amd/csrc/band.hip
@@ -348,8 +348,9 @@
 __device__ __forceinline__ BandPair band_patched(BandPair P, const BandPatch& pt) {
   if (pt.on) {
     const int b = P.bidx;
-    P.delta = pt.delta + b;
-    P.delta_norm = pt.delta_norm ? pt.delta_norm + b : nullptr;
+    const int sb = pt.on == 2 ? 0 : b;
+    P.delta = pt.delta + sb;
+    P.delta_norm = pt.delta_norm ? pt.delta_norm + sb : nullptr;
     P.rowlse = pt.rowlse ? pt.rowlse + int64_t(b) * pt.M : nullptr;
     P.norm = nullptr;
     P.em_copy = nullptr;
@@ -372,15 +373,16 @@
 }
 
 
-__global__ __launch_bounds__(512) void ctc_targets_kernel(const CtcTargetArgs* __restrict__ args, int blank) {
-  const CtcTargetArgs a = args[blockIdx.x];
+template <bool HEAD, class LabelPtr>
+__device__ __forceinline__ void ctc_targets_body(const CtcTargetArgs& a, LabelPtr lab, int blank) {
   __shared__ __attribute__((aligned(16))) int tl[256 + 4];
   __shared__ __attribute__((aligned(16))) int tk[256 + 4];
   const int N = a.N, U = (N - 1) >> 1, m = threadIdx.x;
   if (m < 260) {
-    const int v = m < U ? a.labels[m] : 0x7fffffff;
+    const int v = m < U ? lab[m] : 0x7fffffff;
     tl[m] = v;
-    tk[m] = (m > 0 && m < U && v != a.labels[m - 1]) ? 1 : 0;
+    tk[m] = (m > 0 && m < U && v != lab[m - 1]) ? 1 : 0;
+    if (HEAD && m < U) const_cast<GTNX_G int*>(a.labels)[m] = v;
   }
   __syncthreads();
   if (m >= N) return;
@@ -411,6 +413,21 @@
   a.snode[rank] = m;
   a.slab[rank] = my;
   if (m == N - 1 && a.n_arcs) a.n_arcs[0] = base + 1 + (m > 0 ? 1 : 0) + skip;
+}
+__global__ __launch_bounds__(512) void ctc_targets_kernel(const CtcTargetArgs* __restrict__ args, int blank) {
+  const CtcTargetArgs a = args[blockIdx.x];
+  ctc_targets_body<false>(a, a.labels, blank);
+}
+__global__ __launch_bounds__(512) void ctc_targets_kernel_step_head(const int* __restrict__ lab_src,
+                                                                    const CtcTargetArgs* __restrict__ args,
+                                                                    const BandPair* __restrict__ pairs_src,
+                                                                    BandPair* __restrict__ pairs_dst, int blank) {
+  const CtcTargetArgs a = args[blockIdx.x];
+  constexpr int PW = int(sizeof(BandPair) / 4);
+  static_assert(sizeof(BandPair) % 4 == 0 && PW <= 512, "the pair is copied by the first lanes of the workgroup");
+  if (threadIdx.x < PW)
+    reinterpret_cast<int*>(pairs_dst + blockIdx.x)[threadIdx.x] = reinterpret_cast<const int*>(pairs_src + blockIdx.x)[threadIdx.x];
+  ctc_targets_body<true>(a, lab_src + a.lab_off, blank);
 }
 
 __global__ __launch_bounds__(512) void band_viterbi_kernel(const BandDecode* __restrict__ pairs) {
@@ -996,5 +1013,9 @@
 void launch_ctc_targets(const CtcTargetArgs* d_args, int n, int blank, hipStream_t st) {
   if (n > 0) hipLaunchKernelGGL(ctc_targets_kernel, dim3(n), dim3(512), 0, st, d_args, blank);
 }
-
-}
+void launch_ctc_step_head(const int* lab_src, const CtcTargetArgs* args, const BandPair* pairs_src, BandPair* pairs_dst,
+                          int n, int blank, hipStream_t st) {
+  if (n > 0) hipLaunchKernelGGL(ctc_targets_kernel_step_head, dim3(n), dim3(512), 0, st, lab_src, args, pairs_src, pairs_dst, blank);
+}
+
+}
diff --git a/gtn_amd/csrc/band_forward_body.inc b/gtn_amd/csrc/band_forward_body.inc
--- a/gtn_amd/csrc/band_forward_body.inc
+++ b/gtn_amd/csrc/band_forward_body.inc
@@ -355,10 +355,14 @@
       if (M.fin[2 * k] > DEADF) S += M.fin[2 * k + 1] * ex2(float(M.find[k] + double(M.fin[2 * k]) - Mx));
     const double z2 = dead ? double(NEGF) : Mx + double(lg2(S));
     P.aoff[0] = z2;
-    P.score[0] = dead ? -__builtin_inff() : float(z2 * LN2);
+    const float sc = dead ? -__builtin_inff() : float(z2 * LN2);
+    P.score[0] = sc;
     if (P.norm) {
       double n2 = 0.0;
       for (int k = 0; k < 16; ++k) n2 += M.red[k];
-      P.norm[0] = n2 < double(DEADF) ? -__builtin_inff() : float(n2 * LN2);
+      const float nv = n2 < double(DEADF) ? -__builtin_inff() : float(n2 * LN2);
+      P.norm[0] = nv;
+      GTNX_G float* const loss = (GTNX_BAND_PAIR).loss;
+      if (loss) loss[0] = nv - sc;
     }
   }
diff --git a/gtn_amd/csrc/batch.cpp b/gtn_amd/csrc/batch.cpp
--- a/gtn_amd/csrc/batch.cpp
+++ b/gtn_amd/csrc/batch.cpp
@@ -407,10 +407,17 @@
 }
 }
 
-BatchP batch_ctc_targets(const int* labels, const int* lengths, int n, int blank, bool calc_grad) {
-  GTNX_HOST_T("batch.ctc_targets");
+namespace {
+struct CtcTargetsPlan {
+  BatchP b;
+  bool device = false;
+  size_t lab_bytes = 0, arg_bytes = 0, rec_bytes = 0;
+};
+CtcTargetsPlan plan_ctc_targets(const int* labels, const int* lengths, int n, int blank, bool calc_grad) {
   if (n < 0) throw_invalid("[gtnx_batch_ctc_targets] negative batch size");
-  BatchP b = make_batch(Batch::CTC_TARGETS, n, calc_grad);
+  CtcTargetsPlan pl;
+  pl.b = make_batch(Batch::CTC_TARGETS, n, calc_grad);
+  Batch* b = pl.b.get();
   b->blank = blank;
   b->lab_off.resize(size_t(n) + 1);
   b->lab_off[0] = 0;
@@ -427,32 +434,26 @@
     b->max_label = std::max(b->max_label, labels[i]);
     mn = std::min(mn, labels[i]);
   }
-  if (mn < 0 || b->max_nodes > band_max_nodes() || n == 0) {
-    std::vector<Graph> gs;
-    gs.reserve(size_t(n));
-    for (int i = 0; i < n; ++i)
-      gs.push_back(ctc_target_graph_host(labels + b->lab_off[size_t(i)], lengths[i], blank, calc_grad));
-    return batch_from_graphs(std::move(gs));
-  }
-  Runtime& rt = Runtime::get();
-  const size_t lab_bytes = align_up(sizeof(int) * (total ? total : 1), 256);
-  const size_t arg_bytes = align_up(sizeof(CtcTargetArgs) * size_t(n), 256);
-  size_t bytes = lab_bytes + arg_bytes;
+  pl.device = !(mn < 0 || b->max_nodes > band_max_nodes() || n == 0);
+  if (!pl.device) return pl;
+  pl.lab_bytes = align_up(sizeof(int) * (total ? total : 1), 256);
+  pl.arg_bytes = align_up(sizeof(CtcTargetArgs) * size_t(n), 256);
+  size_t bytes = pl.lab_bytes + pl.arg_bytes;
   b->rec_off.resize(size_t(n));
   for (int i = 0; i < n; ++i) {
     const size_t N = size_t(2 * lengths[i] + 1);
     b->rec_off[size_t(i)] = bytes;
     bytes += align_up(sizeof(BandNode) * N, 64) + align_up(N, 64) + 2 * align_up(4 * N, 64) + 64;
   }
-  b->rec_mem = rt.alloc(bytes);
-  PinnedMemP pin = rt.alloc_pinned(lab_bytes + arg_bytes);
-  std::memcpy(pin->ptr, labels, sizeof(int) * total);
-  CtcTargetArgs* args = reinterpret_cast<CtcTargetArgs*>(static_cast<char*>(pin->ptr) + lab_bytes);
-  for (int i = 0; i < n; ++i) {
-    const size_t N = size_t(2 * lengths[i] + 1);
-    char* base = b->rec_mem->as<char>(b->rec_off[size_t(i)]);
+  pl.rec_bytes = bytes;
+  return pl;
+}
+void fill_ctc_target_args(const Batch& b, CtcTargetArgs* args) {
+  for (int i = 0; i < b.n; ++i) {
+    const size_t N = size_t(2 * (b.lab_off[size_t(i) + 1] - b.lab_off[size_t(i)]) + 1);
+    char* base = b.rec_mem->as<char>(b.rec_off[size_t(i)]);
     CtcTargetArgs& a = args[size_t(i)];
-    a.labels = b->rec_mem->as<int>() + b->lab_off[size_t(i)];
+    a.labels = b.rec_mem->as<int>() + b.lab_off[size_t(i)];
     a.nodes = reinterpret_cast<BandNode*>(base);
     base += align_up(sizeof(BandNode) * N, 64);
     a.nflags = reinterpret_cast<uint8_t*>(base);
@@ -463,10 +464,30 @@
     base += align_up(4 * N, 64);
     a.n_arcs = reinterpret_cast<int*>(base);
     a.N = int(N);
-    a.pad = 0;
-  }
-  rt.h2d_pinned(b->rec_mem->ptr, pin->ptr, lab_bytes + arg_bytes);
-  launch_ctc_targets(reinterpret_cast<const CtcTargetArgs*>(b->rec_mem->as<char>(lab_bytes)), n, blank, rt.stream());
+    a.lab_off = b.lab_off[size_t(i)];
+  }
+}
+}
+
+BatchP batch_ctc_targets(const int* labels, const int* lengths, int n, int blank, bool calc_grad) {
+  GTNX_HOST_T("batch.ctc_targets");
+  CtcTargetsPlan pl = plan_ctc_targets(labels, lengths, n, blank, calc_grad);
+  BatchP b = pl.b;
+  if (!pl.device) {
+    std::vector<Graph> gs;
+    gs.reserve(size_t(n));
+    for (int i = 0; i < n; ++i)
+      gs.push_back(ctc_target_graph_host(labels + b->lab_off[size_t(i)], lengths[i], blank, calc_grad));
+    return batch_from_graphs(std::move(gs));
+  }
+  Runtime& rt = Runtime::get();
+  const size_t total = size_t(b->lab_off[size_t(n)]);
+  b->rec_mem = rt.alloc(pl.rec_bytes);
+  PinnedMemP pin = rt.alloc_pinned(pl.lab_bytes + pl.arg_bytes);
+  std::memcpy(pin->ptr, labels, sizeof(int) * total);
+  fill_ctc_target_args(*b, reinterpret_cast<CtcTargetArgs*>(static_cast<char*>(pin->ptr) + pl.lab_bytes));
+  rt.h2d_pinned(b->rec_mem->ptr, pin->ptr, pl.lab_bytes + pl.arg_bytes);
+  launch_ctc_targets(reinterpret_cast<const CtcTargetArgs*>(b->rec_mem->as<char>(pl.lab_bytes)), n, blank, rt.stream());
   return b;
 }
 
@@ -820,6 +841,71 @@
 }
 
 namespace {
+struct BandPlan {
+  DevMemP arena;
+  std::vector<BandPair> pairs;
+  size_t o_norm = 0, o_lse = 0;
+};
+double band_forward_bytes(const BandPair& p) { return 4.0 * p.T * p.C + 4.0 * double(p.T + 1) * p.NS; }
+BandPlan plan_band_pairs(const Batch& fx, const Batch& ch, bool want_norm) {
+  Runtime& rt = Runtime::get();
+  const int n = fx.n, T = ch.M, C = ch.C;
+  BandPlan bp;
+  size_t bytes = align_up(4 * size_t(n), 256);
+  bp.o_norm = bytes;
+  bytes = align_up(bytes + 4 * size_t(n), 256);
+  bp.o_lse = bytes;
+  bytes = align_up(bytes + 4 * size_t(n) * size_t(T > 0 ? T : 1), 256);
+  std::vector<size_t> oo, ao;
+  oo.resize(size_t(n));
+  ao.resize(size_t(n));
+  for (int b = 0; b < n; ++b) {
+    const int Ub = fx.lab_off[size_t(b) + 1] - fx.lab_off[size_t(b)];
+    const int N = fx.fal ? Ub + 1 : 2 * Ub + 1;
+    const int ns = band_row_stride(N, band_npl(N));
+    oo[size_t(b)] = bytes;
+    bytes = align_up(bytes + 8 * (4 * size_t(T) + 16), 256);
+    ao[size_t(b)] = bytes;
+    bytes = align_up(bytes + 4 * size_t(T + 1) * size_t(ns), 256);
+  }
+  bp.arena = rt.alloc(bytes);
+  bp.pairs.resize(size_t(n));
+  int64_t goff_run = 0;
+  for (int b = 0; b < n; ++b) {
+    BandPair& p = bp.pairs[size_t(b)];
+    p = BandPair{};
+    const int U = fx.lab_off[size_t(b) + 1] - fx.lab_off[size_t(b)];
+    const size_t N = fx.fal ? size_t(U) + 1 : size_t(2 * U + 1);
+    char* base = fx.rec_mem->as<char>(fx.rec_off[size_t(b)]);
+    p.nodes = reinterpret_cast<BandNode*>(base);
+    base += align_up(sizeof(BandNode) * N, 64);
+    p.nflags = reinterpret_cast<uint8_t*>(base);
+    base += align_up(N, 64);
+    p.snode = reinterpret_cast<int*>(base);
+    base += align_up(4 * N, 64);
+    p.slab = reinterpret_cast<int*>(base);
+    p.n_lab = fx.fal ? U : int(N);
+    p.w = fx.fal ? fx.rec_mem->as<float>(fx.w_off[size_t(b)]) : nullptr;
+    p.em = ch.w_dev + size_t(b) * size_t(T) * size_t(C);
+    p.N = int(N);
+    p.T = ch.rows_of(b);
+    p.C = C;
+    p.NS = band_row_stride(p.N, band_npl(p.N));
+    p.alpha = bp.arena->as<float>(ao[size_t(b)]);
+    p.aoff = bp.arena->as<double>(oo[size_t(b)]);
+    p.score = bp.arena->as<float>(4 * size_t(b));
+    if (want_norm) {
+      p.norm = bp.arena->as<float>(bp.o_norm + 4 * size_t(b));
+      p.rowlse = bp.arena->as<float>(bp.o_lse + 4 * size_t(b) * size_t(T));
+    }
+    p.hot = (!fx.fal && U + 1 >= 8) ? fx.blank : -1;
+    p.lgrn = band_forward_lgrn(C);
+    p.bidx = b;
+    p.goff = goff_run;
+    goff_run += int64_t(fx.elem_size(b));
+  }
+  return bp;
+}
 bool asg_transitions_layout(Graph& g, int N) {
   if (!g.s || g.s->lazy || g.s->deferred || g.s->kind != KIND_EXPLICIT || N < 1) return false;
   if (g.num_nodes() != int64_t(N) + 1 || g.num_arcs() != int64_t(N) * (N + 1)) return false;
@@ -956,25 +1042,10 @@
     auto op = std::make_shared<BFsBandOp>();
     op->inputs = {x};
     const bool want_norm = ch.nc_norm == nullptr;
-    size_t bytes = align_up(4 * size_t(n), 256);
-    const size_t o_norm = bytes;
-    bytes = align_up(bytes + 4 * size_t(n), 256);
-    const size_t o_lse = bytes;
-    bytes = align_up(bytes + 4 * size_t(n) * size_t(T > 0 ? T : 1), 256);
-    std::vector<size_t> oo, ao;
-    oo.resize(size_t(n));
-    ao.resize(size_t(n));
-    for (int b = 0; b < n; ++b) {
-      const int Ub = fx.lab_off[size_t(b) + 1] - fx.lab_off[size_t(b)];
-      const int N = fx.fal ? Ub + 1 : 2 * Ub + 1;
-      const int ns = band_row_stride(N, band_npl(N));
-      oo[size_t(b)] = bytes;
-      bytes = align_up(bytes + 8 * (4 * size_t(T) + 16), 256);
-      ao[size_t(b)] = bytes;
-      bytes = align_up(bytes + 4 * size_t(T + 1) * size_t(ns), 256);
-    }
-    op->arena = rt.alloc(bytes);
-    op->pairs.resize(size_t(n));
+    BandPlan bp = plan_band_pairs(fx, ch, want_norm);
+    const size_t o_norm = bp.o_norm, o_lse = bp.o_lse;
+    op->arena = bp.arena;
+    op->pairs = std::move(bp.pairs);
     std::vector<std::pair<BandLaunchKey, BandPair>> tab;
     tab.reserve(size_t(n));
     double abytes = 0;
@@ -992,46 +1063,15 @@
         pend->settle();
       }
     }
-    int64_t goff_run = 0;
     for (int b = 0; b < n; ++b) {
-      BandPair& p = op->pairs[size_t(b)];
-      p = BandPair{};
-      const int U = fx.lab_off[size_t(b) + 1] - fx.lab_off[size_t(b)];
-      const size_t N = fx.fal ? size_t(U) + 1 : size_t(2 * U + 1);
-      char* base = fx.rec_mem->as<char>(fx.rec_off[size_t(b)]);
-      p.nodes = reinterpret_cast<BandNode*>(base);
-      base += align_up(sizeof(BandNode) * N, 64);
-      p.nflags = reinterpret_cast<uint8_t*>(base);
-      base += align_up(N, 64);
-      p.snode = reinterpret_cast<int*>(base);
-      base += align_up(4 * N, 64);
-      p.slab = reinterpret_cast<int*>(base);
-      p.n_lab = fx.fal ? U : int(N);
-      p.w = fx.fal ? fx.rec_mem->as<float>(fx.w_off[size_t(b)]) : nullptr;
-      p.em = ch.w_dev + size_t(b) * size_t(T) * size_t(C);
-      p.N = int(N);
-      p.T = ch.rows_of(b);
-      p.C = C;
-      p.NS = band_row_stride(p.N, band_npl(p.N));
-      p.alpha = op->arena->as<float>(ao[size_t(b)]);
-      p.aoff = op->arena->as<double>(oo[size_t(b)]);
-      p.score = op->arena->as<float>(4 * size_t(b));
-      if (want_norm) {
-        p.norm = op->arena->as<float>(o_norm + 4 * size_t(b));
-        p.rowlse = op->arena->as<float>(o_lse + 4 * size_t(b) * size_t(T));
-      }
-      p.hot = (!fx.fal && U + 1 >= 8) ? fx.blank : -1;
-      p.lgrn = band_forward_lgrn(C);
-      p.bidx = b;
-      p.goff = goff_run;
-      goff_run += int64_t(fx.elem_size(b));
+      const BandPair& p = op->pairs[size_t(b)];
       BandPair q = p;
       if (fuse_copy) {
         q.em = static_cast<const float*>(pend->src_of(p.em));
         q.em_copy = const_cast<float*>(p.em);
       }
       tab.push_back({BandLaunchKey{C, band_npl(q.N), fx.fal ? 0 : 1, 0, band_vec_ok(q)}, q});
-      abytes += 4.0 * p.T * C + 4.0 * double(p.T + 1) * p.NS + (fuse_copy ? 4.0 * T * C : 0.0);
+      abytes += band_forward_bytes(p) + (fuse_copy ? 4.0 * T * C : 0.0);
     }
     band_launch(tab, false, "band_forward_score", abytes, fuse_copy ? nullptr : &op->fwd_table);
     if (fuse_copy) pend->done.store(true, std::memory_order_release);
@@ -1089,6 +1129,93 @@
   }
   batch_materialise(*x);
   return batch_from_graphs(op_shortest_distance(x->graphs, tropical));
+}
+
+bool batch_ctc_loss(const int* labels, const int* lengths, int n, int blank, bool target_grad, const void* em_dev, int T,
+                    int C, const int* frames, void* loss_dev, void* grad_dev, BatchP* targets_out, double* host_ms) {
+  GTNX_HOST_T("batch.ctc_loss");
+  if (n <= 1 || T < 1 || T > (1 << 20) || !labels || !lengths || !em_dev || !loss_dev) return false;
+  if (C < band_min_labels() || C > band_max_labels()) return false;
+  if (std::getenv("GTNX_NO_CTC_FUSED") || std::getenv("GTNX_NO_BAND_PATCH")) return false;
+  if (frames)
+    for (int b = 0; b < n; ++b)
+      if (frames[b] < 1 || frames[b] > T) return false;
+  const double t0 = host_now_ms();
+  CtcTargetsPlan tp = plan_ctc_targets(labels, lengths, n, blank, target_grad);
+  if (!tp.device || tp.b->max_label >= C) return false;
+  const size_t A = size_t(T) * size_t(C);
+  const float* em = static_cast<const float*>(em_dev);
+  const int npl = band_npl(2 * lengths[0] + 1);
+  BandPair probe{};
+  probe.C = C;
+  probe.em = em;
+  const int vec = band_vec_ok(probe);
+  for (int b = 1; b < n; ++b) {
+    probe.em = em + size_t(b) * A;
+    if (band_npl(2 * lengths[b] + 1) != npl || band_vec_ok(probe) != vec) return false;
+  }
+  const size_t pair_bytes = sizeof(BandPair) * size_t(n);
+  const size_t pin_bytes = tp.lab_bytes + tp.arg_bytes + pair_bytes;
+  if (pin_bytes > Runtime::h2d_kernel_limit()) return false;
+  Runtime& rt = Runtime::get();
+  if (!ptr_local_to(loss_dev, rt.device()) || (grad_dev && !ptr_local_to(grad_dev, rt.device()))) return false;
+
+  Batch& fx = *tp.b;
+  fx.rec_mem = rt.alloc(tp.rec_bytes);
+  BatchP chp = batch_linear(n, T, C, grad_dev != nullptr, em_dev, true, frames);
+  Batch& ch = *chp;
+  BandPlan bp = plan_band_pairs(fx, ch, true);
+  DevMemP table = rt.alloc(pair_bytes);
+  int max_ns = 0;
+  double fwd_bytes = 0;
+  {
+    PinnedMemP pin = rt.alloc_pinned(pin_bytes);
+    char* base = static_cast<char*>(pin->ptr);
+    std::memcpy(base, labels, sizeof(int) * fx.labels.size());
+    fill_ctc_target_args(fx, reinterpret_cast<CtcTargetArgs*>(base + tp.lab_bytes));
+    BandPair* hp = reinterpret_cast<BandPair*>(base + tp.lab_bytes + tp.arg_bytes);
+    for (int b = 0; b < n; ++b) {
+      BandPair& p = bp.pairs[size_t(b)];
+      p.loss = static_cast<float*>(loss_dev) + b;
+      hp[b] = p;
+      max_ns = std::max(max_ns, p.NS);
+      fwd_bytes += band_forward_bytes(p);
+    }
+    GTNX_PROF("ctc_step_head", double(pin_bytes) + double(tp.rec_bytes - tp.arg_bytes) + double(pair_bytes));
+    launch_ctc_step_head(reinterpret_cast<const int*>(base), reinterpret_cast<const CtcTargetArgs*>(base + tp.lab_bytes), hp,
+                         table->as<BandPair>(), n, blank, rt.stream());
+  }
+  const double t1 = host_now_ms();
+  {
+    GTNX_PROF("band_forward_score", fwd_bytes);
+    launch_band_forward(table->as<BandPair>(), n, npl, C, max_ns, true, vec != 0, rt.stream());
+  }
+  const double t2 = host_now_ms();
+  if (grad_dev) {
+    float* ge = static_cast<float*>(grad_dev);
+    pad_fill(ch, ge);
+    if (target_grad) alloc_grad(fx, false);
+    double bytes = 0;
+    for (int b = 0; b < n; ++b) {
+      const BandPair& p = bp.pairs[size_t(b)];
+      bytes += 4.0 * p.T * p.C * 2 + 4.0 * double(p.T + 1) * p.NS + (target_grad ? 4.0 * double(fx.elem_size(b)) : 0.0);
+    }
+    const float* seeds = rt.unit_seeds();
+    BandPatch pt{};
+    pt.on = 2;
+    pt.M = T;
+    pt.delta = seeds;
+    pt.delta_norm = seeds + 1;
+    pt.rowlse = bp.arena->as<float>(bp.o_lse);
+    pt.grad_em = ge;
+    pt.grad_fixed = target_grad ? fx.g_dev : nullptr;
+    pt.A = int64_t(A);
+    band_launch_patched(table, n, BandLaunchKey{C, npl, 1, target_grad ? 1 : 0, vec}, max_ns, pt, "band_forward_score_grad", bytes);
+  }
+  const double t3 = host_now_ms();
+  if (host_ms) host_ms[0] = t1 - t0, host_ms[1] = t2 - t1, host_ms[2] = t3 - t2;
+  if (targets_out) *targets_out = tp.b;
+  return true;
 }
 
 BatchP batch_viterbi_path(const BatchP& x) {
diff --git a/gtn_amd/csrc/batch.h b/gtn_amd/csrc/batch.h
--- a/gtn_amd/csrc/batch.h
+++ b/gtn_amd/csrc/batch.h
@@ -78,6 +78,8 @@
 
 BatchP batch_from_graphs(std::vector<Graph> gs);
 BatchP batch_ctc_targets(const int* labels, const int* lengths, int n, int blank, bool calc_grad);
+bool batch_ctc_loss(const int* labels, const int* lengths, int n, int blank, bool target_grad, const void* em_dev, int T,
+                    int C, const int* frames, void* loss_dev, void* grad_dev, BatchP* targets_out, double* host_ms);
 BatchP batch_asg_force_align(const int* labels, const int* lengths, int n, Graph& transitions, int n_labels);
 BatchP batch_linear(int n, int M, int C, bool calc_grad, const void* dev, bool borrow, const int* rows = nullptr);
 BatchP batch_compose(const BatchP& a, const BatchP& b, bool intersect);
diff --git a/gtn_amd/csrc/capi.cpp b/gtn_amd/csrc/capi.cpp
--- a/gtn_amd/csrc/capi.cpp
+++ b/gtn_amd/csrc/capi.cpp
@@ -768,6 +768,21 @@
                                               gtnx_batch_t* out) {
   return guard([&] { *out = HB(batch_ctc_targets(labels, lengths, n, blank, cg != 0)); });
 }
+GTNX_API gtnx_status_t gtnx_batch_ctc_loss(const int* labels, const int* lengths, int n, int blank, int target_grad,
+                                           const void* emissions_device, int T, int C, const int* frames,
+                                           void* loss_device, void* grad_device, gtnx_batch_t* targets_out,
+                                           double* host_ms, int* taken) {
+  return guard([&] {
+    if (!taken) throw_invalid("[gtnx_batch_ctc_loss] null `taken`");
+    *taken = 0;
+    BatchP targets;
+    if (!batch_ctc_loss(labels, lengths, n, blank, target_grad != 0, emissions_device, T, C, frames, loss_device,
+                        grad_device, targets_out ? &targets : nullptr, host_ms))
+      return;
+    if (targets_out) *targets_out = HB(targets);
+    *taken = 1;
+  });
+}
 GTNX_API gtnx_status_t gtnx_batch_asg_force_align(const int* labels, const int* lengths, int n, gtnx_graph_t transitions,
                                                   int n_labels, gtnx_batch_t* out) {
   return guard([&] { *out = HB(batch_asg_force_align(labels, lengths, n, G(transitions), n_labels)); });
diff --git a/gtn_amd/csrc/kernels.h b/gtn_amd/csrc/kernels.h
--- a/gtn_amd/csrc/kernels.h
+++ b/gtn_amd/csrc/kernels.h
@@ -372,6 +372,7 @@
   const GTNX_G float* delta_norm;
   GTNX_G float* grad_em;
   GTNX_G float* grad_fixed;
+  GTNX_G float* loss;
   int N, T, C, NS;
   int hot;
   int lgrn;
@@ -492,9 +493,12 @@
   GTNX_G int* snode;
   GTNX_G int* slab;
   GTNX_G int* n_arcs;
-  int N, pad;
+  int N;
+  int lab_off;
 };
 void launch_ctc_targets(const CtcTargetArgs* d_args, int n, int blank, hipStream_t st);
+void launch_ctc_step_head(const int* lab_src, const CtcTargetArgs* args, const BandPair* pairs_src, BandPair* pairs_dst,
+                          int n, int blank, hipStream_t st);
 struct AsgFalArgs {
   const GTNX_G int* labels;
   const GTNX_G float* trans_w;
diff --git a/gtn_amd/csrc/runtime.cpp b/gtn_amd/csrc/runtime.cpp
--- a/gtn_amd/csrc/runtime.cpp
+++ b/gtn_amd/csrc/runtime.cpp
@@ -608,12 +608,29 @@
   }
   HIP_CHECK(hipMemcpyAsync(pinned_dst, src, bytes, hipMemcpyDeviceToHost, stream_));
 }
-void Runtime::h2d_pinned(void* dst, const void* pinned_src, size_t bytes) {
-  if (!bytes) return;
+size_t Runtime::h2d_kernel_limit() {
   static const size_t lim = [] {
     const char* e = std::getenv("GTNX_H2D_KERNEL_BYTES");
     return e ? size_t(std::atol(e)) : size_t(1) << 20;
   }();
+  return lim;
+}
+const float* Runtime::unit_seeds() {
+  std::lock_guard<std::mutex> lk(seeds_mu_);
+  if (!unit_seeds_) {
+    DevMemP d = alloc(2 * sizeof(float));
+    PinnedMemP p = alloc_pinned(2 * sizeof(float));
+    p->as<float>()[0] = -1.0f;
+    p->as<float>()[1] = 1.0f;
+    h2d_pinned(d->ptr, p->ptr, 2 * sizeof(float));
+    HIP_CHECK(hipStreamSynchronize(stream_));
+    unit_seeds_ = d;
+  }
+  return unit_seeds_->as<float>();
+}
+void Runtime::h2d_pinned(void* dst, const void* pinned_src, size_t bytes) {
+  if (!bytes) return;
+  const size_t lim = h2d_kernel_limit();
   if (bytes <= lim && local_to(dst, device_)) {
     launch_copy_small(dst, pinned_src, bytes, stream_);
     return;
diff --git a/gtn_amd/csrc/runtime.h b/gtn_amd/csrc/runtime.h
--- a/gtn_amd/csrc/runtime.h
+++ b/gtn_amd/csrc/runtime.h
@@ -93,6 +93,8 @@
   void d2d(void* dst, const void* src, size_t bytes);
   void h2d_pinned(void* dst, const void* pinned_src, size_t bytes);
   void d2h_pinned_async(void* pinned_dst, const void* src, size_t bytes);
+  static size_t h2d_kernel_limit();
+  const float* unit_seeds();
 
   struct MirrorSlot {
     float* ptr = nullptr;
@@ -138,6 +140,8 @@
   std::vector<std::pair<void*, size_t>> unstamped_pinned_;
   void stamp_pinned_locked();
   uint64_t reserved_ = 0, in_use_ = 0;
+  std::mutex seeds_mu_;
+  DevMemP unit_seeds_;
   bool prof_on_ = false;
   struct ProfRec {
     std::string name;
diff --git a/include/gtn/batch.h b/include/gtn/batch.h
--- a/include/gtn/batch.h
+++ b/include/gtn/batch.h
@@ -139,6 +139,16 @@
   detail::check(gtnx_batch_linear_decode(ems.handle(), frames, blank, labelsDevice, rowStride, scoresDevice,
                                          collapsedDevice, startsDevice, lengthsDevice));
 }
+inline bool ctcLoss(const int* labels, const int* lengths, int n, int blank, bool targetGrad, const void* emissionsDevice,
+                    int T, int C, const int* frames, void* lossDevice, void* gradDevice, Batch* targetsOut = nullptr,
+                    double* hostMs = nullptr) {
+  gtnx_batch_t targets = nullptr;
+  int taken = 0;
+  detail::check(gtnx_batch_ctc_loss(labels, lengths, n, blank, targetGrad, emissionsDevice, T, C, frames, lossDevice,
+                                    gradDevice, targetsOut ? &targets : nullptr, hostMs, &taken));
+  if (taken && targetsOut) *targetsOut = Batch::fromHandle(targets);
+  return taken != 0;
+}
 inline void backward(const Batch& a, bool retainGraph = false) { detail::check(gtnx_batch_backward(a.handle(), retainGraph)); }
 }
 
diff --git a/include/gtn_amd.h b/include/gtn_amd.h
--- a/include/gtn_amd.h
+++ b/include/gtn_amd.h
@@ -133,6 +133,9 @@
 gtnx_status_t gtnx_batch_from_graphs(const gtnx_graph_t* g, int n, gtnx_batch_t* out);
 gtnx_status_t gtnx_batch_ctc_targets(const int* labels, const int* lengths, int n, int blank, int calc_grad,
                                      gtnx_batch_t* out);
+gtnx_status_t gtnx_batch_ctc_loss(const int* labels, const int* lengths, int n, int blank, int target_grad,
+                                  const void* emissions_device, int T, int C, const int* frames, void* loss_device,
+                                  void* grad_device, gtnx_batch_t* targets_out, double* host_ms, int* taken);
 gtnx_status_t gtnx_batch_asg_force_align(const int* labels, const int* lengths, int n, gtnx_graph_t transitions,
                                          int n_labels, gtnx_batch_t* out);
 gtnx_status_t gtnx_batch_linear(int n, int M, int N, int calc_grad, const void* device_weights, int borrow,
```
